# Jhuighuy/StormRuler

Hardware: AMD Instinct MI355X
Metric: CG iterations/sec, 256^3 Poisson per GPU (+ SpMV achieved HBM GB/s in `roofline`) (higher is better)
Workload: dtype f64

## Files before the change

include/storm_hip.h:

```cpp
#ifndef STORM_HIP_H_
#define STORM_HIP_H_

#include <stddef.h>
#include <stdint.h>

#ifdef __cplusplus
extern "C" {
#endif
#pragma GCC visibility push(default)

#define STORM_HIP_ABI_VERSION 6
#define STORM_HIP_HAS_TWO_STAGE 1
#define STORM_HIP_HAS_FACE_UPDATE 1
#define STORM_HIP_HAS_REDUCED_RECORDS 1

enum {
  STORM_HIP_OK = 0,
  STORM_HIP_E_INVALID = -1,
  STORM_HIP_E_HIP = -2,
  STORM_HIP_E_NO_DEVICE = -3,
  STORM_HIP_E_COMM = -4,
  STORM_HIP_E_ALLOC = -5,
  STORM_HIP_E_UNSUPPORTED = -6
};
// ... 34 lines not shown

int storm_hip_vec_create(storm_hip_ctx *ctx, int64_t n_owned, int64_t n_halo, storm_hip_vec **out);
int storm_hip_vec_create_like(const storm_hip_vec *other, storm_hip_vec **out);
int storm_hip_vec_destroy(storm_hip_vec *v);
int storm_hip_vec_size(const storm_hip_vec *v, int64_t *n_owned, int64_t *n_halo);
int storm_hip_vec_upload(storm_hip_vec *v, const double *host, int64_t n);
int storm_hip_vec_download(const storm_hip_vec *v, double *host, int64_t n);
int storm_hip_vec_device_ptr(storm_hip_vec *v, void **dev_ptr);
int storm_hip_vec_context(const storm_hip_vec *v, storm_hip_ctx **ctx);
int storm_hip_vec_get(const storm_hip_vec *v, int64_t row, double *value);

int storm_hip_block_get_column(const storm_hip_vec *X, int k, int j, storm_hip_vec *v);
int storm_hip_block_set_column(storm_hip_vec *X, int k, int j, const storm_hip_vec *v);
int storm_hip_block_dot(const storm_hip_vec *A, const storm_hip_vec *B, int k, double *out);
int storm_hip_block_axpy(storm_hip_vec *Y, const double *a, const storm_hip_vec *X, int k);

int storm_hip_fill(storm_hip_vec *y, double value);
int storm_hip_copy(storm_hip_vec *y, const storm_hip_vec *x);
int storm_hip_scale(storm_hip_vec *y, double s);
int storm_hip_div_scalar(storm_hip_vec *y, double s);
int storm_hip_axpy(storm_hip_vec *y, double a, const storm_hip_vec *x);
int storm_hip_xpay(storm_hip_vec *y, const storm_hip_vec *x, double b);
int storm_hip_axpbz(storm_hip_vec *y, double a, const storm_hip_vec *x, double b, const storm_hip_vec *z);
int storm_hip_bicgstab_p(storm_hip_vec *p, const storm_hip_vec *r, double beta, double omega,
                         const storm_hip_vec *v);
int storm_hip_lin3(storm_hip_vec *y, const storm_hip_vec *r, double s, double a, const storm_hip_vec *x,
                   double b, const storm_hip_vec *z);
int storm_hip_vmul_add(storm_hip_vec *y, double s, const storm_hip_vec *a, const storm_hip_vec *b);
enum {
  STORM_HIP_MAP_X0 = 0, STORM_HIP_MAP_X1 = 1, STORM_HIP_MAP_Y = 2, STORM_HIP_MAP_CONST = 3,
  STORM_HIP_MAP_NEG = 8, STORM_HIP_MAP_ABS = 9, STORM_HIP_MAP_SQRT = 10,
  STORM_HIP_MAP_ADD = 16, STORM_HIP_MAP_SUB = 17, STORM_HIP_MAP_MUL = 18, STORM_HIP_MAP_DIV = 19,
  STORM_HIP_MAP_MIN = 20, STORM_HIP_MAP_MAX = 21
};
int storm_hip_map(storm_hip_vec *y, const storm_hip_vec *x0, const storm_hip_vec *x1, const int32_t *program, int n_ops,
                  const double *constants, int n_constants);
int storm_hip_vmul(storm_hip_vec *y, const storm_hip_vec *a, const storm_hip_vec *b);
int storm_hip_vdiv(storm_hip_vec *y, double s, const storm_hip_vec *a, const storm_hip_vec *b);
int storm_hip_fill_randomly(storm_hip_vec *y);
void storm_hip_rng_reset(void);
int storm_hip_dot(const storm_hip_vec *a, const storm_hip_vec *b, double *result);
int storm_hip_norm2(const storm_hip_vec *a, double *result);
int storm_hip_multi_dot(const storm_hip_vec *a, const storm_hip_vec *const *bs, int k, double *out);
int storm_hip_multi_dot_begin(const storm_hip_vec *a, const storm_hip_vec *const *bs, int k, int *request);
int storm_hip_multi_dot_end(storm_hip_ctx *ctx, int request, double *out);
int storm_hip_multi_axpy(storm_hip_vec *y, const double *coefs, const storm_hip_vec *const *xs, int k);


int storm_hip_op_create_from_faces(storm_hip_ctx *ctx, int64_t n_owned, int64_t n_halo,
                                   int64_t n_faces, const int64_t *inner, const int64_t *outer,
                                   const double *coef, int64_t n_bfaces, const int64_t *b_cell,
                                   const double *b_coef, const double *volume, storm_hip_op **out);

int storm_hip_op_create_from_mesh(storm_hip_ctx *ctx, int64_t n_owned, int64_t n_halo, int32_t dim, int64_t n_faces,
                                  const int64_t *inner, const int64_t *outer, const double *area, const double *center,
                                  int64_t n_bfaces, const int64_t *b_cell, const double *b_area, const double *b_center,
                                  const double *volume, storm_hip_op **out);

int storm_hip_op_create_from_face_weights(storm_hip_ctx *ctx, int64_t n_owned, int64_t n_halo,
                                          int64_t n_faces, const int64_t *inner,
                                          const int64_t *outer, const double *w_inner,
                                          const double *w_outer, const double *diag_extra,
                                          storm_hip_op **out);

int storm_hip_op_create_from_face_weights_updatable(storm_hip_ctx *ctx, int64_t n_owned, int64_t n_halo,
                                                    int64_t n_faces, const int64_t *inner,
                                                    const int64_t *outer, const double *w_inner,
                                                    const double *w_outer, const double *diag_extra,
                                                    storm_hip_op **out);
int storm_hip_op_face_count(const storm_hip_op *op, int64_t *n_faces);
int storm_hip_op_set_face_weights(storm_hip_op *op, const storm_hip_vec *w_inner, const storm_hip_vec *w_outer,
                                  const storm_hip_vec *diag_extra);
int storm_hip_op_cells_to_faces(const storm_hip_op *op, const storm_hip_vec *cell, storm_hip_vec *at_inner,
                                storm_hip_vec *at_outer);

int storm_hip_op_create_csr(storm_hip_ctx *ctx, int64_t n_rows, int64_t n_halo,
                            const int64_t *row_ptr, const int64_t *col, const double *val,
                            storm_hip_op **out);

int storm_hip_ctx_set_option(storm_hip_ctx *ctx, const char *key, int64_t value);

int storm_hip_ctx_get_counter(storm_hip_ctx *ctx, const char *key, int64_t *value);

int storm_hip_order_cells(int32_t dim, int64_t n_cells, const double *centers, int32_t mode, int64_t *order_out,
                          int32_t *kind_out);

typedef struct storm_hip_mesh storm_hip_mesh;
typedef struct storm_hip_mesh_view {
  int32_t dim, n_nbrs;
  int64_t n_cells, n_halo, n_faces, n_bfaces;
  const int64_t *inner, *outer;
  const double *area;
  const double *center, *volume;
  const int64_t *b_cell;
  const double *b_area, *b_center;
  const int64_t *global_id;
  const int32_t *halo_owner;
  const int32_t *nbr_rank;
  const int64_t *send_ptr, *send_idx, *recv_ptr;
} storm_hip_mesh_view;

int storm_hip_mesh_read_tetgen(const char *prefix, int32_t dim, storm_hip_mesh **out);
int storm_hip_mesh_from_simplices(int32_t dim, int64_t n_nodes, const double *pos, int64_t n_listed, const int64_t *listed,
                                  const int64_t *listed_label, int64_t n_cells, const int64_t *cells, storm_hip_mesh **out);
int storm_hip_mesh_write_tetgen(const char *prefix, int32_t dim, int64_t n_nodes, const double *pos, int64_t n_listed,
                                const int64_t *listed, const int64_t *listed_label, int64_t n_cells, const int64_t *cells);
int storm_hip_mesh_create(int32_t dim, int64_t n_cells, int64_t n_halo, int64_t n_faces, const int64_t *inner,
                          const int64_t *outer, const double *area, const double *center, const double *volume,
                          int64_t n_bfaces, const int64_t *b_cell, const double *b_area, const double *b_center,
                          const int64_t *global_id, const int32_t *halo_owner, storm_hip_mesh **out);
int storm_hip_mesh_get_view(const storm_hip_mesh *mesh, storm_hip_mesh_view *view);
int storm_hip_mesh_permute_cells(storm_hip_mesh *mesh, const int64_t *order);
int storm_hip_partition_rcb(int32_t dim, int64_t n_cells, const double *centers, int32_t n_parts, int32_t *part_out);
int storm_hip_partition_slabs(int32_t dim, int64_t n_cells, const double *centers, int32_t axis, int32_t n_parts,
                              int32_t *part_out);
int storm_hip_mesh_partition(const storm_hip_mesh *global_mesh, const int32_t *part, int32_t n_parts, int32_t rank,
                             storm_hip_mesh **out);
int storm_hip_mesh_halo_plan(storm_hip_mesh *mesh, int32_t rank);
int storm_hip_op_create_from_mesh_object(storm_hip_ctx *ctx, const storm_hip_mesh *mesh, storm_hip_op **out);
int storm_hip_mesh_destroy(storm_hip_mesh *mesh);

int storm_hip_op_set_halo(storm_hip_op *op, int n_nbrs, const int32_t *nbr_rank,
                          const int64_t *send_ptr, const int64_t *send_idx,
                          const int64_t *recv_ptr);

int storm_hip_op_apply(const storm_hip_op *op, double alpha, double beta, const storm_hip_vec *x,
                       storm_hip_vec *y);

int storm_hip_op_apply_block(const storm_hip_op *op, double alpha, double beta, int k, const storm_hip_vec *X,
                             storm_hip_vec *Y);

int storm_hip_op_get_diagonal(const storm_hip_op *op, double alpha, double beta, int invert, storm_hip_vec *d);

int storm_hip_op_apply_add(const storm_hip_op *op, double alpha, const storm_hip_vec *x, storm_hip_vec *y);

int storm_hip_op_apply2(const storm_hip_op *op, double alpha1, double beta1, double alpha2, double beta2,
                        const storm_hip_vec *x, storm_hip_vec *t, storm_hip_vec *y);

typedef struct storm_hip_op_stats {
  int64_t n_rows, n_cols, nnz_offdiag;
  int64_t ell_slots;
  int64_t tail_nnz, tail_rows;
  int64_t n_slices, max_row_len;
  int64_t n_interior_slices;
  int64_t device_bytes;
  int64_t record_bytes;
  int64_t value_dictionary_size;
  int64_t offset_dictionary_size;
  int64_t paired_rows;
  int64_t tiled_planes;
  int64_t spmv_blocks;
  int64_t xcd_run_blocks;
  int64_t streamed_record_bytes;
} storm_hip_op_stats;
int storm_hip_op_get_stats(const storm_hip_op *op, storm_hip_op_stats *stats);
int storm_hip_op_destroy(storm_hip_op *op);

typedef struct storm_hip_solver_params {
  int64_t num_iterations;
  double absolute_error_tolerance;
  double relative_error_tolerance;
  int64_t num_inner_iterations;
  int32_t check_lag;
  int32_t gram_schmidt;
} storm_hip_solver_params;

typedef struct storm_hip_solver_result {
  int64_t iterations;
  double absolute_error, relative_error, initial_error;
  int32_t converged;
  int32_t path_fallback;
  int64_t num_applies;
} storm_hip_solver_result;

void storm_hip_solver_params_default(storm_hip_solver_params *p);

int storm_hip_solve_cg(const storm_hip_op *op, double alpha, double beta, const storm_hip_vec *b,
                       storm_hip_vec *x, const storm_hip_solver_params *params,
                       storm_hip_solver_result *result, double *history);
int storm_hip_solve_bicgstab(const storm_hip_op *op, double alpha, double beta, const storm_hip_vec *b,
                             storm_hip_vec *x, const storm_hip_solver_params *params,
                             storm_hip_solver_result *result, double *history);
int storm_hip_solve_gmres(const storm_hip_op *op, double alpha, double beta, const storm_hip_vec *b,
                          storm_hip_vec *x, const storm_hip_solver_params *params,
                          storm_hip_solver_result *result, double *history);

int storm_hip_solve_cg2(const storm_hip_op *op, double alpha1, double beta1, double alpha2, double beta2,
                        const storm_hip_vec *b, storm_hip_vec *x, const storm_hip_solver_params *params,
                        storm_hip_solver_result *result, double *history);

int storm_hip_solve_cg_block(const storm_hip_op *op, double alpha, double beta, int k, const storm_hip_vec *B,
                             storm_hip_vec *X, const storm_hip_solver_params *params,
                             storm_hip_solver_result *results, double *histories);

typedef struct storm_hip_krylov storm_hip_krylov;
typedef int (*storm_hip_apply_fn)(void *user, storm_hip_vec *y, const storm_hip_vec *x);

enum storm_hip_method {
  STORM_HIP_CG = 0,
  STORM_HIP_BICGSTAB = 1,
  STORM_HIP_GMRES = 2,
  STORM_HIP_FGMRES = 3,
  STORM_HIP_CGS = 4,
  STORM_HIP_TFQMR = 5,
  STORM_HIP_TFQMR1 = 6,
  STORM_HIP_BICGSTAB_L = 7,
  STORM_HIP_IDRS = 8,
  STORM_HIP_RICHARDSON = 9,
  STORM_HIP_JFNK = 10
};
enum storm_hip_side { STORM_HIP_LEFT = 0, STORM_HIP_RIGHT = 1, STORM_HIP_SYMMETRIC = 2 };

int storm_hip_krylov_create(storm_hip_ctx *ctx, int method, storm_hip_krylov **out);
int storm_hip_krylov_destroy(storm_hip_krylov *k);
int storm_hip_krylov_set_operator(storm_hip_krylov *k, const storm_hip_op *op, double alpha, double beta);
int storm_hip_krylov_set_operator_fn(storm_hip_krylov *k, storm_hip_apply_fn apply, void *user);
int storm_hip_krylov_set_operator_fd(storm_hip_krylov *k, storm_hip_apply_fn apply, void *user,
                                     const storm_hip_vec *x, const storm_hip_vec *w, double mu);
int storm_hip_krylov_apply(storm_hip_krylov *k, const storm_hip_vec *y, storm_hip_vec *z);
int storm_hip_krylov_get_int(const storm_hip_krylov *k, const char *key, int64_t *value);
int storm_hip_krylov_set_operator2(storm_hip_krylov *k, const storm_hip_op *op, double alpha1, double beta1, double alpha2,
                                   double beta2);
int storm_hip_krylov_set_preconditioner_fn(storm_hip_krylov *k, storm_hip_apply_fn apply, void *user, int side);
int storm_hip_krylov_set_preconditioner_diag(storm_hip_krylov *k, const storm_hip_vec *d, int side);
int storm_hip_krylov_set_real(storm_hip_krylov *k, const char *key, double value);
int storm_hip_krylov_solve(storm_hip_krylov *k, const storm_hip_vec *b, storm_hip_vec *x,
                           const storm_hip_solver_params *params, storm_hip_solver_result *result,
                           double *history, int64_t *pre_applies);
int storm_hip_krylov_init(storm_hip_krylov *k, const storm_hip_vec *b, storm_hip_vec *x,
                          const storm_hip_solver_params *params, double *initial_error);
int storm_hip_krylov_iterate(storm_hip_krylov *k, double *error);
int storm_hip_krylov_finalize(storm_hip_krylov *k);

typedef struct storm_hip_cheb storm_hip_cheb;
int storm_hip_cheb_coefficients(double lmin, double lmax, int degree, double *theta, double *c1, double *c2);
int storm_hip_op_gershgorin(const storm_hip_op *op, double alpha, double beta, const storm_hip_vec *scale,
                            double *lambda_max);
int storm_hip_cheb_create(const storm_hip_op *op, double alpha, double beta, const storm_hip_vec *dinv, int degree,
                          double lmin, double lmax, storm_hip_cheb **out);
int storm_hip_cheb_apply(const storm_hip_cheb *h, const storm_hip_vec *r, storm_hip_vec *z);
int storm_hip_cheb_get(const storm_hip_cheb *h, const char *key, double *value);
int storm_hip_cheb_destroy(storm_hip_cheb *h);
int storm_hip_krylov_set_preconditioner_cheb(storm_hip_krylov *k, const storm_hip_cheb *h, int side);

int storm_hip_op_build_reduced(storm_hip_op *op);
int storm_hip_op_drop_reduced(storm_hip_op *op);
int storm_hip_op_reduced_bytes(const storm_hip_op *op, int64_t *record_bytes);
int storm_hip_op_apply_reduced(const storm_hip_op *op, double alpha, double beta, const storm_hip_vec *x, storm_hip_vec *y);
int storm_hip_op_gershgorin_reduced(const storm_hip_op *op, double alpha, double beta, const storm_hip_vec *scale,
                                    double *lambda_max);
int storm_hip_cheb_create_reduced(const storm_hip_op *op, double alpha, double beta, const storm_hip_vec *dinv, int degree,
                                  double lmin, double lmax, storm_hip_cheb **out);

#define STORM_HIP_HAS_AMG 1
typedef struct storm_hip_amg_params {
  double strength_theta;
  double prolongator_omega;
  int32_t smoother_degree;
  double smoother_ratio;
  int32_t max_levels;
  int32_t coarse_rows;
  int32_t reduced_records;
} storm_hip_amg_params;
typedef struct storm_hip_amg_hierarchy storm_hip_amg_hierarchy;
typedef struct storm_hip_amg storm_hip_amg;
void storm_hip_amg_params_default(storm_hip_amg_params *params);
int storm_hip_amg_setup_csr(int64_t n_rows, const int64_t *row_ptr, const int64_t *col, const double *val,
                            const storm_hip_amg_params *params, storm_hip_amg_hierarchy **out);
int storm_hip_amg_hierarchy_destroy(storm_hip_amg_hierarchy *h);
int storm_hip_amg_hierarchy_levels(const storm_hip_amg_hierarchy *h, int *levels);
int storm_hip_amg_hierarchy_level_sizes(const storm_hip_amg_hierarchy *h, int level, int64_t *n_rows, int64_t *nnz_a,
                                        int64_t *n_aggregates, int64_t *nnz_p);
int storm_hip_amg_hierarchy_get_operator(const storm_hip_amg_hierarchy *h, int level, int64_t *row_ptr, int64_t *col,
                                         double *val);
int storm_hip_amg_hierarchy_get_aggregates(const storm_hip_amg_hierarchy *h, int level, int64_t *aggregate);
int storm_hip_amg_hierarchy_get_prolongator(const storm_hip_amg_hierarchy *h, int level, int64_t *row_ptr, int64_t *col,
                                            double *val);
int storm_hip_amg_hierarchy_get_coarse_inverse(const storm_hip_amg_hierarchy *h, double *inverse);
int storm_hip_amg_hierarchy_get(const storm_hip_amg_hierarchy *h, const char *key, double *value);
#define STORM_HIP_HAS_AMG_REFRESH 1
int storm_hip_amg_setup_csr_structural(int64_t n_rows, const int64_t *row_ptr, const int64_t *col, const double *val,
                                       const storm_hip_amg_params *params, storm_hip_amg_hierarchy **out);
int storm_hip_amg_hierarchy_get_strong(const storm_hip_amg_hierarchy *h, int level, uint8_t *mask);
int storm_hip_amg_create_refreshable(storm_hip_op *op, double alpha, double beta, const storm_hip_amg_params *params,
                                     storm_hip_amg **out);
int storm_hip_amg_refresh(storm_hip_amg *h);
int storm_hip_amg_download(storm_hip_amg *h);
int storm_hip_amg_create(storm_hip_op *op, double alpha, double beta, const storm_hip_amg_params *params, storm_hip_amg **out);
int storm_hip_amg_apply(const storm_hip_amg *h, const storm_hip_vec *r, storm_hip_vec *z);
int storm_hip_amg_restrict(const storm_hip_amg *h, int level, const storm_hip_vec *fine, storm_hip_vec *coarse);
int storm_hip_amg_prolong_add(const storm_hip_amg *h, int level, const storm_hip_vec *coarse, storm_hip_vec *fine);
int storm_hip_amg_coarse_solve(const storm_hip_amg *h, const storm_hip_vec *r, storm_hip_vec *z);
int storm_hip_amg_get(const storm_hip_amg *h, const char *key, double *value);
int storm_hip_amg_get_hierarchy(const storm_hip_amg *h, const storm_hip_amg_hierarchy **out);
int storm_hip_amg_destroy(storm_hip_amg *h);
int storm_hip_krylov_set_preconditioner_amg(storm_hip_krylov *k, const storm_hip_amg *h, int side);
#define STORM_HIP_HAS_AMG_NULLSPACE 1
int storm_hip_amg_setup_csr_nullspace(int64_t n_rows, const int64_t *row_ptr, const int64_t *col, const double *val,
                                      const storm_hip_amg_params *params, int structural, storm_hip_amg_hierarchy **out);
int storm_hip_amg_create_nullspace(storm_hip_op *op, double alpha, double beta, const storm_hip_amg_params *params,
                                   int refreshable, storm_hip_amg **out);
int storm_hip_amg_project(const storm_hip_amg *h, storm_hip_vec *v);

#pragma GCC visibility pop
#ifdef __cplusplus
}
// ... 3 lines not shown
```

stormruler_amd/_lib.py:

```python
from __future__ import annotations

import ctypes as C
import os

try:
    import torch
except Exception:
    torch = None

_HERE = os.path.dirname(os.path.abspath(__file__))
LIB_PATH = os.environ.get("STORM_HIP_LIB") or os.path.join(_HERE, "libstorm_hip.so")

if not os.path.exists(LIB_PATH):
    raise ImportError(
        f"{LIB_PATH} is missing: build it with `python -c 'import __graft_entry__ as g; g.build()'` "
        "(or `make -C stormruler_amd/csrc`).  stormruler_amd has no CPU fallback.")

lib = C.CDLL(LIB_PATH, mode=C.RTLD_GLOBAL)

f64p = C.POINTER(C.c_double)
i64p = C.POINTER(C.c_int64)
i32p = C.POINTER(C.c_int32)
vp = C.c_void_p


class SolverParams(C.Structure):
    _fields_ = [("num_iterations", C.c_int64), ("absolute_error_tolerance", C.c_double),
                ("relative_error_tolerance", C.c_double), ("num_inner_iterations", C.c_int64),
                ("check_lag", C.c_int32), ("gram_schmidt", C.c_int32)]


class SolverResult(C.Structure):
    _fields_ = [("iterations", C.c_int64), ("absolute_error", C.c_double), ("relative_error", C.c_double),
                ("initial_error", C.c_double), ("converged", C.c_int32), ("path_fallback", C.c_int32),
                ("num_applies", C.c_int64)]


class OpStats(C.Structure):
    _fields_ = [(n, C.c_int64) for n in ("n_rows", "n_cols", "nnz_offdiag", "ell_slots", "tail_nnz",
                                          "tail_rows", "n_slices", "max_row_len", "n_interior_slices",
                                          "device_bytes", "record_bytes", "value_dictionary_size",
                                          "offset_dictionary_size", "paired_rows", "tiled_planes", "spmv_blocks", "xcd_run_blocks",
                                          "streamed_record_bytes")]


class MeshView(C.Structure):
    _fields_ = [("dim", C.c_int32), ("n_nbrs", C.c_int32), ("n_cells", C.c_int64), ("n_halo", C.c_int64),
                ("n_faces", C.c_int64), ("n_bfaces", C.c_int64), ("inner", i64p), ("outer", i64p), ("area", f64p),
                ("center", f64p), ("volume", f64p), ("b_cell", i64p), ("b_area", f64p), ("b_center", f64p),
                ("global_id", i64p), ("halo_owner", i32p), ("nbr_rank", i32p), ("send_ptr", i64p), ("send_idx", i64p),
                ("recv_ptr", i64p)]


class AmgParams(C.Structure):
    _fields_ = [("strength_theta", C.c_double), ("prolongator_omega", C.c_double), ("smoother_degree", C.c_int32),
                ("smoother_ratio", C.c_double), ("max_levels", C.c_int32), ("coarse_rows", C.c_int32),
                ("reduced_records", C.c_int32)]


ALLREDUCE_FN = C.CFUNCTYPE(C.c_int, C.c_void_p, C.POINTER(C.c_double), C.c_int)
EXCHANGE_FN = C.CFUNCTYPE(C.c_int, C.c_void_p, C.c_int, C.POINTER(C.c_int32), C.POINTER(C.c_int64),
                          C.POINTER(C.c_double), C.POINTER(C.c_int64), C.POINTER(C.c_double))

APPLY_FN = C.CFUNCTYPE(C.c_int, C.c_void_p, C.c_void_p, C.c_void_p)

SIGNATURES = {
    "storm_hip_abi_version": (C.c_int, []),
    "storm_hip_last_error": (C.c_char_p, []),
    "storm_hip_ctx_create": (C.c_int, [C.c_int, C.POINTER(vp)]),
    "storm_hip_ctx_destroy": (C.c_int, [vp]),
    "storm_hip_ctx_sync": (C.c_int, [vp]),
    "storm_hip_ctx_info": (C.c_int, [vp, C.c_char_p, C.c_int, C.POINTER(C.c_int), i64p]),
    "storm_hip_ctx_set_option": (C.c_int, [vp, C.c_char_p, C.c_int64]),
    "storm_hip_order_cells": (C.c_int, [C.c_int32, C.c_int64, C.POINTER(C.c_double), C.c_int32, C.POINTER(C.c_int64),
                                        C.POINTER(C.c_int32)]),
    "storm_hip_ctx_get_counter": (C.c_int, [vp, C.c_char_p, C.POINTER(C.c_int64)]),
    "storm_hip_ctx_get_spmv_profile": (C.c_int, [vp, i64p, f64p, f64p]),
    "storm_hip_ctx_get_spmv_profile_samples": (C.c_int, [vp, C.POINTER(C.c_double), C.c_int64, C.POINTER(C.c_int64)]),
    "storm_hip_timer_start": (C.c_int, [vp]),
    "storm_hip_timer_stop": (C.c_int, [vp, C.POINTER(C.c_float)]),
    "storm_hip_comm_unique_id": (C.c_int, [vp]),
    "storm_hip_ctx_comm_init": (C.c_int, [vp, vp, C.c_int, C.c_int]),
    "storm_hip_ctx_comm_init_host": (C.c_int, [vp, C.c_int, C.c_int, ALLREDUCE_FN, EXCHANGE_FN, vp]),
    "storm_hip_map": (C.c_int, [vp, vp, vp, C.POINTER(C.c_int32), C.c_int, C.POINTER(C.c_double), C.c_int]),
    "storm_hip_ctx_comm_size": (C.c_int, [vp, C.POINTER(C.c_int), C.POINTER(C.c_int)]),
    "storm_hip_ctx_comm_rccl_view": (C.c_int, [vp, C.POINTER(C.c_int), C.POINTER(C.c_int), C.POINTER(C.c_int), C.POINTER(C.c_int),
                                               C.POINTER(C.c_int), C.c_char_p, C.c_int]),
    "storm_hip_ctx_comm_ipc_export": (C.c_int, [vp, C.c_int, C.c_int, C.c_int64, vp]),
    "storm_hip_ctx_comm_init_ipc": (C.c_int, [vp, vp]),
    "storm_hip_vec_create": (C.c_int, [vp, C.c_int64, C.c_int64, C.POINTER(vp)]),
    "storm_hip_vec_create_like": (C.c_int, [vp, C.POINTER(vp)]),
    "storm_hip_vec_destroy": (C.c_int, [vp]),
    "storm_hip_vec_size": (C.c_int, [vp, i64p, i64p]),
    "storm_hip_vec_upload": (C.c_int, [vp, f64p, C.c_int64]),
    "storm_hip_vec_download": (C.c_int, [vp, f64p, C.c_int64]),
    "storm_hip_vec_device_ptr": (C.c_int, [vp, C.POINTER(vp)]),
    "storm_hip_vec_context": (C.c_int, [vp, C.POINTER(vp)]),
    "storm_hip_vec_get": (C.c_int, [vp, C.c_int64, f64p]),
    "storm_hip_fill": (C.c_int, [vp, C.c_double]),
    "storm_hip_copy": (C.c_int, [vp, vp]),
    "storm_hip_scale": (C.c_int, [vp, C.c_double]),
    "storm_hip_div_scalar": (C.c_int, [vp, C.c_double]),
    "storm_hip_axpy": (C.c_int, [vp, C.c_double, vp]),
    "storm_hip_xpay": (C.c_int, [vp, vp, C.c_double]),
    "storm_hip_axpbz": (C.c_int, [vp, C.c_double, vp, C.c_double, vp]),
    "storm_hip_bicgstab_p": (C.c_int, [vp, vp, C.c_double, C.c_double, vp]),
    "storm_hip_fill_randomly": (C.c_int, [vp]),
    "storm_hip_rng_reset": (None, []),
    "storm_hip_lin3": (C.c_int, [vp, vp, C.c_double, C.c_double, vp, C.c_double, vp]),
    "storm_hip_vmul_add": (C.c_int, [vp, C.c_double, vp, vp]),
    "storm_hip_vdiv": (C.c_int, [vp, C.c_double, vp, vp]),
    "storm_hip_vmul": (C.c_int, [vp, vp, vp]),
    "storm_hip_dot": (C.c_int, [vp, vp, f64p]),
    "storm_hip_norm2": (C.c_int, [vp, f64p]),
    "storm_hip_multi_dot": (C.c_int, [vp, C.POINTER(vp), C.c_int, f64p]),
    "storm_hip_multi_dot_begin": (C.c_int, [vp, C.POINTER(vp), C.c_int, C.POINTER(C.c_int)]),
    "storm_hip_multi_dot_end": (C.c_int, [vp, C.c_int, f64p]),
    "storm_hip_multi_axpy": (C.c_int, [vp, f64p, C.POINTER(vp), C.c_int]),
    "storm_hip_block_get_column": (C.c_int, [vp, C.c_int, C.c_int, vp]),
    "storm_hip_block_set_column": (C.c_int, [vp, C.c_int, C.c_int, vp]),
    "storm_hip_block_dot": (C.c_int, [vp, vp, C.c_int, f64p]),
    "storm_hip_block_axpy": (C.c_int, [vp, f64p, vp, C.c_int]),
    "storm_hip_op_create_from_faces": (C.c_int, [vp, C.c_int64, C.c_int64, C.c_int64, i64p, i64p, f64p,
                                                 C.c_int64, i64p, f64p, f64p, C.POINTER(vp)]),
    "storm_hip_op_create_from_mesh": (C.c_int, [vp, C.c_int64, C.c_int64, C.c_int32, C.c_int64, i64p, i64p, f64p, f64p,
                                                C.c_int64, i64p, f64p, f64p, f64p, C.POINTER(vp)]),
    "storm_hip_op_create_from_face_weights": (C.c_int, [vp, C.c_int64, C.c_int64, C.c_int64, i64p, i64p,
                                                        f64p, f64p, f64p, C.POINTER(vp)]),
    "storm_hip_op_create_from_face_weights_updatable": (C.c_int, [vp, C.c_int64, C.c_int64, C.c_int64, i64p, i64p,
                                                                  f64p, f64p, f64p, C.POINTER(vp)]),
    "storm_hip_op_face_count": (C.c_int, [vp, C.POINTER(C.c_int64)]),
    "storm_hip_op_set_face_weights": (C.c_int, [vp, vp, vp, vp]),
    "storm_hip_op_cells_to_faces": (C.c_int, [vp, vp, vp, vp]),
    "storm_hip_op_create_csr": (C.c_int, [vp, C.c_int64, C.c_int64, i64p, i64p, f64p, C.POINTER(vp)]),
    "storm_hip_op_set_halo": (C.c_int, [vp, C.c_int, i32p, i64p, i64p, i64p]),
    "storm_hip_mesh_read_tetgen": (C.c_int, [C.c_char_p, C.c_int32, C.POINTER(vp)]),
    "storm_hip_mesh_from_simplices": (C.c_int, [C.c_int32, C.c_int64, f64p, C.c_int64, i64p, i64p, C.c_int64, i64p, C.POINTER(vp)]),
    "storm_hip_mesh_write_tetgen": (C.c_int, [C.c_char_p, C.c_int32, C.c_int64, f64p, C.c_int64, i64p, i64p, C.c_int64, i64p]),
    "storm_hip_mesh_create": (C.c_int, [C.c_int32, C.c_int64, C.c_int64, C.c_int64, i64p, i64p, f64p, f64p, f64p, C.c_int64,
                                        i64p, f64p, f64p, i64p, i32p, C.POINTER(vp)]),
    "storm_hip_mesh_get_view": (C.c_int, [vp, C.POINTER(MeshView)]),
    "storm_hip_mesh_permute_cells": (C.c_int, [vp, i64p]),
    "storm_hip_partition_rcb": (C.c_int, [C.c_int32, C.c_int64, f64p, C.c_int32, i32p]),
    "storm_hip_partition_slabs": (C.c_int, [C.c_int32, C.c_int64, f64p, C.c_int32, C.c_int32, i32p]),
    "storm_hip_mesh_partition": (C.c_int, [vp, i32p, C.c_int32, C.c_int32, C.POINTER(vp)]),
    "storm_hip_mesh_halo_plan": (C.c_int, [vp, C.c_int32]),
    "storm_hip_op_create_from_mesh_object": (C.c_int, [vp, vp, C.POINTER(vp)]),
    "storm_hip_mesh_destroy": (C.c_int, [vp]),
    "storm_hip_op_apply": (C.c_int, [vp, C.c_double, C.c_double, vp, vp]),
    "storm_hip_op_apply_block": (C.c_int, [vp, C.c_double, C.c_double, C.c_int, vp, vp]),
    "storm_hip_op_apply_add": (C.c_int, [vp, C.c_double, vp, vp]),
    "storm_hip_op_apply2": (C.c_int, [vp, C.c_double, C.c_double, C.c_double, C.c_double, vp, vp, vp]),
    "storm_hip_op_get_diagonal": (C.c_int, [vp, C.c_double, C.c_double, C.c_int, vp]),
    "storm_hip_op_get_stats": (C.c_int, [vp, C.POINTER(OpStats)]),
    "storm_hip_op_destroy": (C.c_int, [vp]),
    "storm_hip_solver_params_default": (None, [C.POINTER(SolverParams)]),
    "storm_hip_solve_cg": (C.c_int, [vp, C.c_double, C.c_double, vp, vp, C.POINTER(SolverParams),
                                     C.POINTER(SolverResult), f64p]),
    "storm_hip_solve_bicgstab": (C.c_int, [vp, C.c_double, C.c_double, vp, vp, C.POINTER(SolverParams),
                                           C.POINTER(SolverResult), f64p]),
    "storm_hip_solve_gmres": (C.c_int, [vp, C.c_double, C.c_double, vp, vp, C.POINTER(SolverParams),
                                        C.POINTER(SolverResult), f64p]),
    "storm_hip_solve_cg2": (C.c_int, [vp, C.c_double, C.c_double, C.c_double, C.c_double, vp, vp, C.POINTER(SolverParams),
                                      C.POINTER(SolverResult), f64p]),
    "storm_hip_solve_cg_block": (C.c_int, [vp, C.c_double, C.c_double, C.c_int, vp, vp, C.POINTER(SolverParams),
                                           C.POINTER(SolverResult), f64p]),
    "storm_hip_krylov_create": (C.c_int, [vp, C.c_int, C.POINTER(vp)]),
    "storm_hip_krylov_destroy": (C.c_int, [vp]),
    "storm_hip_krylov_set_operator": (C.c_int, [vp, vp, C.c_double, C.c_double]),
    "storm_hip_krylov_set_operator2": (C.c_int, [vp, vp, C.c_double, C.c_double, C.c_double, C.c_double]),
    "storm_hip_krylov_set_operator_fn": (C.c_int, [vp, APPLY_FN, vp]),
    "storm_hip_krylov_set_operator_fd": (C.c_int, [vp, APPLY_FN, vp, vp, vp, C.c_double]),
    "storm_hip_krylov_apply": (C.c_int, [vp, vp, vp]),
    "storm_hip_krylov_get_int": (C.c_int, [vp, C.c_char_p, i64p]),
    "storm_hip_krylov_set_preconditioner_fn": (C.c_int, [vp, APPLY_FN, vp, C.c_int]),
    "storm_hip_krylov_set_preconditioner_diag": (C.c_int, [vp, vp, C.c_int]),
    "storm_hip_krylov_set_real": (C.c_int, [vp, C.c_char_p, C.c_double]),
    "storm_hip_krylov_solve": (C.c_int, [vp, vp, vp, C.POINTER(SolverParams), C.POINTER(SolverResult), f64p, i64p]),
    "storm_hip_krylov_init": (C.c_int, [vp, vp, vp, C.POINTER(SolverParams), f64p]),
    "storm_hip_krylov_iterate": (C.c_int, [vp, f64p]),
    "storm_hip_krylov_finalize": (C.c_int, [vp]),
    "storm_hip_cheb_coefficients": (C.c_int, [C.c_double, C.c_double, C.c_int, f64p, f64p, f64p]),
    "storm_hip_op_gershgorin": (C.c_int, [vp, C.c_double, C.c_double, vp, f64p]),
    "storm_hip_cheb_create": (C.c_int, [vp, C.c_double, C.c_double, vp, C.c_int, C.c_double, C.c_double, C.POINTER(vp)]),
    "storm_hip_cheb_create_reduced": (C.c_int, [vp, C.c_double, C.c_double, vp, C.c_int, C.c_double, C.c_double, C.POINTER(vp)]),
    "storm_hip_op_build_reduced": (C.c_int, [vp]),
    "storm_hip_op_drop_reduced": (C.c_int, [vp]),
    "storm_hip_op_reduced_bytes": (C.c_int, [vp, C.POINTER(C.c_int64)]),
    "storm_hip_op_apply_reduced": (C.c_int, [vp, C.c_double, C.c_double, vp, vp]),
    "storm_hip_op_gershgorin_reduced": (C.c_int, [vp, C.c_double, C.c_double, vp, f64p]),
    "storm_hip_cheb_apply": (C.c_int, [vp, vp, vp]),
    "storm_hip_cheb_get": (C.c_int, [vp, C.c_char_p, f64p]),
    "storm_hip_cheb_destroy": (C.c_int, [vp]),
    "storm_hip_krylov_set_preconditioner_cheb": (C.c_int, [vp, vp, C.c_int]),
    "storm_hip_amg_params_default": (None, [C.POINTER(AmgParams)]),
    "storm_hip_amg_setup_csr": (C.c_int, [C.c_int64, i64p, i64p, f64p, C.POINTER(AmgParams), C.POINTER(vp)]),
# ... 47 lines not shown
```

stormruler_amd/csrc/common.hpp:

```cpp
#pragma once

#include <hip/hip_runtime.h>

#include <cstdint>
#include <cstdio>
#include <string>
#include <unordered_map>
#include <vector>

#include "../../include/storm_hip.h"

namespace storm {

void set_error(const char *fmt, ...) __attribute__((format(printf, 1, 2)));

#define STORM_FAIL(code, ...)        \
  do {                               \
    ::storm::set_error(__VA_ARGS__); \
    return (code);                   \
  } while (0)

#define STORM_REQUIRE(cond, ...) \
  do {                           \
    if (!(cond)) STORM_FAIL(STORM_HIP_E_INVALID, __VA_ARGS__); \
  } while (0)

#define HIP_TRY(expr)                                                               \
  do {                                                                              \
    hipError_t e_ = (expr);                                                         \
    if (e_ != hipSuccess)                                                           \
      STORM_FAIL(STORM_HIP_E_HIP, "%s failed: %s (%s:%d)", #expr, hipGetErrorString(e_), \
                 __FILE__, __LINE__);                                               \
  } while (0)

#define STORM_TRY(expr)        \
  do {                         \
    int s_ = (expr);           \
    if (s_ != 0) return s_;    \
  } while (0)

constexpr int kWave = 64;
constexpr int kBlock = 256;
constexpr int kNumXcd = 8;
constexpr int kMaxReduceBlocks = 2048;
constexpr int kMaxMulti = 64;
constexpr int kResultRing = 8;
constexpr int kSlab = 256;
constexpr int kStateRing = 64;
constexpr int kStage2 = 128;
constexpr int kSinglePassPartials = 8192;

struct SolverState {
  double s[kSlab];
  double initial_error;
  double absolute_error;
  double relative_error;
  double abs_tol, rel_tol;
  long long iteration;
  long long num_iterations;
  int done;
  int converged;
  double *history;
  unsigned long long *done_ring;
  int verify_failed;
  unsigned long long ring_gen;
};
constexpr unsigned long long kRingIterMask = (1ull << 43) - 1;
__host__ __device__ inline unsigned long long ring_word(unsigned long long gen, unsigned long long iteration, bool done) {
  return ((gen & 0xfffffull) << 44) | ((iteration & kRingIterMask) << 1) | (done ? 1ull : 0ull);
}

struct Comm;

struct LazyStmt {
  int kind = 0;
  double *y = nullptr;
  const double *v[2] = {nullptr, nullptr};
  double c[2] = {0.0, 0.0};
  int nt = 0;
  int64_t n = 0;
  const storm_hip_op *op = nullptr;
  double alpha = 0.0, beta = 0.0;
  const double *x = nullptr;
  storm_hip_vec *yvec = nullptr;
};

struct KrylovRes {
  SolverState *d_st = nullptr, *h_st = nullptr;
  unsigned long long *h_ring = nullptr, *d_ring = nullptr;
  double *S = nullptr;
  int S_cap = 0;
};

}

struct storm_hip_ctx {
  int device = 0;
  hipStream_t stream = nullptr;
  hipStream_t comm_stream = nullptr;
  hipEvent_t ev_x_ready = nullptr, ev_halo_done = nullptr;
  hipEvent_t ev_t0 = nullptr, ev_t1 = nullptr;
  int num_cus = 0;
  std::string name;
  int64_t total_mem = 0;
  double *d_partials = nullptr;
  int64_t partials_capacity = 0;
  double *d_partials2 = nullptr;
  double *d_scalars = nullptr;
  unsigned long long lat_seq = 0;
  double *d_gmres = nullptr;
  size_t gmres_capacity = 0;
  double *d_ticket_sums = nullptr;
  int *d_tickets = nullptr;
  char *d_lat_slots = nullptr;
  double *h_scalars = nullptr;
  unsigned long long *h_result_words = nullptr, *d_result_words = nullptr;
  unsigned result_seq = 0;
  struct ResultSlot {
    unsigned tag = 0;
    int k = 0;
    bool ready = false;
    double value[storm::kMaxMulti] = {};
  } result_ring[storm::kResultRing];
  storm::SolverState *d_state = nullptr;
  storm::SolverState *h_state = nullptr;
  unsigned long long *h_done_ring = nullptr;
  unsigned long long *d_done_ring = nullptr;
  std::vector<storm::KrylovRes> krylov_free;
  unsigned long long ring_gen = 0;
  int64_t opt_ell_cap = 0;
  int64_t opt_spmv_dict = 4;
  int64_t opt_spmv_spw = 0;
  int64_t opt_spmv_xcd_remap = 8;
  int64_t opt_spmv_xcd_remap_sell = 64;
  int64_t opt_nt = 1;
  int stream_reverse = 0;
  int spmv_reverse = 0;
  int64_t opt_spmv_canon_tile_min_rows = (int64_t)1 << 20;
  int64_t opt_spmv_record_index = 1;
  int64_t opt_spmv_canon_tile = 2;
  int64_t opt_mgs_steps = 4;
  int64_t opt_resident_early = 1;
  int64_t opt_resident_apply_cache = 1;
  int64_t opt_resident_halo_interleave = 1;
  int64_t opt_coop_mgs_prefetch = 1;
  int64_t opt_coop_mgs_lds_prefetch = 1;
  int64_t opt_coop_mgs_rotate_early = 1;
  int64_t opt_coop_mgs_alternate = 1;
  int64_t opt_coop_mgs_xcd_runs = 1;
  int64_t opt_coop_mgs_apply = 1;
  int64_t opt_coop_mgs_quad = 1;
  char *d_quad_slots = nullptr;
  int64_t opt_coop_mgs_lds = 1;
  int64_t opt_spmv_mixed = 1;
  int64_t opt_profile_spmv = 0;
  std::vector<storm::LazyStmt> lazy_q;
  std::unordered_map<const void *, int> occupancy;
  int64_t opt_test_disable = 0;
  int64_t opt_lazy = 0;
  int callback_depth = 0;
  int64_t n_lazy_fused_dots = 0, n_lazy_fused_pairs = 0, n_lazy_apply_dots = 0, n_lazy_cg_steps = 0;
  storm_hip_vec *lazy_spare = nullptr;
  int64_t opt_profile_comm = 0;
  int64_t opt_blas1_nt = 1;
  int64_t opt_coop_mgs = 1;
  int64_t opt_latency_publish = 1;
  int64_t opt_coop_plain = 1;
  int64_t opt_coop_force_fail = 0;
  int coop_ran = 0;
  int coop_disabled = 0;
  int coop_fallback = 0;
  int64_t coop_skip = 0, coop_backoff = 0;
  int64_t opt_latency_path = 1;
  int64_t opt_resident_path = 1;
  int64_t opt_resident_max_rows = (int64_t)1 << 22;
  int64_t opt_resident_planes = 0;
  char *d_res_exch = nullptr;
  int64_t res_exch_rows = 0;
  int64_t opt_resident_profile = 0;
  long long *d_res_prof = nullptr;
  int res_prof_blocks = 0;
  char *d_res_slots = nullptr;
  int opt_lin_fuse = 1;
  int64_t opt_ticket_verify_inject = 0;
  int64_t opt_ticket_verify = 0;
  int opt_ticket_reduce = 1;
  int opt_fused_reduce = 1;
  int opt_latency_cache = 1;
  int64_t opt_latency_rows = 1 << 19;
  int64_t opt_rccl_fused = 1;
  int64_t opt_rccl_ticket = 1;
  int64_t opt_comm_wait_seconds = 120;
  int64_t opt_rccl_flag_wait = 1;
  int64_t opt_rccl_early_halo = 1;
  int64_t opt_generic_solvers = 0;
  int64_t opt_cg_march_fill = 2048;
  int64_t opt_cg_march_alternate = 1;
  int64_t opt_cg_march = 8;
  int64_t opt_cg_residual_march = 1;
  int64_t opt_cg_residual_planes = 1;
  int64_t opt_cg_residual_chunk = 16;
  int64_t opt_cg_residual_fill = 512;
  int64_t opt_cg_pz_fold = 1;
  int64_t opt_cg_fuse = 1;
  std::vector<std::pair<size_t, double *>> pool;
  struct VecArena {
    char *base = nullptr;
    size_t bytes = 0, pitch = 0;
    int slots = 0, used = 0;
  };
  std::vector<VecArena> arenas;
  int64_t opt_vec_arena = 1;
  size_t pool_bytes = 0;
  int64_t opt_pool_bytes = (int64_t)16 << 30;
  std::vector<hipEvent_t> prof_events;
  size_t prof_used = 0;
  const int *api_done = nullptr;
  int64_t n_resident_solves = 0, n_latency_solves = 0, n_throughput_solves = 0, n_engine_solves = 0, n_cg_fused_steps = 0;
  int64_t n_host_reductions = 0;
  int64_t n_jfnk_inner_solves = 0;
  int64_t n_fd_fused_dots = 0;
  int64_t n_block_solves = 0;
  int64_t n_op_face_updates = 0;
  int64_t opt_cheb_fused = 1;
  int64_t n_cheb_fused_applies = 0, n_cheb_statement_applies = 0;
  int64_t n_op_reduced_builds = 0, n_op_reduced_refreshes = 0;
  int64_t n_cheb_reduced_applies = 0;
  int64_t opt_amg_fused = 1;
  int64_t n_amg_applies = 0, n_amg_fused_residuals = 0, n_amg_statement_residuals = 0;
  int64_t n_amg_refreshes = 0;
  int64_t n_amg_projections = 0, n_amg_fused_projections = 0;
  int64_t n_cg_residual_marches = 0;
  int64_t n_cg_residual_plane_marches = 0;
  int64_t n_cg_pz_consumer_folds = 0;
  int64_t n_mgs_chain_steps = 0, n_mgs_quad_steps = 0;
  int64_t n_mgs_lds_steps = 0;
  storm::Comm *comm = nullptr;
  int n_ranks = 1, rank = 0;
};

struct storm_hip_vec {
  storm_hip_ctx *ctx = nullptr;
  int64_t n_owned = 0, n_halo = 0;
  double *d = nullptr;
  double *base = nullptr;
  size_t bytes = 0;
  bool exposed = false;
};
constexpr int kVecGuard = 32;

namespace storm {

struct HaloPlan {
  int n_nbrs = 0;
  std::vector<int> nbr_rank;
  std::vector<int64_t> send_ptr, recv_ptr;
  int *d_send_idx = nullptr;
  double *d_sendbuf = nullptr;
  int64_t n_send = 0;
};

}

struct storm_hip_op {
  storm_hip_ctx *ctx = nullptr;
  int64_t n_rows = 0, n_halo = 0;
  int64_t n_slices = 0, n_interior_slices = 0;
  int64_t nnz = 0, ell_slots = 0, max_row_len = 0;
  int64_t *d_slice_off = nullptr;
  char *d_pack = nullptr;
  double *d_dict = nullptr;
  int dict_size = 0;
  int *d_offs = nullptr;
  int offs_size = 0;
  int xcd_group_sell = 0;
  int pair = 0;
  uint8_t *d_rec_idx = nullptr;
  uint64_t *d_rec_words = nullptr;
  int rec_words = 0;
  char *d_bnd_pack = nullptr;
  int bnd_width = 0;
  int canon_k = 0, canon_m1 = -1;
  int canon_off[7] = {0, 0, 0, 0, 0, 0, 0};
  int64_t pack_bytes = 0;
  int64_t spw = 1;
  int64_t tail_rows = 0, tail_nnz = 0;
  int *d_tail_row = nullptr;
  int64_t *d_tail_ptr = nullptr;
  int *d_tail_col = nullptr;
  double *d_tail_val = nullptr;
  int uniform_width = 0;
  std::vector<int> h_interior, h_boundary;
  int *d_interior = nullptr, *d_boundary = nullptr;
  int64_t n_interior = 0, n_boundary = 0;
  int64_t int_plane0 = 0, int_plane1 = 0;
  int64_t device_bytes = 0;
  char *d_lat_pack = nullptr;
  int64_t *d_lat_off = nullptr;
  int64_t lat_bytes = 0;
  storm::HaloPlan halo;
  int updatable = 0;
  int64_t n_faces = 0;
  int *d_src = nullptr, *d_tail_src = nullptr;
  int *d_face_inner = nullptr, *d_face_outer = nullptr;
  char *d_pack32 = nullptr;
  int64_t *d_slice_off32 = nullptr;
  float *d_tail_val32 = nullptr;
  int64_t pack32_bytes = 0;
};

constexpr int kChebMaxDegree = 16;
struct storm_hip_cheb {
  storm_hip_ctx *ctx = nullptr;
  const storm_hip_op *op = nullptr;
  double alpha = 0.0, beta = 0.0;
  const storm_hip_vec *dinv = nullptr;
  int degree = 0;
  double lmin = 0.0, lmax = 0.0, theta = 0.0, inv_theta = 0.0;
  double c1[kChebMaxDegree] = {}, c2[kChebMaxDegree] = {};
  storm_hip_vec *d[2] = {nullptr, nullptr}, *res = nullptr;
  int reduced = 0;
};

namespace storm {

struct Scal {
  const double *p;
  double v;
  double sign;
};
static inline Scal host_scal(double v) { return Scal{nullptr, v, 1.0}; }
static inline Scal dev_scal(const double *p, double sign = 1.0) { return Scal{p, 0.0, sign}; }

constexpr int kUnroll = 4;
constexpr int kStreamBlockElems = kBlock * kUnroll * 2;
constexpr int kMaxStreamBlocks = 32768;
static inline int stream_blocks(int64_t n) {
  int64_t b = (n + kStreamBlockElems - 1) / kStreamBlockElems;
  if (b < 1) b = 1;
  if (b > kMaxStreamBlocks) b = kMaxStreamBlocks;
  return (int)b;
}

constexpr int64_t kBlas1NtRows = (int64_t)6 << 20;
static inline int stream_nt(const storm_hip_ctx *c, int64_t n) {
  return (c->opt_blas1_nt == 2 || (c->opt_blas1_nt == 1 && n >= kBlas1NtRows)) ? 1 : 0;
}

int k_fill(storm_hip_ctx *c, double *y, int64_t n, double v);
int k_copy(storm_hip_ctx *c, double *y, const double *x, int64_t n, const int *done);
int k_scale(storm_hip_ctx *c, double *y, int64_t n, Scal s, bool divide, const int *done);
int k_axpbz(storm_hip_ctx *c, double *y, Scal a, const double *x, Scal b, const double *z,
            int64_t n, const int *done);
int k_bicg_p(storm_hip_ctx *c, double *p, const double *r, Scal beta, Scal omega, const double *v,
             int64_t n, const int *done);
int k_multi_dot(storm_hip_ctx *c, const double *a, const double *const *bs, int k, int64_t n,
                double *d_out, const int *done);
int k_multi_dot_partials(storm_hip_ctx *c, const double *a, const double *const *bs, int k, int64_t n,
                         int *nb_out, const int *done);
int k_multi_axpy(storm_hip_ctx *c, double *y, const double *d_coef, double sign,
                 const double *const *xs, int k, int64_t n, const int *done);
int k_dot_partials(storm_hip_ctx *c, const double *a, const double *b, int64_t n, double *partials, int nb,
                   const int *done);
int k_reduce_final(storm_hip_ctx *c, const double *partials, int nblocks, int k, double *d_out,
                   const int *done);
int k_reduce_stage1(storm_hip_ctx *c, const double **partials, int *nblocks, int k, const int *done);

int partials_reserve(storm_hip_ctx *c, int64_t need);
#define STORM_K_SWITCH(k, GO) \
  switch (k) {                \
    case 1: GO(1); break;     \
    case 2: GO(2); break;     \
    case 3: GO(3); break;     \
    case 4: GO(4); break;     \
    case 5: GO(5); break;     \
    case 6: GO(6); break;     \
    case 7: GO(7); break;     \
    default: GO(8); break;    \
  }
int vec_create_work(const storm_hip_vec *like, storm_hip_vec **out);
int vec_create_work_batch(const storm_hip_vec *like, int count, storm_hip_vec **out);
int state_read(storm_hip_ctx *c, const SolverState *d_state, SolverState *h_pinned);
int state_init(storm_hip_ctx *c, SolverState *d_state, double abs_tol, double rel_tol, long long num_iterations, double *history,
               unsigned long long *d_ring);

int ring_wait(storm_hip_ctx *c, volatile unsigned long long *ring, int64_t it, bool *stop, unsigned long long generation);

struct SpmvDot {
  const double *w = nullptr;
  bool yy = false;
  double *partials = nullptr;
  int *nblocks_out = nullptr;
  double *out[2] = {nullptr, nullptr};
  int *ticketed_out = nullptr;
  struct {
    const long long *iteration = nullptr;
    long long my_iteration = 0;
    const double *ca = nullptr, *cb = nullptr;
    double *x = nullptr;
    const double *r = nullptr;
    double *p_out = nullptr;
    double ca_imm = 0.0, cb_imm = 0.0;
  } cg;
};
int spmv_launch(const storm_hip_op *op, Scal alpha, Scal beta, const double *x, double *y,
                const SpmvDot *dot, const int *done, bool accumulate = false);
int spmv_grid_blocks(const storm_hip_op *op);
bool spmv_can_fuse_cg(const storm_hip_op *op);
bool spmv_can_march(const storm_hip_op *op);
int op_upload_slice_lists(storm_hip_op *op);
int spmv_block_launch(const storm_hip_op *op, double alpha, double beta, int k, const double *X, double *Y,
                      double *pz_partials, int *n_partials, const int *done);
int spmv_block_check(const storm_hip_op *op, int k, const storm_hip_vec *X, const storm_hip_vec *Y, const char *what);

constexpr int kLatBlock = 1024;
int occupancy_cached(storm_hip_ctx *c, const void *fn, int threads, size_t dyn_lds);
bool coop_launch(storm_hip_ctx *c, const void *fn, unsigned blocks, void **args, size_t dyn_lds = 0, unsigned threads = kLatBlock);
constexpr int kStatusCoopGaveUp = 1000;
int lat_check_gave_up(storm_hip_ctx *c);
int coop_solve_with_fallback(storm_hip_ctx *c, storm_hip_vec *x, int (*run)(void *), void *arg, int *fallback_out);

struct PackOptions {
  int64_t ell_cap = 0, spmv_dict = 4, spmv_mixed = 1, spmv_spw = 0, latency_path = 1, latency_rows = 1 << 19;
  int64_t updatable = 0;
};
struct OpImage {
  int64_t n_rows = 0, n_halo = 0, nnz = 0, n_slices = 0, max_row_len = 0, ell_slots = 0;
  int uniform_width = 0, pair = 0, bnd_width = 0, canon_k = 0, canon_m1 = -1;
  int canon_off[7] = {0, 0, 0, 0, 0, 0, 0};
  int dict_size = 0, offs_size = 0;
  int64_t spw = 1, tail_rows = 0, tail_nnz = 0, pack_bytes = 0;
  std::vector<int64_t> slice_off;
  std::vector<char> pack;
  std::vector<double> dict;
  std::vector<int> offs;
  std::vector<uint8_t> rec_idx;
  std::vector<uint64_t> rec_words;
  std::vector<char> bnd_pack;
  std::vector<int> tail_row;
  std::vector<int64_t> tail_ptr;
  std::vector<int> tail_col;
  std::vector<double> tail_val;
  std::vector<int> interior, boundary;
  std::vector<int64_t> lat_off;
  std::vector<char> lat_pack;
  int updatable = 0;
  int64_t n_faces = 0;
  std::vector<int> src;
  std::vector<int> tail_src;
  std::vector<int> face_inner, face_outer;
};
int op_pack(const PackOptions &o, int64_t n, int64_t n_halo, const std::vector<int64_t> &row_ptr, const std::vector<int> &col,
            const std::vector<double> &val, const std::vector<double> &ext, OpImage *img, const std::vector<int> *src = nullptr);
int op_pack_from_face_weights(const PackOptions &o, int64_t n_owned, int64_t n_halo, int64_t n_faces, const int64_t *inner,
                              const int64_t *outer, const double *w_inner, const double *w_outer, const double *diag_extra,
                              OpImage *img);
int op_pack_from_faces(const PackOptions &o, int64_t n_owned, int64_t n_halo, int64_t n_faces, const int64_t *inner,
                       const int64_t *outer, const double *coef, int64_t n_bfaces, const int64_t *b_cell, const double *b_coef,
                       const double *volume, OpImage *img);
int op_pack_from_mesh(const PackOptions &o, int64_t n_owned, int64_t n_halo, int32_t dim, int64_t n_faces, const int64_t *inner,
                      const int64_t *outer, const double *area, const double *center, int64_t n_bfaces, const int64_t *b_cell,
                      const double *b_area, const double *b_center, const double *volume, OpImage *img);
int op_pack_csr(const PackOptions &o, int64_t n_rows, int64_t n_halo, const int64_t *row_ptr, const int64_t *col,
                const double *val, OpImage *img);

int gershgorin_run(const storm_hip_op *op, bool reduced, double alpha, double beta, const storm_hip_vec *scale, double *lambda_max);
int op_reduced_check(const storm_hip_op *op, const char *who);
int op_reduced_require(const storm_hip_op *op, const char *who);
int op_reduced_convert(storm_hip_op *op, int *d_flag);
int op_reduced_apply(const storm_hip_op *op, double alpha, double beta, const double *x, double *y, const int *done);

bool cg_latency_eligible(const storm_hip_op *op);
int cg_latency_solve(const storm_hip_op *op, double alpha, double beta, const double *b, double *x, double *p,
                     double *r, SolverState *d_state, bool *taken);
int bicgstab_latency_solve(const storm_hip_op *op, double alpha, double beta, const double *b, double *x,
                           double *const work[4], SolverState *d_state, bool *taken);
int cg2_latency_solve(const storm_hip_op *op, double alpha1, double beta1, double alpha2, double beta2, const double *b,
                      double *x, double *const work[3], SolverState *d_state, bool *taken);

struct MgsGivens {
  SolverState *st;
  double *H, *beta, *cs, *sn, *hn_slot;
};
struct ChainApply {
  const storm_hip_op *op;
  double alpha, beta;
  const double *x;
};
int gmres_mgs_chain_coop(storm_hip_ctx *c, int64_t n, const int *done, double *w, const double *const *q, int k, int m,
                         double *H, double *norm2_out, bool normalise, bool *taken, const MgsGivens *givens,
                         const ChainApply *apply = nullptr, bool *applied = nullptr);

int gmres_orthogonalize(storm_hip_ctx *c, int64_t n, const SolverState *st, const int *done, double *qn,
                        const double *const *q, int k, int m, double *H, double *norm2_out, double *scratch,
                        int gram_schmidt, bool *normalised, const MgsGivens *givens = nullptr,
                        bool *givens_done = nullptr, const ChainApply *apply = nullptr);
int cg2_latency_try(const storm_hip_op *op, double alpha1, double beta1, double alpha2, double beta2, const storm_hip_vec *b,
                    storm_hip_vec *x, const storm_hip_solver_params *params, storm_hip_solver_result *result, double *history,
                    bool *taken);

bool res_eligible(const storm_hip_op *op, bool bicgstab);
int res_solve(bool bicgstab, const storm_hip_op *op, double alpha, double beta, const double *b, double *x, double *rt,
              SolverState *d_state, bool *taken);

int lazy_flush(storm_hip_ctx *c);
static inline int lazy_sync(storm_hip_ctx *c) { return (c != nullptr && !c->lazy_q.empty()) ? lazy_flush(c) : 0; }
int lazy_push_lin(storm_hip_ctx *c, storm_hip_vec *y, double c0, const double *v0, double c1, const double *v1, int nt, int64_t n);
int lazy_push_apply(const storm_hip_op *op, double alpha, double beta, const double *x, double *y);
bool lazy_try_dot(storm_hip_ctx *c, const double *a, const double *b, int64_t n, double *result, int *status);

int comm_allreduce_sum(storm_hip_ctx *c, double *d_buf, int count);
int comm_halo_exchange_begin(const storm_hip_op *op, double *x);
int comm_halo_exchange_end(const storm_hip_op *op);
bool comm_is_rccl(const storm_hip_ctx *c);
int comm_halo_exchange_begin_direction(const storm_hip_op *op, const double *p, const double *r, const double *cb, double *p_out);
void comm_forget_prebegun(storm_hip_ctx *c);
int comm_halo_exchange_begin_formed(const storm_hip_op *op, int mode, const double *r, const double *p, const double *v,
                                    const double *sa, const double *sb, double *target, double *alpha_seen = nullptr);
void comm_destroy(storm_hip_ctx *c);
int comm_check_error(storm_hip_ctx *c);
struct IpcDev;
struct IpcSendPlan;
struct IpcRecvPlan;
bool comm_ipc_next(storm_hip_ctx *c, IpcDev *w);
bool comm_is_ipc(const storm_hip_ctx *c);
long long comm_ipc_stat(storm_hip_ctx *c, int k);
int comm_profile_reset(storm_hip_ctx *c);
long long comm_profile_read(storm_hip_ctx *c, int k);
int comm_ipc_exchange(const storm_hip_op *op, IpcDev *w, IpcSendPlan *sp, IpcRecvPlan *rp);
int comm_ipc_send(const storm_hip_op *op, const double *x, const IpcDev &w, const IpcSendPlan &sp);
int comm_ipc_recv_copy(const storm_hip_op *op, double *x, const IpcDev &w, const IpcRecvPlan &rp);

}
```

stormruler_amd/csrc/context.hip:

```cpp
#include <cstdarg>
#include <cstring>
#include <random>

#include <algorithm>
#include "common.hpp"

#include <cstddef>

namespace storm {

static thread_local char g_error[1024] = "";

void set_error(const char *fmt, ...) {
  va_list ap;
  va_start(ap, fmt);
  vsnprintf(g_error, sizeof g_error, fmt, ap);
  va_end(ap);
}

}

using namespace storm;

static void pool_release(storm_hip_ctx *c);
// ... 42 lines not shown
  HIP_TRY(hipMalloc((void **)&c->d_lat_slots, 2 * 256 * 256 + 256));
  HIP_TRY(hipMemset(c->d_lat_slots, 0, 2 * 256 * 256 + 256));
  HIP_TRY(hipMalloc((void **)&c->d_ticket_sums, sizeof(double) * 8 * 2048));
  HIP_TRY(hipMalloc((void **)&c->d_tickets, sizeof(int) * (1 + 2048) * 16));
  HIP_TRY(hipMemset(c->d_tickets, 0, sizeof(int) * (1 + 2048) * 16));
  HIP_TRY(hipMalloc((void **)&c->d_state, sizeof(SolverState)));
  HIP_TRY(hipMemset(c->d_state, 0, sizeof(SolverState)));
  HIP_TRY(hipHostMalloc((void **)&c->h_state, sizeof(SolverState), hipHostMallocMapped));
  HIP_TRY(hipHostMalloc((void **)&c->h_done_ring, sizeof(unsigned long long) * kStateRing, hipHostMallocMapped));
  HIP_TRY(hipHostGetDevicePointer((void **)&c->d_done_ring, c->h_done_ring, 0));
  *out = c;
  return STORM_HIP_OK;
}

int storm_hip_ctx_destroy(storm_hip_ctx *c) {
  if (!c) return STORM_HIP_OK;
  (void)hipSetDevice(c->device);
  c->lazy_q.clear();
  if (c->lazy_spare) (void)storm_hip_vec_destroy(c->lazy_spare), c->lazy_spare = nullptr;
  (void)hipDeviceSynchronize();
  comm_destroy(c);
  for (auto &r : c->krylov_free) {
    if (r.S) (void)hipFree(r.S);
    (void)hipFree(r.d_st);
    (void)hipHostFree(r.h_st);
    (void)hipHostFree(r.h_ring);
  }
  for (auto &ev : c->prof_events) (void)hipEventDestroy(ev);
  pool_release(c);
  for (auto &a : c->arenas) (void)hipFree(a.base);
  (void)hipFree(c->d_partials);
  if (c->d_gmres) (void)hipFree(c->d_gmres);
  (void)hipFree(c->d_partials2);
  (void)hipFree(c->d_scalars);
  (void)hipFree(c->d_lat_slots);
  if (c->d_res_exch) (void)hipFree(c->d_res_exch);
  if (c->d_res_slots) (void)hipFree(c->d_res_slots);
  if (c->d_quad_slots) (void)hipFree(c->d_quad_slots);
  if (c->d_res_prof) (void)hipFree(c->d_res_prof);
  (void)hipFree(c->d_tickets);
  (void)hipFree(c->d_ticket_sums);
  (void)hipHostFree(c->h_scalars);
  (void)hipHostFree(c->h_result_words);
  (void)hipFree(c->d_state);
  (void)hipHostFree(c->h_state);
  (void)hipHostFree(c->h_done_ring);
  (void)hipEventDestroy(c->ev_x_ready);
  (void)hipEventDestroy(c->ev_halo_done);
  (void)hipEventDestroy(c->ev_t0);
  (void)hipEventDestroy(c->ev_t1);
  (void)hipStreamDestroy(c->stream);
  (void)hipStreamDestroy(c->comm_stream);
  delete c;
  return STORM_HIP_OK;
}

int storm_hip_ctx_sync(storm_hip_ctx *c) {
  STORM_REQUIRE(c, "ctx_sync: null context");
  STORM_TRY(lazy_sync(c));
  HIP_TRY(hipStreamSynchronize(c->comm_stream));
  HIP_TRY(hipStreamSynchronize(c->stream));
  return comm_check_error(c);
}

int storm_hip_ctx_info(storm_hip_ctx *c, char *name, int name_len, int *num_cus,
                       int64_t *total_mem_bytes) {
  STORM_REQUIRE(c, "ctx_info: null context");
  if (name && name_len > 0) {
    strncpy(name, c->name.c_str(), (size_t)name_len - 1);
    name[name_len - 1] = 0;
  }
  if (num_cus) *num_cus = c->num_cus;
  if (total_mem_bytes) *total_mem_bytes = c->total_mem;
  return STORM_HIP_OK;
}

int storm_hip_ctx_set_option(storm_hip_ctx *c, const char *key, int64_t value) {
  STORM_REQUIRE(c && key, "ctx_set_option: null argument");
  if (!strcmp(key, "ell_cap")) c->opt_ell_cap = value;
  else if (!strcmp(key, "generic_solvers")) c->opt_generic_solvers = value;
  else if (!strcmp(key, "rccl_fused")) c->opt_rccl_fused = value;
  else if (!strcmp(key, "rccl_ticket")) c->opt_rccl_ticket = value;
  else if (!strcmp(key, "rccl_early_halo")) c->opt_rccl_early_halo = value;
  else if (!strcmp(key, "rccl_flag_wait")) c->opt_rccl_flag_wait = value;
  else if (!strcmp(key, "comm_wait_seconds")) {
    STORM_REQUIRE(value >= 1 && value <= 3600, "ctx_set_option: comm_wait_seconds %lld (1 .. 3600)", (long long)value);
    c->opt_comm_wait_seconds = value;
  }
  else if (!strcmp(key, "latency_path")) c->opt_latency_path = value;
  else if (!strcmp(key, "resident_path")) c->opt_resident_path = value;
  else if (!strcmp(key, "resident_max_rows")) c->opt_resident_max_rows = value;
  else if (!strcmp(key, "resident_planes")) c->opt_resident_planes = value;
  else if (!strcmp(key, "resident_profile")) c->opt_resident_profile = value;
  else if (!strcmp(key, "coop_force_fail")) c->opt_coop_force_fail = value;
  else if (!strcmp(key, "coop_mgs")) c->opt_coop_mgs = value;
  else if (!strcmp(key, "coop_mgs_lds")) c->opt_coop_mgs_lds = value;
  else if (!strcmp(key, "coop_mgs_quad")) c->opt_coop_mgs_quad = value;
  else if (!strcmp(key, "cg_march_fill")) c->opt_cg_march_fill = value;
  else if (!strcmp(key, "resident_early")) c->opt_resident_early = value;
  else if (!strcmp(key, "mgs_steps")) c->opt_mgs_steps = value;
  else if (!strcmp(key, "vec_arena")) c->opt_vec_arena = value;
  else if (!strcmp(key, "spmv_mixed")) c->opt_spmv_mixed = value;
  else if (!strcmp(key, "spmv_canon_tile")) c->opt_spmv_canon_tile = value;
  else if (!strcmp(key, "spmv_canon_tile_min_rows")) c->opt_spmv_canon_tile_min_rows = value;
  else if (!strcmp(key, "fused_reduce")) c->opt_fused_reduce = (int)value;
  else if (!strcmp(key, "ticket_reduce")) c->opt_ticket_reduce = (int)value;
  else if (!strcmp(key, "ticket_verify")) c->opt_ticket_verify = value;
  else if (!strcmp(key, "ticket_verify_inject")) c->opt_ticket_verify_inject = value;
  else if (!strcmp(key, "lin_fuse")) c->opt_lin_fuse = (int)value;
  else if (!strcmp(key, "latency_rows")) c->opt_latency_rows = value;
  else if (!strcmp(key, "latency_cache")) c->opt_latency_cache = (int)value;
  else if (!strcmp(key, "nontemporal")) c->opt_nt = value;
  else if (!strcmp(key, "spmv_dict")) c->opt_spmv_dict = value;
  else if (!strcmp(key, "pool_bytes")) {
    c->opt_pool_bytes = value;
    if ((int64_t)c->pool_bytes > value || (value == 0 && !c->pool.empty())) {
      (void)hipStreamSynchronize(c->stream);
      pool_release(c);
    }
  }
  else if (!strcmp(key, "spmv_spw")) c->opt_spmv_spw = value;
  else if (!strcmp(key, "spmv_xcd_remap")) {
    STORM_REQUIRE(value >= 0 && value <= 4096, "ctx_set_option: spmv_xcd_remap %lld (0 .. 4096)", (long long)value);
    c->opt_spmv_xcd_remap = c->opt_spmv_xcd_remap_sell = value;
  }
  else if (!strcmp(key, "test_disable")) {
    c->opt_test_disable = value;
    c->opt_coop_mgs_apply = !(value & 1), c->opt_coop_mgs_prefetch = c->opt_coop_mgs_lds_prefetch = !(value & 2);
    c->opt_resident_apply_cache = !(value & 4), c->opt_resident_halo_interleave = !(value & 8);
    c->opt_latency_publish = !(value & 16), c->opt_coop_plain = !(value & 32), c->opt_cg_march_alternate = !(value & 64);
    c->opt_coop_mgs_xcd_runs = !(value & 128), c->opt_coop_mgs_alternate = !(value & 256);
    c->opt_coop_mgs_rotate_early = !(value & 512);
  }
  else if (!strcmp(key, "lazy_statements")) {
    if (value == 0) {
      STORM_TRY(lazy_sync(c));
      if (c->lazy_spare) (void)storm_hip_vec_destroy(c->lazy_spare), c->lazy_spare = nullptr;
    }
    c->opt_lazy = value;
  }
  else if (!strcmp(key, "profile_spmv")) c->opt_profile_spmv = value;
  else if (!strcmp(key, "profile_comm")) {
    c->opt_profile_comm = value;
    if (value != 0) STORM_TRY(comm_profile_reset(c));
  }
  else if (!strcmp(key, "cg_fuse")) c->opt_cg_fuse = value;
  else if (!strcmp(key, "cg_march")) c->opt_cg_march = value;
  else if (!strcmp(key, "cg_residual_march")) c->opt_cg_residual_march = value;
  else if (!strcmp(key, "cg_residual_planes")) c->opt_cg_residual_planes = value;
  else if (!strcmp(key, "cg_residual_chunk")) c->opt_cg_residual_chunk = value;
  else if (!strcmp(key, "cg_residual_fill")) c->opt_cg_residual_fill = value;
  else if (!strcmp(key, "cg_pz_fold")) c->opt_cg_pz_fold = value;
  else if (!strcmp(key, "spmv_record_index")) c->opt_spmv_record_index = value;
  else if (!strcmp(key, "blas1_nt")) c->opt_blas1_nt = value;
  else if (!strcmp(key, "cheb_fused")) c->opt_cheb_fused = value;
  else if (!strcmp(key, "amg_fused")) c->opt_amg_fused = value;
  else STORM_FAIL(STORM_HIP_E_INVALID, "ctx_set_option: unknown key '%s'", key);
  return STORM_HIP_OK;
}

int storm_hip_ctx_get_counter(storm_hip_ctx *c, const char *key, int64_t *value) {
  STORM_REQUIRE(c && key && value, "ctx_get_counter: null argument");
  if (!strcmp(key, "resident_solves")) *value = c->n_resident_solves;
  else if (!strcmp(key, "latency_solves")) *value = c->n_latency_solves;
  else if (!strcmp(key, "throughput_solves")) *value = c->n_throughput_solves;
  else if (!strcmp(key, "engine_solves")) *value = c->n_engine_solves;
  else if (!strcmp(key, "block_solves")) *value = c->n_block_solves;
  else if (!strcmp(key, "op_face_updates")) *value = c->n_op_face_updates;
  else if (!strcmp(key, "host_reductions")) *value = c->n_host_reductions;
  else if (!strcmp(key, "cheb_fused_applies")) *value = c->n_cheb_fused_applies;
  else if (!strcmp(key, "cheb_statement_applies")) *value = c->n_cheb_statement_applies;
  else if (!strcmp(key, "cheb_reduced_applies")) *value = c->n_cheb_reduced_applies;
  else if (!strcmp(key, "amg_applies")) *value = c->n_amg_applies;
  else if (!strcmp(key, "amg_fused_residuals")) *value = c->n_amg_fused_residuals;
  else if (!strcmp(key, "amg_statement_residuals")) *value = c->n_amg_statement_residuals;
  else if (!strcmp(key, "amg_refreshes")) *value = c->n_amg_refreshes;
  else if (!strcmp(key, "option_spmv_dict")) *value = c->opt_spmv_dict;
  else if (!strcmp(key, "amg_projections")) *value = c->n_amg_projections;
  else if (!strcmp(key, "amg_fused_projections")) *value = c->n_amg_fused_projections;
  else if (!strcmp(key, "op_reduced_builds")) *value = c->n_op_reduced_builds;
  else if (!strcmp(key, "op_reduced_refreshes")) *value = c->n_op_reduced_refreshes;
  else if (!strcmp(key, "jfnk_inner_solves")) *value = c->n_jfnk_inner_solves;
  else if (!strcmp(key, "fd_fused_dots")) *value = c->n_fd_fused_dots;
  else if (!strcmp(key, "cg_fused_steps")) *value = c->n_cg_fused_steps;
  else if (!strcmp(key, "cg_residual_marches")) *value = c->n_cg_residual_marches;
  else if (!strcmp(key, "cg_residual_plane_marches")) *value = c->n_cg_residual_plane_marches;
  else if (!strcmp(key, "cg_pz_consumer_folds")) *value = c->n_cg_pz_consumer_folds;
  else if (!strcmp(key, "mgs_chain_steps")) *value = c->n_mgs_chain_steps;
  else if (!strcmp(key, "mgs_quad_steps")) *value = c->n_mgs_quad_steps;
  else if (!strcmp(key, "mgs_lds_steps")) *value = c->n_mgs_lds_steps;
  else if (!strcmp(key, "lazy_fused_dots")) *value = c->n_lazy_fused_dots;
  else if (!strcmp(key, "lazy_fused_pairs")) *value = c->n_lazy_fused_pairs;
  else if (!strcmp(key, "lazy_apply_dots")) *value = c->n_lazy_apply_dots;
  else if (!strcmp(key, "lazy_cg_steps")) *value = c->n_lazy_cg_steps;
  else if (!strcmp(key, "lazy_waiting")) *value = (int64_t)c->lazy_q.size();
  else if (!strncmp(key, "ipc_", 4)) {
    static const char *names[6] = {"ipc_allreduce_wait_ticks", "ipc_allreduces", "ipc_ack_wait_ticks", "ipc_ack_waits",
                                   "ipc_halo_slow_poll_ticks", "ipc_halo_slow_polls"};
    int k = -1;
    for (int i = 0; i < 6; ++i)
      if (!strcmp(key, names[i])) k = i;
    STORM_REQUIRE(k >= 0, "ctx_get_counter: unknown key '%s'", key);
    const long long v = comm_ipc_stat(c, k);
    STORM_REQUIRE(v >= 0, "ctx_get_counter: '%s' needs the peer-window transport", key);
    *value = v;
  }
  else if (!strncmp(key, "rccl_prof_", 10)) {
    static const char *names[8] = {"rccl_prof_exchanges", "rccl_prof_event_to_comm_ticks", "rccl_prof_pack_ticks",
                                   "rccl_prof_sendrecv_ticks", "rccl_prof_unhidden_wait_ticks", "rccl_prof_resume_ticks",
                                   "rccl_prof_allreduces", "rccl_prof_allreduce_ticks"};
    int k = -1;
    for (int i = 0; i < 8; ++i)
      if (!strcmp(key, names[i])) k = i;
    STORM_REQUIRE(k >= 0, "ctx_get_counter: unknown key '%s'", key);
    const long long v = comm_profile_read(c, k);
    STORM_REQUIRE(v >= 0, "ctx_get_counter: '%s' needs the RCCL transport with option profile_comm = 1", key);
    *value = v;
  }
  else if (!strncmp(key, "resident_phase_max_", 19) || !strncmp(key, "resident_phase_mean_", 20)) {
    const bool mx = key[15] == 'm' && key[16] == 'a';
    const int k = atoi(key + (mx ? 19 : 20));
    STORM_REQUIRE(c->d_res_prof != nullptr && c->res_prof_blocks > 0 && k >= 0 && k < 8, "ctx_get_counter: no resident profile (option resident_profile)");
    std::vector<long long> h((size_t)c->res_prof_blocks * 8);
    HIP_TRY(hipStreamSynchronize(c->stream));
    HIP_TRY(hipMemcpy(h.data(), c->d_res_prof, sizeof(long long) * h.size(), hipMemcpyDeviceToHost));
    long long m = 0, sum = 0;
    for (int b = 0; b < c->res_prof_blocks; ++b) m = std::max(m, h[(size_t)b * 8 + k]), sum += h[(size_t)b * 8 + k];
    *value = mx ? m : sum / c->res_prof_blocks;
  } else if (!strncmp(key, "resident_phase_block_", 21)) {
    int b = 0, k = 0;
    STORM_REQUIRE(sscanf(key + 21, "%d_%d", &b, &k) == 2 && c->d_res_prof != nullptr && b >= 0 && b < c->res_prof_blocks && k >= 0 && k < 8,
                  "ctx_get_counter: no such block / phase");
    long long v = 0;
    HIP_TRY(hipStreamSynchronize(c->stream));
    HIP_TRY(hipMemcpy(&v, c->d_res_prof + (size_t)b * 8 + k, sizeof v, hipMemcpyDeviceToHost));
    *value = v;
  }
  else STORM_FAIL(STORM_HIP_E_INVALID, "ctx_get_counter: unknown key '%s'", key);
  return STORM_HIP_OK;
}

int storm_hip_ctx_get_spmv_profile(storm_hip_ctx *c, int64_t *launches, double *total_ms, double *min_ms) {
  STORM_REQUIRE(c, "get_spmv_profile: null context");
  HIP_TRY(hipStreamSynchronize(c->stream));
  double total = 0.0, mn = 0.0;
  const size_t pairs = c->prof_used / 2;
  for (size_t i = 0; i < pairs; ++i) {
    float ms = 0.f;
    HIP_TRY(hipEventElapsedTime(&ms, c->prof_events[2 * i], c->prof_events[2 * i + 1]));
    total += ms;
    if (i == 0 || ms < mn) mn = ms;
  }
  if (launches) *launches = (int64_t)pairs;
  if (total_ms) *total_ms = total;
  if (min_ms) *min_ms = mn;
  c->prof_used = 0;
  return STORM_HIP_OK;
}

int storm_hip_ctx_get_spmv_profile_samples(storm_hip_ctx *c, double *ms_out, int64_t capacity, int64_t *count) {
  STORM_REQUIRE(c && count && (ms_out || capacity == 0), "get_spmv_profile_samples: null argument");
  HIP_TRY(hipStreamSynchronize(c->stream));
  const size_t pairs = c->prof_used / 2;
  for (size_t i = 0; i < pairs && (int64_t)i < capacity; ++i) {
    float ms = 0.f;
    HIP_TRY(hipEventElapsedTime(&ms, c->prof_events[2 * i], c->prof_events[2 * i + 1]));
    ms_out[i] = ms;
  }
  *count = (int64_t)pairs;
  c->prof_used = 0;
  return STORM_HIP_OK;
}

int storm_hip_timer_start(storm_hip_ctx *c) {
  STORM_REQUIRE(c, "timer_start: null context");
  STORM_TRY(lazy_sync(c));
  HIP_TRY(hipEventRecord(c->ev_t0, c->stream));
  return STORM_HIP_OK;
}

int storm_hip_timer_stop(storm_hip_ctx *c, float *elapsed_ms) {
  STORM_REQUIRE(c && elapsed_ms, "timer_stop: null argument");
  STORM_TRY(lazy_sync(c));
  HIP_TRY(hipEventRecord(c->ev_t1, c->stream));
  HIP_TRY(hipEventSynchronize(c->ev_t1));
  HIP_TRY(hipEventElapsedTime(elapsed_ms, c->ev_t0, c->ev_t1));
  return STORM_HIP_OK;
}


}
enum { kZeroAll = 0, kZeroEdges = 1, kZeroNothing = 2 };
static int vec_create_impl(storm_hip_ctx *c, int64_t n_owned, int64_t n_halo, storm_hip_vec **out, int zero_mode);
extern "C" int storm_hip_vec_create(storm_hip_ctx *c, int64_t n_owned, int64_t n_halo, storm_hip_vec **out) {
  return vec_create_impl(c, n_owned, n_halo, out, kZeroAll);
}
namespace storm {
int ring_wait(storm_hip_ctx *c, volatile unsigned long long *ring, int64_t it, bool *stop, unsigned long long generation) {
  volatile unsigned long long *w = ring + it % kStateRing;
  const unsigned long long want = (unsigned long long)(it + 1);
  const unsigned long long gen = generation & 0xfffffull;
  auto posted = [&](bool *s) {
    const unsigned long long v = *w;
    if ((v >> 44) != gen) return false;
    const unsigned long long i = (v >> 1) & kRingIterMask;
    if (i == kRingIterMask) return *s = true, true;
// ... 319 lines not shown
```

stormruler_amd/csrc/op_pack.hip:

```cpp
#include <algorithm>
#include <atomic>
#include <cmath>
#include <cstdlib>
#include <cstring>
#include <numeric>
#include <thread>

#include "common.hpp"
#include "host_threads.hpp"
#include "op_layout.hpp"

namespace storm {
namespace {

int64_t forced_min_chunk() {
  static const int64_t forced = getenv("STORM_HIP_BUILD_MIN_CHUNK") ? atoll(getenv("STORM_HIP_BUILD_MIN_CHUNK")) : 0;
  return forced;
}
template <class F>
int parallel_chunks(int64_t n, int64_t min_chunk, F &&fn) {
  if (forced_min_chunk() > 0) min_chunk = forced_min_chunk();
  const int T = (int)std::max<int64_t>(1, std::min<int64_t>(host_threads(), n / std::max<int64_t>(1, min_chunk)));
  const int64_t per = (n + T - 1) / T;
  if (T == 1) {
// ... 185 lines not shown
      for (int k = 0; k < 7; ++k) {
        wa |= zero_v << (8 * (k + 1)), wb |= zero_v << (8 * (k + 1));
        jw |= (k < m ? ((uint64_t)od.lookup((uint64_t)merged[k]) << 2) : zero_o) << (8 * k);
      }
      for (int k = 0; k < na; ++k) {
        wa &= ~(0xffull << (8 * (pa[k] + 1)));
        wa |= ((uint64_t)vd.lookup(A.val[(size_t)(A.row_ptr[ra] + k)]) << 3) << (8 * (pa[k] + 1));
      }
      for (int k = 0; k < nb2; ++k) {
        wb &= ~(0xffull << (8 * (pb[k] + 1)));
        wb |= ((uint64_t)vd.lookup(A.val[(size_t)(A.row_ptr[rb] + k)]) << 3) << (8 * (pb[k] + 1));
      }
      char *rec = pack.data() + (p / kWave) * kPairRecBytes;
      const int l = (int)(p % kWave);
      reinterpret_cast<uint64_t *>(rec)[2 * l] = wa;
      reinterpret_cast<uint64_t *>(rec)[2 * l + 1] = wb;
      reinterpret_cast<uint64_t *>(rec + 2 * kWave * 8)[l] = jw;
    }
    widths[(size_t)t_] = pair_width;
  });
  return pr_ok.load() != 0 ? *std::max_element(widths.begin(), widths.end()) : 0;
}

int64_t boundary_groups(const Rows &A, std::vector<char> &grp_bnd) {
  grp_bnd.assign((size_t)A.groups(), 0);
  if (A.n_halo == 0) return 0;
  std::vector<int64_t> cnt((size_t)host_threads(), 0);
  parallel_chunks(A.groups(), 1 << 10, [&](int t, int64_t gb, int64_t ge) {
    for (int64_t g = gb; g < ge; ++g) {
      const int64_t r1 = std::min<int64_t>(A.n, (g + 1) * 2 * kWave);
      for (int64_t k = A.row_ptr[g * 2 * kWave]; k < A.row_ptr[r1] && !grp_bnd[(size_t)g]; ++k) grp_bnd[(size_t)g] = A.col[(size_t)k] >= A.n;
      cnt[(size_t)t] += grp_bnd[(size_t)g];
    }
  });
  return std::accumulate(cnt.begin(), cnt.end(), (int64_t)0);
}

struct OffsetRelation {
  int64_t dist[8];
  int nd = 0;
  bool before[8][8] = {};
  bool ok = true;
};
OffsetRelation offset_relation(const Rows &A, const std::vector<char> &grp_bnd) {
  std::vector<OffsetRelation> loc((size_t)host_threads());
  const int T = parallel_chunks(A.n, 1 << 14, [&](int t, int64_t rb_, int64_t re_) {
    OffsetRelation &L = loc[(size_t)t];
    for (int64_t r = rb_; L.ok && r < re_; ++r) {
      if (grp_bnd[(size_t)(r / (2 * kWave))]) continue;
      int idx[8], no = 0;
      for (int64_t k = A.row_ptr[r]; L.ok && k < A.row_ptr[r + 1]; ++k) {
        const int64_t o = (int64_t)A.col[(size_t)k] - r;
        int q = 0;
        while (q < L.nd && L.dist[q] != o) ++q;
        if (q == L.nd) {
          if (L.nd == 7) { L.ok = false; break; }
          L.dist[L.nd++] = o;
        }
        idx[no++] = q;
      }
      for (int i = 0; L.ok && i < no; ++i)
        for (int j = i + 1; j < no; ++j) {
          if (idx[i] == idx[j]) L.ok = false;
          L.before[idx[i]][idx[j]] = true;
        }
    }
  });
  OffsetRelation R;
  for (int t = 0; R.ok && t < T; ++t) {
    const OffsetRelation &L = loc[(size_t)t];
    R.ok = L.ok;
    int map_[8];
    for (int q = 0; R.ok && q < L.nd; ++q) {
      int g = 0;
      while (g < R.nd && R.dist[g] != L.dist[q]) ++g;
      if (g == R.nd) {
        if (R.nd == 7) { R.ok = false; break; }
        R.dist[R.nd++] = L.dist[q];
      }
      map_[q] = g;
    }
    for (int i = 0; R.ok && i < L.nd; ++i)
      for (int j = 0; j < L.nd; ++j)
        if (L.before[i][j]) R.before[map_[i]][map_[j]] = true;
  }
  return R;
}
int common_offset_order(const OffsetRelation &R, int64_t *canon, int *canon_m1) {
  int len = 0, m1 = -1;
  bool placed[8] = {};
  while (R.ok && len < R.nd) {
    int pick = -1;
    for (int q = 0; q < R.nd; ++q) {
      if (placed[q]) continue;
      bool free_ = true;
      for (int q2 = 0; q2 < R.nd; ++q2) free_ = free_ && !(R.before[q2][q] && !placed[q2]);
      if (free_ && (pick < 0 || R.dist[q] < R.dist[pick])) pick = q;
    }
    if (pick < 0) return 0;
    placed[pick] = true;
    canon[len++] = R.dist[pick];
  }
  for (int q = 0; q + 1 < len; ++q)
    if (canon[q] == -1 && canon[q + 1] == 1) m1 = q;
  bool cn = R.ok && ((len == 6 && m1 == 2) || (len == 4 && m1 == 1) || (len == 2 && m1 == 0));
  for (int q = 0; cn && q < len; ++q) cn = canon[q] > -(int64_t)INT32_MAX / 2 && canon[q] < (int64_t)INT32_MAX / 2;
  *canon_m1 = m1;
  return cn ? len : 0;
}

void canonical_records(const Rows &A, const ValueDict &vd, uint64_t zero_v, const std::vector<char> &grp_bnd, const int64_t *canon,
                       std::vector<char> &pack) {
  const int64_t n = A.n;
  pack.assign((size_t)A.groups() * kCanonRecBytes, 0);
  parallel_chunks(A.groups() * kWave, 1 << 13, [&](int, int64_t p_begin, int64_t p_end) {
    for (int64_t p = p_begin; p < p_end; ++p) {
      uint64_t w2[2];
      for (int half = 0; half < 2; ++half) {
        const int64_t r = 2 * p + half;
        uint64_t w = r < n ? ((uint64_t)vd.lookup(A.ext[(size_t)r]) << 3) : zero_v;
        for (int k = 0; k < 7; ++k) w |= zero_v << (8 * (k + 1));
        if (r < n) {
          int q = 0;
          const bool by_entry = grp_bnd[(size_t)(r / (2 * kWave))] != 0;
          for (int64_t k = A.row_ptr[r]; k < A.row_ptr[r + 1]; ++k) {
            if (by_entry) q = (int)(k - A.row_ptr[r]);
            else while (canon[q] != (int64_t)A.col[(size_t)k] - r) ++q;
            w &= ~(0xffull << (8 * (q + 1)));
            w |= ((uint64_t)vd.lookup(A.val[(size_t)k]) << 3) << (8 * (q + 1));
          }
        }
        w2[half] = w;
      }
      uint64_t *rec = reinterpret_cast<uint64_t *>(pack.data() + (p / kWave) * kCanonRecBytes);
      rec[2 * (p % kWave)] = w2[0], rec[2 * (p % kWave) + 1] = w2[1];
    }
  });
}

void row_record_index(const std::vector<char> &pack, std::vector<uint8_t> &rec_idx, std::vector<uint64_t> &rec_words) {
  const int64_t n_words = (int64_t)pack.size() / 8;
  auto word_at = [&](int64_t i) {
    uint64_t w;
    memcpy(&w, pack.data() + (size_t)i * 8, 8);
    return w;
  };
  ValueDict wd;
  if (!wd.add_all(n_words, word_at)) return;
  rec_idx.resize((size_t)n_words);
  parallel_chunks(n_words, 1 << 16, [&](int, int64_t b, int64_t e) {
    for (int64_t i = b; i < e; ++i) rec_idx[(size_t)i] = (uint8_t)wd.lookup(word_at(i));
  });
  rec_words = std::move(wd.values);
}

std::vector<int> slice_widths(const Rows &A, int64_t cap, int64_t slot_bytes, int64_t w_op, OpImage *img) {
  const int64_t n_slices = img->n_slices;
  std::vector<int> width((size_t)n_slices, 0);
  img->slice_off.assign((size_t)n_slices + 1, 0);
  bool uniform = true;
  for (int64_t s = 0; s < n_slices; ++s) {
    int64_t w = 0;
    const int64_t r1 = std::min<int64_t>(A.n, (s + 1) * kWave);
    for (int64_t r = s * kWave; r < r1; ++r) w = std::max(w, A.len(r));
    w = std::min(w, cap);
    if (w_op > 0) w = w_op;
    width[(size_t)s] = (int)w;
    img->slice_off[(size_t)s + 1] = img->slice_off[(size_t)s] + (w_op > 0 ? (int64_t)kWave * 16 : kExtBytes + w * slot_bytes);
    if (s > 0 && width[(size_t)s] != width[0]) uniform = false;
    img->ell_slots += w * kWave;
  }
  img->uniform_width = (uniform && n_slices > 0 && width[0] > 0) ? width[0] : 0;
  return width;
}
void sell_records(const Rows &A, const std::vector<int> &width, ValueDict *vd, ValueDict *od, OpImage *img) {
  const int64_t n = A.n;
  const bool cv = vd != nullptr, co = od != nullptr;
  img->pack.assign((size_t)img->slice_off[(size_t)img->n_slices], 0);
  if (A.src) img->src.assign((size_t)((img->slice_off[(size_t)img->n_slices] - img->n_slices * kExtBytes) / (kSlotBytes / kWave)), -1);
  for (int64_t s = 0; s < img->n_slices; ++s) {
    const int W = width[(size_t)s];
    char *rec = img->pack.data() + img->slice_off[(size_t)s];
    int *s_ = A.src ? img->src.data() + (img->slice_off[(size_t)s] - s * kExtBytes) / (kSlotBytes / kWave) : nullptr;
    double *e_ = reinterpret_cast<double *>(rec);
    uint64_t *i_ = reinterpret_cast<uint64_t *>(rec);
    int *c_ = reinterpret_cast<int *>(rec + kExtBytes);
    double *v_ = reinterpret_cast<double *>(rec + kExtBytes + (int64_t)W * (kWave * 4));
    bool touches_halo = false;
    for (int l = 0; l < kWave; ++l) {
      const int64_t r = s * kWave + l;
      const int64_t pad_col = r < n ? r : (n > 0 ? n - 1 : 0);
      const int64_t b = r < n ? A.row_ptr[r] : 0, e = r < n ? A.row_ptr[r + 1] : 0;
      uint64_t iw = 0, jw = 0;
      if (cv) iw = (uint64_t)vd->index(r < n ? A.ext[(size_t)r] : 0.0);
      else e_[l] = r < n ? A.ext[(size_t)r] : 0.0;
      if (co) {
        for (int k = 0; k < W; ++k) {
          const bool real = b + k < e;
          iw |= (uint64_t)vd->index(real ? A.val[(size_t)(b + k)] : 0.0) << (8 * (k + 1));
          jw |= (uint64_t)od->find(real ? (uint64_t)((int64_t)A.col[(size_t)(b + k)] - r) : 0, false) << (8 * k);
          touches_halo |= real && A.col[(size_t)(b + k)] >= n;
        }
        i_[2 * l] = iw, i_[2 * l + 1] = jw;
      }
      const int np2 = W >> 1;
      for (int k = 0; k < (co ? 0 : W); ++k) {
        const int at = (k < 2 * np2) ? ((k >> 1) * kWave + l) * 2 + (k & 1) : np2 * 2 * kWave + l;
        const bool real = b + k < e;
        c_[at] = real ? A.col[(size_t)(b + k)] : (int)pad_col;
        const double w_k = real ? A.val[(size_t)(b + k)] : 0.0;
        if (cv) iw |= (uint64_t)vd->index(w_k) << (8 * (k + 1));
        else v_[at] = w_k;
        if (s_ && real) s_[at] = (*A.src)[(size_t)(b + k)];
        touches_halo |= real && c_[at] >= n;
      }
      if (cv && !co) i_[l] = iw;
      if (e - b > W) {
        img->tail_row.push_back((int)r);
        for (int64_t k = b + W; k < e; ++k) {
          img->tail_col.push_back(A.col[(size_t)k]);
          img->tail_val.push_back(A.val[(size_t)k]);
          if (A.src) img->tail_src.push_back((*A.src)[(size_t)k]);
          touches_halo |= A.col[(size_t)k] >= n;
        }
        img->tail_ptr.push_back((int64_t)img->tail_col.size());
      }
    }
    (touches_halo ? img->boundary : img->interior).push_back((int)s);
  }
}

void dictionary_tables(const ValueDict *vd, const ValueDict *od, OpImage *img) {
  if (vd) {
    img->dict.assign((size_t)kDictSize, 0.0);
    for (size_t k = 0; k < vd->values.size(); ++k) memcpy(&img->dict[k], &vd->values[k], 8);
    img->dict_size = (int)vd->values.size();
  }
  if (od) {
    img->offs.assign((size_t)kDictSize, 0);
    for (size_t k = 0; k < od->values.size(); ++k) img->offs[k] = (int)(int64_t)od->values[k];
    img->offs_size = (int)od->values.size();
  }
}

}

int op_pack(const PackOptions &options, int64_t n, int64_t n_halo, const std::vector<int64_t> &row_ptr, const std::vector<int> &col,
            const std::vector<double> &val, const std::vector<double> &ext, OpImage *img, const std::vector<int> *src) {
  PackOptions o = options;
  if (src) o.spmv_dict = 0, o.latency_path = 0;
  const Rows A{n, n_halo, row_ptr, col, val, ext, src};
  *img = OpImage();
  img->n_rows = n, img->n_halo = n_halo, img->nnz = row_ptr[n];
  BuildTimer timer;
  const int64_t max_len = img->max_row_len = longest_row(A);
  latency_image(o, A, img->lat_off, img->lat_pack);
  int64_t cap = o.ell_cap;
  if (cap <= 0) {
    const double mean = n > 0 ? (double)img->nnz / (double)n : 0.0;
    cap = std::max<int64_t>(8, (int64_t)std::ceil(2.0 * mean));
  }
  const int64_t w_op = std::min(max_len, cap);
  timer.lap("latency copy, max row");
  ValueDict vd, od;
  const bool cv = o.spmv_dict != 0 && w_op <= 7 && value_dictionary(A, vd);
  timer.lap("value dictionary");
  const bool co = cv && o.spmv_dict >= 2 && w_op > 0 && n + n_halo < (int64_t)INT32_MAX && offset_dictionary(A, w_op, od);
  timer.lap("offset dictionary");
  const int64_t n_groups = A.groups();
  const int pair_width = co && o.spmv_dict >= 3 && max_len <= std::min<int64_t>(7, cap) && vd.values.size() <= 32 &&
                                 od.values.size() <= 64 && n + n_halo < ((int64_t)1 << 28)
                             ? paired_records(A, vd, od, img->pack)
                             : 0;
  timer.lap("paired records");
  const bool pr = pair_width > 0;
  img->tail_ptr.assign(1, 0);
  std::vector<char> grp_bnd;
  const int64_t n_bnd_groups = pr ? boundary_groups(A, grp_bnd) : 0;
  int64_t canon[8];
  int canon_len = 0, canon_m1 = -1;
  if (pr && o.spmv_dict >= 4 && 2 * n_bnd_groups <= n_groups && (n_bnd_groups == 0 || o.spmv_mixed != 0))
    canon_len = common_offset_order(offset_relation(A, grp_bnd), canon, &canon_m1);
  if (canon_len > 0) {
    for (int64_t g = 0; g < n_groups; ++g)
      if (grp_bnd[(size_t)g])
        img->bnd_pack.insert(img->bnd_pack.end(), img->pack.begin() + (size_t)g * kPairRecBytes, img->pack.begin() + (size_t)(g + 1) * kPairRecBytes);
    canonical_records(A, vd, (uint64_t)vd.index(0.0) << 3, grp_bnd, canon, img->pack);
    timer.lap("canonical order + records");
    row_record_index(img->pack, img->rec_idx, img->rec_words);
    timer.lap("row-record index");
    img->canon_k = canon_len, img->canon_m1 = canon_m1;
    for (int k = 0; k < canon_len; ++k) img->canon_off[k] = (int)canon[k];
  }
  if (pr) {
    const int rec_bytes = canon_len > 0 ? kCanonRecBytes : kPairRecBytes;
    img->pair = canon_len > 0 ? 2 : 1;
    img->bnd_width = pair_width;
    img->uniform_width = canon_len > 0 ? canon_len : pair_width;
    img->n_slices = n_groups;
    img->ell_slots = n_groups * 2 * kWave * img->uniform_width;
    img->slice_off.resize((size_t)n_groups + 1);
    for (int64_t s = 0; s <= n_groups; ++s) img->slice_off[(size_t)s] = s * rec_bytes;
    for (int64_t s = 0; s < n_groups; ++s) (grp_bnd[(size_t)s] ? img->boundary : img->interior).push_back((int)s);
    img->spw = 1;
  } else {
    img->n_slices = (n + kWave - 1) / kWave;
    sell_records(A, slice_widths(A, cap, cv ? kColSlotBytes : kSlotBytes, co ? w_op : 0, img), cv ? &vd : nullptr, co ? &od : nullptr, img);
    img->spw = (o.spmv_spw == 1 || o.spmv_spw == 2 || o.spmv_spw == 4) ? o.spmv_spw : 2;
  }
  dictionary_tables(cv ? &vd : nullptr, co ? &od : nullptr, img);
  img->tail_rows = (int64_t)img->tail_row.size();
  img->tail_nnz = (int64_t)img->tail_col.size();
  img->pack_bytes = (int64_t)img->pack.size() + (int64_t)img->bnd_pack.size();
  return STORM_HIP_OK;
}

namespace {

template <class W>
void rows_from_faces(int64_t n_owned, int64_t n_faces, const int64_t *inner, const int64_t *outer, W &&weight,
                     std::vector<int64_t> &row_ptr, std::vector<int> &col, std::vector<double> &val, std::vector<int> *src = nullptr) {
  row_ptr.assign((size_t)n_owned + 1, 0);
  auto put = [&](size_t at, int64_t c, int64_t f, bool outer_side) {
    col[at] = (int)c, val[at] = weight(f, outer_side);
    if (src) (*src)[at] = (int)(2 * f + (outer_side ? 1 : 0));
  };
  const int64_t face_chunk = forced_min_chunk() > 0 ? forced_min_chunk() : (1 << 16);
  const int T = (int)std::max<int64_t>(1, std::min<int64_t>(host_threads(), n_faces / face_chunk));
  const int64_t per = (n_faces + T - 1) / T;
  std::vector<std::vector<unsigned char>> cnt((size_t)T);
  std::atomic<int> overflow{0};
  parallel_chunks(T, 1, [&](int, int64_t tb, int64_t te) {
    for (int64_t t = tb; t < te; ++t) {
      std::vector<unsigned char> &c_ = cnt[(size_t)t];
      c_.assign((size_t)n_owned, 0);
      for (int64_t f = t * per; f < std::min(n_faces, (t + 1) * per); ++f) {
        const int64_t a = inner[f], b = outer[f];
        if (a < n_owned && ++c_[(size_t)a] == 0) overflow = 1;
        if (b < n_owned && ++c_[(size_t)b] == 0) overflow = 1;
      }
    }
  });
  if (overflow.load()) {
    parallel_chunks(n_owned, 1 << 15, [&](int, int64_t r0, int64_t r1) {
      for (int64_t f = 0; f < n_faces; ++f) {
        const int64_t a = inner[f], b = outer[f];
        if (a >= r0 && a < r1) row_ptr[(size_t)a + 1]++;
        if (b >= r0 && b < r1) row_ptr[(size_t)b + 1]++;
      }
    });
    for (int64_t i = 0; i < n_owned; ++i) row_ptr[(size_t)i + 1] += row_ptr[(size_t)i];
    col.resize((size_t)row_ptr[(size_t)n_owned]), val.resize(col.size());
    if (src) src->resize(col.size());
    std::vector<int64_t> fill(row_ptr.begin(), row_ptr.end() - 1);
    parallel_chunks(n_owned, 1 << 15, [&](int, int64_t r0, int64_t r1) {
      for (int64_t f = 0; f < n_faces; ++f) {
        const int64_t a = inner[f], b = outer[f];
        if (a >= r0 && a < r1) {
          const size_t at = (size_t)fill[(size_t)a]++;
          put(at, b, f, false);
        }
        if (b >= r0 && b < r1) {
          const size_t at = (size_t)fill[(size_t)b]++;
          put(at, a, f, true);
        }
      }
    });
    return;
  }
  parallel_chunks(n_owned, 1 << 16, [&](int, int64_t r0, int64_t r1) {
    for (int64_t r = r0; r < r1; ++r) {
      int64_t run = 0;
      for (int t = 0; t < T; ++t) {
        const int64_t here = cnt[(size_t)t][(size_t)r];
        cnt[(size_t)t][(size_t)r] = (unsigned char)run;
        run += here;
      }
      row_ptr[(size_t)r + 1] = run;
    }
  });
  bool long_rows = false;
  for (int64_t i = 0; i < n_owned; ++i) {
    long_rows |= row_ptr[(size_t)i + 1] > 255;
    row_ptr[(size_t)i + 1] += row_ptr[(size_t)i];
  }
  col.resize((size_t)row_ptr[(size_t)n_owned]), val.resize(col.size());
  if (src) src->resize(col.size());
  if (long_rows) {
    std::vector<int64_t> fill(row_ptr.begin(), row_ptr.end() - 1);
    for (int64_t f = 0; f < n_faces; ++f) {
      const int64_t a = inner[f], b = outer[f];
      if (a < n_owned) {
        const size_t at = (size_t)fill[(size_t)a]++;
        put(at, b, f, false);
      }
      if (b < n_owned) {
        const size_t at = (size_t)fill[(size_t)b]++;
        put(at, a, f, true);
      }
    }
    return;
  }
  parallel_chunks(T, 1, [&](int, int64_t tb, int64_t te) {
    for (int64_t t = tb; t < te; ++t) {
      std::vector<unsigned char> &o_ = cnt[(size_t)t];
      for (int64_t f = t * per; f < std::min(n_faces, (t + 1) * per); ++f) {
        const int64_t a = inner[f], b = outer[f];
        if (a < n_owned) {
          const size_t at = (size_t)(row_ptr[(size_t)a] + o_[(size_t)a]++);
          put(at, b, f, false);
        }
        if (b < n_owned) {
          const size_t at = (size_t)(row_ptr[(size_t)b] + o_[(size_t)b]++);
          put(at, a, f, true);
        }
      }
    }
  });
}

int64_t first_bad_face(int64_t n_faces, const int64_t *inner, const int64_t *outer, int64_t nt) {
  std::atomic<int64_t> bad{-1};
  parallel_chunks(n_faces, 1 << 16, [&](int, int64_t fb, int64_t fe) {
    for (int64_t f = fb; f < fe; ++f) {
      const int64_t a = inner[f], b = outer[f];
      if (!(a >= 0 && a < nt && b >= 0 && b < nt) || a == b) {
        int64_t cur = bad.load();
        while ((cur < 0 || f < cur) && !bad.compare_exchange_weak(cur, f)) {
        }
        return;
      }
    }
  });
  return bad.load();
}
int require_valid_faces(const char *who, int64_t n_faces, const int64_t *inner, const int64_t *outer, int64_t nt) {
  const int64_t f = first_bad_face(n_faces, inner, outer, nt);
  if (f < 0) return STORM_HIP_OK;
  const int64_t a = inner[f], b = outer[f];
  STORM_REQUIRE(a >= 0 && a < nt && b >= 0 && b < nt, "%s: face %lld joins cells (%lld, %lld) outside [0, %lld)", who,
                (long long)f, (long long)a, (long long)b, (long long)nt);
  STORM_REQUIRE(a != b, "%s: face %lld joins cell %lld to itself", who, (long long)f, (long long)a);
// ... 126 lines not shown
```

stormruler_amd/csrc/solver_cg.hip:

```cpp
#include <algorithm>
#include "solver_fused.hpp"
#include "blas1_device.hpp"
#include "spmv_device.hpp"

namespace storm {

template <class Fold, class Gamma>
__device__ __forceinline__ double cg_r_alpha_of(SolverState *st, bool folds, Fold fold, Gamma gamma) {
  double pz;
  if (folds) {
    pz = fold();
    if (blockIdx.x == 0 && threadIdx.x == 0) st->s[S_PZ] = pz;
  } else {
    pz = st->s[S_PZ];
  }
  const double alpha = safe_divide(gamma(), pz);
  if (blockIdx.x == 0 && threadIdx.x == 0) st->s[S_ALPHA] = alpha;
  return alpha;
}
__device__ __forceinline__ double cg_r_alpha(SolverState *st, const double *__restrict__ pz_partials, int n_pz, double *lds4) {
  return cg_r_alpha_of(st, pz_partials != nullptr, [&] { return block_fold(pz_partials, n_pz, lds4); }, [&] { return st->s[S_GAMMA]; });
}
__device__ __forceinline__ double cg_r_alpha(SolverState *st, bool folds, const FoldWhole &pz_flight, int n_pz, double gamma,
                                             double *lds4) {
// ... 16 lines not shown
      if (use_ipc != 2) do_step(STEP_CG_RR, st, GmresDev{});
    }
  }
}

__global__ __launch_bounds__(kBlock) void cg_r_kernel(int64_t n, SolverState *st, double *__restrict__ r,
                                                      const double *__restrict__ z,
                                                      double *__restrict__ partials, int nt,
                                                      const double *__restrict__ pz_partials, int n_pz, int reverse,
                                                      TicketArgs tickets, IpcDev w, int use_ipc) {
  if (st->done) return;
  __shared__ double lds4[4];
  const unsigned bx = reverse ? gridDim.x - 1 - blockIdx.x : blockIdx.x;
  const double alpha = cg_r_alpha(st, pz_partials, n_pz, lds4);
  double acc = 0.0;
  const int64_t n2 = n >> 1;
  double2v *r2 = reinterpret_cast<double2v *>(r);
  const double2v *z2 = reinterpret_cast<const double2v *>(z);
  nt_dispatch(nt, [&](auto nt) {
  for (int64_t base = (int64_t)bx * (kBlock * kUnroll) + threadIdx.x; base < n2;
       base += (int64_t)gridDim.x * (kBlock * kUnroll)) {
    double2v vr[kUnroll], vz[kUnroll];
#pragma unroll
    for (int u = 0; u < kUnroll; ++u) {
      const int64_t i = base + u * kBlock;
      if (i < n2) vr[u] = ldv(r2 + i, nt), vz[u] = ldv(z2 + i, nt);
    }
#pragma unroll
    for (int u = 0; u < kUnroll; ++u) {
      const int64_t i = base + u * kBlock;
      if (i < n2) {
        vr[u] -= alpha * vz[u];
        stv(r2 + i, vr[u], nt);
        acc += vr[u].x * vr[u].x;
        acc += vr[u].y * vr[u].y;
      }
    }
  }
  });
  if ((n & 1) && bx == 0 && threadIdx.x == 0) {
    const double vr = r[n - 1] - alpha * z[n - 1];
    r[n - 1] = vr;
    acc += vr * vr;
  }
  cg_r_finish(st, acc, bx, partials, tickets, w, use_ipc, lds4);
}

template <bool IDX>
__global__ __launch_bounds__(kBlock) void cg_r_recompute_kernel(int64_t n, SolverState *st, double *__restrict__ r,
                                                                const double *__restrict__ p, SellArgs A, CanonTileArgs T,
                                                                Scal alpha_s, Scal beta_s, const double *__restrict__ pz_partials,
                                                                int n_pz, int reverse, TicketArgs tickets) {
  if (st->done) return;
  __shared__ double lds4[4];
  __shared__ double dict_sh[32];
  extern __shared__ __attribute__((aligned(16))) unsigned long long words_sh[];
  const int lane = threadIdx.x & (kWave - 1);
  if (threadIdx.x < 32) dict_sh[threadIdx.x] = A.dict[threadIdx.x];
  if (IDX) rec_table_fill(A, words_sh);
  __syncthreads();
  const unsigned bx = reverse ? gridDim.x - 1 - blockIdx.x : blockIdx.x;
  const double alpha = cg_r_alpha(st, pz_partials, n_pz, lds4);
  const double op_alpha = ld_scal2(alpha_s), op_beta = ld_scal2(beta_s);
  const int64_t a = T.a, b = T.b, mg = T.max_gather;
  const char *pg = reinterpret_cast<const char *>(p) - (size_t)kVecGuard * 8;
  auto pair_at = [&](int64_t row) {
    int64_t gi = row + kVecGuard;
    gi = gi < 0 ? 0 : (gi > mg ? mg : gi);
    return *reinterpret_cast<const double2v *>(pg + (size_t)gi * 8);
  };
  auto one_at = [&](int64_t row) {
    int64_t gi = row + kVecGuard;
    gi = gi < 0 ? 0 : (gi > mg + 1 ? mg + 1 : gi);
    return *reinterpret_cast<const double *>(pg + (size_t)gi * 8);
  };
  double acc = 0.0;
  const int64_t n2 = n >> 1;
  double2v *r2 = reinterpret_cast<double2v *>(r);
  for (int64_t base = (int64_t)bx * (kBlock * kUnroll) + threadIdx.x; base - lane < n2;
       base += (int64_t)gridDim.x * (kBlock * kUnroll)) {
    double2v vr[kUnroll], c[kUnroll], nb[kUnroll][4];
    double el[kUnroll];
    RecRaw<IDX> w[kUnroll];
#pragma unroll
    for (int u = 0; u < kUnroll; ++u) {
      const int64_t i = base + u * kBlock;
      const int64_t row = 2 * (i < n2 ? i : n2 - 1);
      vr[u] = r2[row >> 1];
      c[u] = pair_at(row);
      w[u] = rec_load<IDX>(A, (uint32_t)row);
      nb[u][0] = pair_at(row - b), nb[u][1] = pair_at(row - a), nb[u][2] = pair_at(row + a), nb[u][3] = pair_at(row + b);
      el[u] = 0.0;
      if (lane == 0) el[u] = one_at(row - 1);
      if (lane == kWave - 1) el[u] = one_at(row + 2);
    }
#pragma unroll
    for (int u = 0; u < kUnroll; ++u) {
      const int64_t i = base + u * kBlock;
      double2v xg[6];
      xg[0] = nb[u][0], xg[1] = nb[u][1], xg[4] = nb[u][2], xg[5] = nb[u][3];
      const double left = dpp_shift<0x138>(c[u].y);
      const double right = dpp_shift<0x130>(c[u].x);
      xg[2].x = lane == 0 ? el[u] : left;
      xg[2].y = c[u].x;
      xg[3].x = c[u].y;
      xg[3].y = lane == kWave - 1 ? el[u] : right;
      const double2v vz = lattice_pair_apply(dict_sh, rec_word<IDX>(w[u], words_sh), xg, c[u], op_alpha, op_beta);
      if (i < n2) {
        vr[u] -= alpha * vz;
        r2[i] = vr[u];
        acc += vr[u].x * vr[u].x;
        acc += vr[u].y * vr[u].y;
      }
    }
  }
  cg_r_finish(st, acc, bx, nullptr, tickets, IpcDev{}, 0, lds4);
}

static bool cg_r_recompute_applies(const storm_hip_op *op, bool tick) {
  storm_hip_ctx *c = op->ctx;
  MarchArgs M;
  int nb = 0;
  return c->opt_cg_residual_march != 0 && tick && c->comm == nullptr && c->opt_ticket_verify == 0 && op->n_rows % 2 == 0 &&
         spmv_can_march(op) && cg_march_geometry(op, &M, &nb);
}
static int cg_r_recompute_run(const storm_hip_op *op, int nbv, Scal alpha, Scal beta, const double *p, SolverState *st, double *r,
                              const double *pz_partials, int n_pz, int reverse) {
  storm_hip_ctx *c = op->ctx;
  CanonTileArgs T;
  int nbt = 0;
  STORM_REQUIRE(canon_tile_geometry(op, &T, &nbt), "cg: the residual recompute needs a lattice operator");
  const SellArgs A = lattice_args(op);
  const size_t lds = sizeof(uint64_t) * (size_t)A.rec_words_n;
  const TicketArgs tk{c->d_tickets, c->d_partials, c->d_ticket_sums};
  if (A.rec_idx != nullptr)
    hipLaunchKernelGGL(cg_r_recompute_kernel<true>, dim3(nbv), dim3(kBlock), lds, c->stream, op->n_rows, st, r, p, A, T, alpha,
                       beta, pz_partials, n_pz, reverse, tk);
  else
    hipLaunchKernelGGL(cg_r_recompute_kernel<false>, dim3(nbv), dim3(kBlock), lds, c->stream, op->n_rows, st, r, p, A, T, alpha,
                       beta, pz_partials, n_pz, reverse, tk);
  HIP_TRY(hipGetLastError());
  return STORM_HIP_OK;
}

struct ResidualPlanesArgs {
  int a, b;
  int runs_per_plane;
  int per_xcd;
  int planes;
  int nz;
  int max_gather;
};
constexpr int kResidualMaxChunk = 32;
template <int HLP, bool IDX>
__global__ __launch_bounds__(kBlock) void cg_r_planes_kernel(SolverState *st, double *__restrict__ r, const double *__restrict__ p,
                                                             SellArgs A, ResidualPlanesArgs G, Scal alpha_s, Scal beta_s,
                                                             const double *__restrict__ pz_partials, int n_pz, int reverse,
                                                             TicketArgs tickets) {
  const int done = st->done;
  const double gamma = st->s[S_GAMMA];
  __shared__ double lds4[4];
  __shared__ double dict_sh[32];
  __shared__ double wave_part[kResidualMaxChunk * (kBlock / kWave)];
  extern __shared__ __attribute__((aligned(16))) double plane_sh[];
  const int a = G.a, b = G.b;
  const int ldw = kStreamBlockElems + 2 * a;
  unsigned long long *words_sh = reinterpret_cast<unsigned long long *>(plane_sh + 2 * ldw);
  const int lane = threadIdx.x & (kWave - 1);
  const int wave = __builtin_amdgcn_readfirstlane(threadIdx.x >> 6);
  const int bidx = reverse ? (int)(gridDim.x - 1 - blockIdx.x) : (int)blockIdx.x;
  int zc, yt;
  if (G.per_xcd > 0) {
    const int xcd = bidx & (kNumXcd - 1), j = bidx >> 3;
    zc = j / G.per_xcd;
    yt = xcd * G.per_xcd + (j - zc * G.per_xcd);
  } else {
    zc = bidx / G.runs_per_plane;
    yt = bidx - zc * G.runs_per_plane;
  }
  const int z_begin = zc * G.nz, z_end = min(z_begin + G.nz, G.planes), nz = z_end - z_begin;
  auto plane = [&](int s) { return z_begin + s; };
  const int p0 = yt * kStreamBlockElems;
  const char *pg = reinterpret_cast<const char *>(p) - (size_t)kVecGuard * 8;
  double2v *r2 = reinterpret_cast<double2v *>(r);

  struct Flight {
    double2v p[kUnroll], hp[HLP];
  };
  int hat[HLP], hjj[HLP];
#pragma unroll
  for (int i = 0; i < HLP; ++i) {
    const int h = (int)threadIdx.x + kBlock * i;
    hjj[i] = 2 * h < a ? 2 * h - a : kStreamBlockElems + 2 * h - a;
    hat[i] = h < a ? a + hjj[i] : -1;
  }
  auto load_p = [&](int64_t row) {
    int64_t gi = row + kVecGuard;
    gi = gi < 0 ? 0 : (gi > (int64_t)G.max_gather ? (int64_t)G.max_gather : gi);
    return *reinterpret_cast<const double2v *>(pg + (size_t)gi * 8);
  };
  auto issue_p = [&](int zp, bool own, Flight &f) {
    const int64_t row0 = (int64_t)zp * b + p0;
#pragma unroll
    for (int u = 0; u < kUnroll; ++u) f.p[u] = load_p(row0 + 2 * ((int)threadIdx.x + kBlock * u));
#pragma unroll
    for (int i = 0; i < HLP; ++i) {
      f.hp[i] = double2v{0.0, 0.0};
      if (own && hat[i] >= 0) f.hp[i] = load_p(row0 + hjj[i]);
    }
  };
  auto issue_rw = [&](int zp, double2v (&vr)[kUnroll], RecRaw<IDX> (&w)[kUnroll]) {
    const int64_t row0 = (int64_t)zp * b + p0;
#pragma unroll
    for (int u = 0; u < kUnroll; ++u) {
      const int64_t row = row0 + 2 * ((int)threadIdx.x + kBlock * u);
      vr[u] = r2[row >> 1];
      w[u] = rec_load<IDX>(A, (uint32_t)row);
    }
  };

  Flight cur, nxt, fl;
  double2v pm[kUnroll], vr[kUnroll];
  RecRaw<IDX> w[kUnroll];
  issue_p(plane(-1), false, fl);
#pragma unroll
  for (int u = 0; u < kUnroll; ++u) pm[u] = fl.p[u];
  issue_p(plane(0), true, cur);
  issue_rw(plane(0), vr, w);
  issue_p(plane(1), 1 < nz, nxt);
  const bool folds = pz_partials != nullptr;
  FoldWhole pz_flight;
  if (folds) block_fold_issue(pz_partials, n_pz, pz_flight);
  if (threadIdx.x < 32) dict_sh[threadIdx.x] = A.dict[threadIdx.x];
  if (IDX) rec_table_fill(A, words_sh);
  if (done) return;
  const double alpha = cg_r_alpha(st, folds, pz_flight, n_pz, gamma, lds4);
  const double op_alpha = ld_scal2(alpha_s), op_beta = ld_scal2(beta_s);
  for (int s = 0; s < nz; ++s) {
    const int zp = plane(s);
    double *buf = plane_sh + (s & 1) * ldw;
#pragma unroll
    for (int u = 0; u < kUnroll; ++u) *reinterpret_cast<double2v *>(&buf[a + 2 * ((int)threadIdx.x + kBlock * u)]) = cur.p[u];
#pragma unroll
    for (int i = 0; i < HLP; ++i)
      if (hat[i] >= 0) *reinterpret_cast<double2v *>(&buf[hat[i]]) = cur.hp[i];
    double2v vrn[kUnroll];
    RecRaw<IDX> wn[kUnroll];
    if (s + 2 <= nz) issue_p(plane(s + 2), s + 2 < nz, fl);
    if (s + 1 < nz) issue_rw(plane(s + 1), vrn, wn);
    __syncthreads();
    const int64_t i0 = (((int64_t)zp * b + p0) >> 1) + threadIdx.x;
    double acc = 0.0;
#pragma unroll
    for (int u = 0; u < kUnroll; ++u) {
      const int at = a + 2 * ((int)threadIdx.x + kBlock * u);
      double2v xg[6];
      march_neighbours(buf, at, a, lane, pm[u], nxt.p[u], cur.p[u], xg);
      const double2v vz = lattice_pair_apply(dict_sh, rec_word<IDX>(w[u], words_sh), xg, cur.p[u], op_alpha, op_beta);
      vr[u] -= alpha * vz;
      r2[i0 + u * kBlock] = vr[u];
      acc += vr[u].x * vr[u].x;
      acc += vr[u].y * vr[u].y;
    }
    acc = wave_sum_down(acc);
    if (lane == 0) wave_part[s * (kBlock / kWave) + wave] = acc;
#pragma unroll
    for (int u = 0; u < kUnroll; ++u) pm[u] = cur.p[u], vr[u] = vrn[u], w[u] = wn[u];
    cur = nxt, nxt = fl;
  }
  __syncthreads();
  if (threadIdx.x >= kWave) return;
  const bool on = lane < nz;
  const double mine = on ? block_sum256_of_waves(wave_part + lane * (kBlock / kWave)) : 0.0;
  const unsigned bxv = on ? (unsigned)(plane(lane) * G.runs_per_plane + yt) : 0u;
  double total;
  if (ticket_reduce_wave0_slots(tickets, mine, on, bxv, (unsigned)(G.planes * G.runs_per_plane), &total) && threadIdx.x == 0) {
    st->s[S_GAMMA_NEW] = total;
    do_step(STEP_CG_RR, st, GmresDev{});
  }
}

static bool cg_r_planes_geometry(const storm_hip_op *op, ResidualPlanesArgs *G, int *n_blocks) {
  storm_hip_ctx *c = op->ctx;
  CanonTileArgs T;
  int nbt = 0;
  if (c->opt_cg_residual_planes == 0 || !canon_tile_geometry(op, &T, &nbt)) return false;
  const int64_t n = op->n_rows;
  if (T.b % kStreamBlockElems != 0 || n % T.b != 0 || n / kStreamBlockElems > kMaxStreamBlocks) return false;
  if ((int64_t)sizeof(double) * 2 * (kStreamBlockElems + 2 * T.a) + (int64_t)sizeof(uint64_t) * op->rec_words > 60 * 1024) return false;
  G->a = T.a, G->b = T.b, G->max_gather = T.max_gather;
  G->runs_per_plane = T.b / kStreamBlockElems;
  G->per_xcd = (G->runs_per_plane % kNumXcd == 0 && c->opt_spmv_xcd_remap != 0) ? G->runs_per_plane / kNumXcd : 0;
  G->planes = (int)(n / T.b);
  const int64_t zc = std::min<int64_t>(std::max<int64_t>(c->opt_cg_residual_chunk, 2), kResidualMaxChunk);
  const int64_t want = c->opt_cg_residual_fill;
  const int64_t fill = want > 0 ? (int64_t)G->planes * G->runs_per_plane / want : zc;
  G->nz = (int)std::min<int64_t>(std::min<int64_t>(zc, std::max<int64_t>(2, fill)), G->planes);
  *n_blocks = ((G->planes + G->nz - 1) / G->nz) * G->runs_per_plane;
  return true;
}
static int cg_r_planes_run(const storm_hip_op *op, const ResidualPlanesArgs &G, int n_blocks, Scal alpha, Scal beta, const double *p,
                           SolverState *st, double *r, const double *pz_partials, int n_pz, int reverse, double *rr_partials) {
  storm_hip_ctx *c = op->ctx;
  STORM_REQUIRE(pz_partials == nullptr || n_pz <= kSinglePassPartials, "cg: the plane march folds at most %d partials of <p,z>, not %d",
                kSinglePassPartials, n_pz);
  const SellArgs A = lattice_args(op);
  const size_t lds = sizeof(double) * 2 * (size_t)(kStreamBlockElems + 2 * G.a) + sizeof(uint64_t) * (size_t)A.rec_words_n;
  const TicketArgs tk{c->d_tickets, rr_partials, c->d_ticket_sums};
#define PLANES_GO(HLP_, IX_)                                                                                                   \
  hipLaunchKernelGGL((cg_r_planes_kernel<HLP_, IX_>), dim3(n_blocks), dim3(kBlock), lds, c->stream, st, r, p, A, G, alpha, beta, \
                     pz_partials, n_pz, reverse, tk)
  if (G.a <= kBlock) {
    if (A.rec_idx != nullptr) PLANES_GO(1, true);
    else PLANES_GO(1, false);
  } else {
    if (A.rec_idx != nullptr) PLANES_GO(2, true);
    else PLANES_GO(2, false);
  }
#undef PLANES_GO
  HIP_TRY(hipGetLastError());
  return STORM_HIP_OK;
}

constexpr int kUnrollXp = 1;
__global__ __launch_bounds__(kBlock) void cg_xp_kernel(int64_t n, const SolverState *st, long long my_iteration,
                                                       double *__restrict__ x, double *__restrict__ p,
                                                       const double *__restrict__ r, int nt, int reverse) {
  if (st->iteration < my_iteration) return;
  const unsigned bx = reverse ? gridDim.x - 1 - blockIdx.x : blockIdx.x;
  const bool update_p = !st->done && r != nullptr;
  const double alpha = st->s[S_ALPHA], beta = st->s[S_BETA];
  const int64_t n2 = n >> 1;
  double2v *x2 = reinterpret_cast<double2v *>(x), *p2 = reinterpret_cast<double2v *>(p);
  const double2v *r2 = reinterpret_cast<const double2v *>(r);
  nt_dispatch(nt, [&](auto nt) {
  for (int64_t base = (int64_t)bx * (kBlock * kUnrollXp) + threadIdx.x; base < n2;
       base += (int64_t)gridDim.x * (kBlock * kUnrollXp)) {
    double2v vx[kUnrollXp], vp[kUnrollXp], vr[kUnrollXp];
#pragma unroll
    for (int u = 0; u < kUnrollXp; ++u) {
      const int64_t i = base + u * kBlock;
      if (i < n2) {
        vx[u] = ldv(x2 + i, nt), vp[u] = ldv(p2 + i, nt);
        if (update_p) vr[u] = ldv(r2 + i, nt);
      }
    }
#pragma unroll
    for (int u = 0; u < kUnrollXp; ++u) {
      const int64_t i = base + u * kBlock;
      if (i < n2) {
        vx[u] += alpha * vp[u];
        stv(x2 + i, vx[u], nt);
        if (update_p) stv(p2 + i, vr[u] + beta * vp[u], nt);
      }
    }
  }
  });
  if ((n & 1) && bx == 0 && threadIdx.x == 0) {
    const int64_t i = n - 1;
    x[i] += alpha * p[i];
    if (update_p) p[i] = r[i] + beta * p[i];
  }
}
static inline int xp_blocks(int64_t n) {
  int64_t b = ((n >> 1) + kBlock * kUnrollXp - 1) / (kBlock * kUnrollXp);
  return (int)(b < 1 ? 1 : (b > 131072 ? 131072 : b));
}


struct CgRoads {
  bool may_fuse_step;
  bool ipc, tick;
  bool tick_spmv;
  bool rccl, fuse_step;
  bool rtick;
  bool r_march;
  bool r_planes;
  ResidualPlanesArgs planes_args;
  int planes_blocks = 0;
};
static CgRoads cg_roads(Driver &d, int nbv) {
  storm_hip_ctx *c = d.c;
  CgRoads w;
  w.may_fuse_step = c->opt_cg_fuse != 0 && spmv_can_fuse_cg(d.op);
  w.ipc = c->comm != nullptr && comm_ipc_next(c, &d.ipc_w);
  w.tick = c->opt_ticket_reduce != 0 && (c->comm == nullptr || w.ipc) && nbv <= kTicketGroup * kTicketMaxGroups;
  w.tick_spmv = w.tick && !w.ipc && 4 * (int64_t)spmv_grid_blocks(d.op) <= kSinglePassPartials;
  w.rccl = c->comm != nullptr && comm_is_rccl(c);
  w.fuse_step = w.may_fuse_step && (w.rccl ? true : ((c->comm == nullptr || w.ipc) && w.tick && !w.tick_spmv));
  w.rtick = w.rccl && w.fuse_step && c->opt_ticket_reduce != 0 && c->opt_rccl_ticket != 0 && nbv <= kTicketGroup * kTicketMaxGroups;
  w.r_march = w.fuse_step && !w.rccl && cg_r_recompute_applies(d.op, w.tick);
  w.r_planes = w.r_march && cg_r_planes_geometry(d.op, &w.planes_args, &w.planes_blocks);
  if (w.fuse_step) ++c->n_cg_fused_steps;
  if (w.r_march) ++c->n_cg_residual_marches;
  if (w.r_planes) ++c->n_cg_residual_plane_marches;
  return w;
}

static int solve_cg_body(const FusedSolveArgs &args) {
  const storm_hip_op *op = args.op;
  const double *b = args.b->d;
  double *x = args.x->d;
  Driver d;
  STORM_TRY(prepare_state(args, &d));
  storm_hip_ctx *c = d.c;
  const int64_t n = d.n;
  VecPool pool;
  if (res_eligible(op, false)) {
    bool taken = false;
    STORM_TRY(res_solve(false, op, d.alpha, d.beta, b, x, nullptr, c->d_state, &taken));
    if (taken) return ++c->n_resident_solves, collect(d, args, 1);
  }
  if (cg_latency_eligible(op)) {
    STORM_TRY(pool.make(args.x, 2));
    bool taken = false;
    STORM_TRY(cg_latency_solve(op, d.alpha, d.beta, b, x, pool.v[0]->d, pool.v[1]->d, c->d_state, &taken));
    if (taken) return ++c->n_latency_solves, collect(d, args, 1);
  }
  ++c->n_throughput_solves;
  const size_t v0 = pool.v.size();
  const int nbv = stream_blocks(n);
  const CgRoads road = cg_roads(d, nbv);
  STORM_TRY(pool.make(args.x, road.may_fuse_step ? 4 : 3, false));
  static const int kRolesFused[4] = {1, 2, 0, 3}, kRolesPlain[3] = {0, 1, 2};
  const int *role = road.may_fuse_step ? kRolesFused : kRolesPlain;
  double *p = pool.v[v0 + role[0]]->d, *r = pool.v[v0 + role[1]]->d, *z = pool.v[v0 + role[2]]->d;
  double *p_alt = road.fuse_step ? pool.v[v0 + role[3]]->d : nullptr;

  int nb = 0;
  STORM_TRY(d.apply(x, r, &nb, {}, false));
  STORM_TRY(d.init_residual(r, b, p));
  STORM_TRY(d.finish(nbv, 1, S_GAMMA, STEP_CG_INIT, true));
  int64_t cur_it = 0;
  const int nt_stream = stream_nt(c, n);
  int64_t last_enqueued = -1;
  bool pz_fold_counted = false;
  auto enqueue_iteration = [&]() -> int {
    const int q = road.fuse_step ? 0 : (int)(cur_it & 1);
    c->spmv_reverse = q;
    int pz_done = 0;
    int st_apply;
    const bool r_march_now = road.r_march && cur_it > 0;
    if (road.fuse_step && cur_it > 0) {
      const CgStep step{(long long)cur_it, x, r, p_alt};
      st_apply = d.apply(p, r_march_now ? nullptr : z, &nb, {.w = p, .ticketed = &pz_done}, true, &step);
      std::swap(p, p_alt);
    } else {
      st_apply = d.apply(p, z, &nb, {.w = p, .out0 = road.tick_spmv ? (int)S_PZ : -1, .ticketed = &pz_done});
    }
    last_enqueued = cur_it;
    c->spmv_reverse = 0;
    STORM_TRY(st_apply);
    const bool tickets_now = road.tick && (nb > kSinglePassPartials || road.ipc);
    const Driver::Road allow = road.rtick ? Driver::ROAD_TICKETS_RCCL
                                          : !tickets_now ? Driver::ROAD_PLAIN : road.ipc ? Driver::ROAD_TICKETS_IPC : Driver::ROAD_TICKETS;
    Driver::Road ran;
    const double *pz_partials = nullptr, *const pz_with[1] = {z};
    const int64_t rr_slots = road.r_planes ? (int64_t)road.planes_args.planes * road.planes_args.runs_per_plane : 0;
    const bool pz_fold_now = c->opt_cg_pz_fold != 0 && r_march_now && road.r_planes && c->comm == nullptr && !tickets_now &&
                             !pz_done && nb > 0 && nb <= kSinglePassPartials && nb + rr_slots <= c->partials_capacity;
    if (pz_fold_now && !pz_fold_counted) ++c->n_cg_pz_consumer_folds, pz_fold_counted = true;
    if (!pz_fold_now) STORM_TRY(d.finish_dots(pz_done, nb, 1, S_PZ, p, pz_with, allow, STEP_NONE, &ran, &pz_partials));
    if (pz_fold_now) {
      STORM_TRY(cg_r_planes_run(op, road.planes_args, road.planes_blocks, host_scal(d.alpha), host_scal(d.beta), p, d.st, r, c->d_partials,
                                nb, 1 - q, c->d_partials + nb));
    } else if (r_march_now && road.r_planes) {
      STORM_TRY(cg_r_planes_run(op, road.planes_args, road.planes_blocks, host_scal(d.alpha), host_scal(d.beta), p, d.st, r, pz_partials,
                                (int)kStage2, 1 - q, c->d_partials));
    } else if (r_march_now) {
      STORM_TRY(cg_r_recompute_run(op, nbv, host_scal(d.alpha), host_scal(d.beta), p, d.st, r, pz_partials, (int)kStage2, 1 - q));
// ... 68 lines not shown
```

stormruler_amd/csrc/spmv.hip:

```cpp
#include <algorithm>
#include <cstring>

#include "spmv_device.hpp"

namespace storm {


static int interior_blocks(const storm_hip_op *op, bool accumulate, int n_send_blocks) {
  CanonTileArgs T;
  int nbt = 0;
  if (!accumulate && canon_tile_geometry(op, &T, &nbt, true)) return nbt + n_send_blocks;
  return -1;
}

struct SpmvFormat {
  const char *name;
  bool (*run)(const RangeLaunch &L);
};
static const SpmvFormat kSpmvFormats[] = {
    {"format 4 on a lattice: tiles of 1024 rows x 2|4 planes (spmv_lattice.hip)", spmv_tile_run},
    {"formats 4, 5: paired rows, common offsets (spmv_pair.hip)", spmv_canon_run},
    {"format 3: paired rows, per-lane offsets (spmv_pair.hip)", spmv_pair_run},
    {"formats 1, 2 of one width: value (+ offset) dictionaries (spmv_dict.hip)", spmv_dict_run},
    {"format 0 and mixed-width dictionary records: sliced ELL (spmv_sell.hip)", spmv_sell_run},
// ... 271 lines not shown
    const double row = fabs(beta + alpha * md[i]) + fabs(alpha) * ab[i];
    v = fmax(v, scale ? fabs(scale[i]) * row : row);
  }
  for (int off = kWave / 2; off > 0; off >>= 1) v = fmax(v, __shfl_xor(v, off, kWave));
  if ((threadIdx.x & (kWave - 1)) == 0) atomicMax(out, (unsigned long long)__double_as_longlong(v));
}

__global__ void safe_invert_kernel(int64_t n, double *__restrict__ d) {
  const int64_t i = (int64_t)blockIdx.x * blockDim.x + threadIdx.x;
  if (i < n) d[i] = d[i] == 0.0 ? 0.0 : 1.0 / d[i];
}


}

using namespace storm;

extern "C" {

int storm_hip_op_apply(const storm_hip_op *op, double alpha, double beta, const storm_hip_vec *x,
                       storm_hip_vec *y) {
  STORM_REQUIRE(op && x && y, "op_apply: null argument");
  STORM_REQUIRE(x->ctx == op->ctx && y->ctx == op->ctx, "op_apply: context mismatch");
  STORM_REQUIRE(x != y && x->d != y->d, "op_apply: x and y must not alias");
  STORM_REQUIRE(x->n_owned == op->n_rows && y->n_owned == op->n_rows, "op_apply: operator has %lld rows, x %lld, y %lld",
                (long long)op->n_rows, (long long)x->n_owned, (long long)y->n_owned);
  STORM_REQUIRE(x->n_halo >= op->n_halo, "op_apply: x has %lld halo rows, operator needs %lld", (long long)x->n_halo,
                (long long)op->n_halo);
  if (op->ctx->opt_lazy != 0 && op->ctx->callback_depth == 0 && op->ctx->api_done == nullptr)
    return lazy_push_apply(op, alpha, beta, x->d, y->d);
  STORM_TRY(lazy_sync(op->ctx));
  return spmv_launch(op, host_scal(alpha), host_scal(beta), x->d, y->d, nullptr, op->ctx->api_done);
}

int storm_hip_op_apply_block(const storm_hip_op *op, double alpha, double beta, int k, const storm_hip_vec *X,
                             storm_hip_vec *Y) {
  STORM_TRY(spmv_block_check(op, k, X, Y, "op_apply_block"));
  HIP_TRY(hipSetDevice(op->ctx->device));
  STORM_TRY(lazy_sync(op->ctx));
  return spmv_block_launch(op, alpha, beta, k, X->d, Y->d, nullptr, nullptr, op->ctx->api_done);
}

int storm_hip_op_apply_add(const storm_hip_op *op, double alpha, const storm_hip_vec *x, storm_hip_vec *y) {
  STORM_REQUIRE(op && x && y, "op_apply_add: null argument");
  STORM_REQUIRE(x->ctx == op->ctx && y->ctx == op->ctx, "op_apply_add: context mismatch");
  STORM_REQUIRE(x != y && x->d != y->d, "op_apply_add: x and y must not alias");
  STORM_REQUIRE(x->n_owned == op->n_rows && y->n_owned == op->n_rows, "op_apply_add: operator has %lld rows, x %lld, y %lld",
                (long long)op->n_rows, (long long)x->n_owned, (long long)y->n_owned);
  STORM_REQUIRE(x->n_halo >= op->n_halo, "op_apply_add: x has %lld halo rows, operator needs %lld", (long long)x->n_halo,
                (long long)op->n_halo);
  STORM_TRY(lazy_sync(op->ctx));
  return spmv_launch(op, host_scal(alpha), host_scal(0.0), x->d, y->d, nullptr, op->ctx->api_done, true);
}

int storm_hip_op_get_diagonal(const storm_hip_op *op, double alpha, double beta, int invert, storm_hip_vec *d) {
  STORM_REQUIRE(op && d, "op_get_diagonal: null argument");
  STORM_REQUIRE(d->ctx == op->ctx, "op_get_diagonal: context mismatch");
  STORM_REQUIRE(d->n_owned == op->n_rows, "op_get_diagonal: operator has %lld rows, d %lld", (long long)op->n_rows,
                (long long)d->n_owned);
  if (op->n_rows == 0) return STORM_HIP_OK;
  storm_hip_ctx *c = op->ctx;
  HIP_TRY(hipSetDevice(c->device));
  STORM_TRY(lazy_sync(c));
  const int64_t n64 = (op->n_rows + kWave - 1) / kWave;
  const int nb = (int)((n64 + (kBlock / kWave) - 1) / (kBlock / kWave));
  hipLaunchKernelGGL(diag_sell_kernel, dim3(nb), dim3(kBlock), 0, c->stream, op->d_pack, op->d_slice_off, op->n_rows,
                     op->d_dict, op->pair >= 2 ? op->pair + 2 : op->pair ? 3 : (int)(op->offs_size > 0), alpha, beta, d->d);
  if (op->tail_rows > 0)
    hipLaunchKernelGGL(diag_tail_kernel, dim3((int)((op->tail_rows + 255) / 256)), dim3(256), 0, c->stream,
                       op->tail_rows, op->d_tail_row, op->d_tail_ptr, op->d_tail_val, alpha, d->d);
  if (invert)
    hipLaunchKernelGGL(safe_invert_kernel, dim3((int)((op->n_rows + 255) / 256)), dim3(256), 0, c->stream, op->n_rows,
                       d->d);
  HIP_TRY(hipGetLastError());
  return STORM_HIP_OK;
}

int storm_hip_op_gershgorin(const storm_hip_op *op, double alpha, double beta, const storm_hip_vec *scale, double *lambda_max) {
  STORM_REQUIRE(op && lambda_max, "op_gershgorin: null argument");
  STORM_REQUIRE(scale == nullptr || (scale->ctx == op->ctx && scale->n_owned == op->n_rows),
                "op_gershgorin: the scale must be a vector of the operator's context and size");
  if (op->halo.n_nbrs > 0 || op->n_halo > 0 || op->ctx->comm != nullptr)
    STORM_FAIL(STORM_HIP_E_UNSUPPORTED, "op_gershgorin: single-rank operators only (the operator has a halo plan or halo "
                                        "columns, or the context a communicator)");
  return gershgorin_run(op, false, alpha, beta, scale, lambda_max);
}

}

int storm::gershgorin_run(const storm_hip_op *op, bool reduced, double alpha, double beta, const storm_hip_vec *scale,
                          double *lambda_max) {
  *lambda_max = 0.0;
  if (op->n_rows == 0) return STORM_HIP_OK;
  storm_hip_ctx *c = op->ctx;
  HIP_TRY(hipSetDevice(c->device));
  STORM_TRY(lazy_sync(c));
  const int64_t n = op->n_rows;
  double *work = nullptr;
  HIP_TRY(hipMalloc((void **)&work, sizeof(double) * (size_t)(2 * n + 1)));
  double *md = work, *ab = work + n;
  unsigned long long *word = reinterpret_cast<unsigned long long *>(work + 2 * n);
  hipError_t e = hipMemsetAsync(word, 0, sizeof(*word), c->stream);
  const int64_t n64 = (n + kWave - 1) / kWave;
  const int nb = (int)((n64 + (kBlock / kWave) - 1) / (kBlock / kWave));
  if (reduced)
    hipLaunchKernelGGL(rowsum_sell_kernel<true>, dim3(nb), dim3(kBlock), 0, c->stream, op->d_pack32, op->d_slice_off32, n,
                       (const double *)nullptr, 0, md, ab, op->uniform_width);
  else
    hipLaunchKernelGGL(rowsum_sell_kernel<false>, dim3(nb), dim3(kBlock), 0, c->stream, op->d_pack, op->d_slice_off, n, op->d_dict,
                       op->pair >= 2 ? op->pair + 2 : op->pair ? 3 : (int)(op->offs_size > 0), md, ab, 0);
  if (op->tail_rows > 0 && reduced)
    hipLaunchKernelGGL(rowsum_tail_kernel<float>, dim3((int)((op->tail_rows + 255) / 256)), dim3(256), 0, c->stream, op->tail_rows,
                       op->d_tail_row, op->d_tail_ptr, op->d_tail_val32, md, ab);
  else if (op->tail_rows > 0)
    hipLaunchKernelGGL(rowsum_tail_kernel<double>, dim3((int)((op->tail_rows + 255) / 256)), dim3(256), 0, c->stream, op->tail_rows,
                       op->d_tail_row, op->d_tail_ptr, op->d_tail_val, md, ab);
  hipLaunchKernelGGL(gershgorin_fold_kernel, dim3((int)std::min<int64_t>((n + kBlock - 1) / kBlock, 1024)), dim3(kBlock), 0,
                     c->stream, n, md, ab, scale ? scale->d : nullptr, alpha, beta, word);
  if (e == hipSuccess) e = hipGetLastError();
  unsigned long long bits = 0;
  if (e == hipSuccess) e = hipMemcpyAsync(&bits, word, sizeof(bits), hipMemcpyDeviceToHost, c->stream);
  if (e == hipSuccess) e = hipStreamSynchronize(c->stream);
  (void)hipFree(work);
  HIP_TRY(e);
  memcpy(lambda_max, &bits, sizeof(bits));
  return STORM_HIP_OK;
}

extern "C" {

int storm_hip_op_get_stats(const storm_hip_op *op, storm_hip_op_stats *s) {
  STORM_REQUIRE(op && s, "op_get_stats: null argument");
  s->n_rows = op->n_rows;
  s->n_cols = op->n_rows + op->n_halo;
  s->nnz_offdiag = op->nnz;
  s->ell_slots = op->ell_slots;
  s->tail_nnz = op->tail_nnz;
  s->tail_rows = op->tail_rows;
  s->n_slices = op->n_slices;
  s->max_row_len = op->max_row_len;
  s->n_interior_slices = op->n_interior_slices;
  s->device_bytes = op->device_bytes;
  s->record_bytes = op->pack_bytes;
  s->value_dictionary_size = op->dict_size;
  s->offset_dictionary_size = op->offs_size;
  s->paired_rows = op->pair;
  CanonTileArgs T;
  int nbt = 0;
  s->tiled_planes = canon_tile_geometry(op, &T, &nbt, op->d_bnd_pack != nullptr) ? canon_tile_planes(op) : 0;
  s->spmv_blocks = spmv_grid_blocks(op);
  s->xcd_run_blocks = op->xcd_group_sell;
  const bool idx = s->tiled_planes > 0 && op->ctx->opt_spmv_record_index != 0 && op->rec_words > 0;
  s->streamed_record_bytes = idx ? op->n_slices * 2 * kWave + (int64_t)sizeof(uint64_t) * op->rec_words : op->pack_bytes;
  return STORM_HIP_OK;
}

int storm_hip_op_destroy(storm_hip_op *op) {
  if (!op) return STORM_HIP_OK;
  if (op->ctx) (void)storm_hip_ctx_sync(op->ctx);
  (void)hipFree(op->d_interior);
  (void)hipFree(op->d_boundary);
  (void)hipFree(op->d_slice_off);
  (void)hipFree(op->d_pack);
  (void)hipFree(op->d_bnd_pack);
  (void)hipFree(op->d_rec_idx);
  (void)hipFree(op->d_rec_words);
  (void)hipFree(op->d_dict);
  (void)hipFree(op->d_offs);
  (void)hipFree(op->d_tail_row);
  (void)hipFree(op->d_tail_ptr);
  (void)hipFree(op->d_tail_col);
  (void)hipFree(op->d_tail_val);
  (void)hipFree(op->d_lat_pack);
  (void)hipFree(op->d_lat_off);
  (void)hipFree(op->d_src);
  (void)hipFree(op->d_tail_src);
  (void)hipFree(op->d_face_inner);
  (void)hipFree(op->d_face_outer);
  (void)hipFree(op->d_pack32);
  (void)hipFree(op->d_slice_off32);
  (void)hipFree(op->d_tail_val32);
  (void)hipFree(op->halo.d_send_idx);
  (void)hipFree(op->halo.d_sendbuf);
  delete op;
  return STORM_HIP_OK;
}

}
```

stormruler_amd/csrc/spmv_build.hip:

```cpp
#include <algorithm>
#include <utility>

#include <hip/hip_runtime.h>

#include "common.hpp"
#include "host_threads.hpp"

namespace storm {

template <class T>
static int upload(T **dst, const std::vector<T> &src, int64_t *bytes) {
  const size_t nbytes = sizeof(T) * (src.size() ? src.size() : 1);
  hipError_t e = hipMalloc((void **)dst, nbytes);
  if (e != hipSuccess) STORM_FAIL(STORM_HIP_E_ALLOC, "hipMalloc(%zu) failed: %s", nbytes, hipGetErrorString(e));
  if (!src.empty()) HIP_TRY(hipMemcpy(*dst, src.data(), sizeof(T) * src.size(), hipMemcpyHostToDevice));
  *bytes += (int64_t)nbytes;
  return STORM_HIP_OK;
}

int op_upload_slice_lists(storm_hip_op *op) {
  if (op->d_interior || op->d_boundary) return STORM_HIP_OK;
  int64_t bytes = 0;
  STORM_TRY(upload(&op->d_interior, op->h_interior, &bytes));
  STORM_TRY(upload(&op->d_boundary, op->h_boundary, &bytes));
  op->n_interior = (int64_t)op->h_interior.size();
  op->n_boundary = (int64_t)op->h_boundary.size();
  op->int_plane0 = op->int_plane1 = 0;
  if (op->pair == 2 && op->canon_k == 6 && op->n_interior > 0) {
    const int64_t b = op->canon_off[5], g0 = op->h_interior.front(), g1 = (int64_t)op->h_interior.back() + 1;
    const int64_t r0 = g0 * 2 * kWave, r1 = std::min<int64_t>(op->n_rows, g1 * 2 * kWave);
    if (b > 0 && g1 - g0 == op->n_interior && r0 % b == 0 && (r1 % b == 0 || r1 == op->n_rows))
      op->int_plane0 = r0 / b, op->int_plane1 = (r1 + b - 1) / b;
  }
  op->device_bytes += bytes;
  return STORM_HIP_OK;
}

static int op_upload_arrays(storm_hip_ctx *c, const OpImage &img, storm_hip_op *op) {
  HIP_TRY(hipSetDevice(c->device));
  BuildTimer timer;
  int64_t bytes = 0;
  if (!img.lat_off.empty()) {
    HIP_TRY(hipMalloc((void **)&op->d_lat_pack, img.lat_pack.size() ? img.lat_pack.size() : 1));
    HIP_TRY(hipMalloc((void **)&op->d_lat_off, sizeof(int64_t) * img.lat_off.size()));
    HIP_TRY(hipMemcpy(op->d_lat_pack, img.lat_pack.data(), img.lat_pack.size(), hipMemcpyHostToDevice));
    HIP_TRY(hipMemcpy(op->d_lat_off, img.lat_off.data(), sizeof(int64_t) * img.lat_off.size(), hipMemcpyHostToDevice));
    op->lat_bytes = (int64_t)img.lat_pack.size();
  }
  if (!img.dict.empty()) STORM_TRY(upload(&op->d_dict, img.dict, &bytes));
  if (!img.offs.empty()) STORM_TRY(upload(&op->d_offs, img.offs, &bytes));
  STORM_TRY(upload(&op->d_slice_off, img.slice_off, &bytes));
  STORM_TRY(upload(&op->d_pack, img.pack, &bytes));
  STORM_TRY(upload(&op->d_tail_row, img.tail_row, &bytes));
  STORM_TRY(upload(&op->d_tail_ptr, img.tail_ptr, &bytes));
  STORM_TRY(upload(&op->d_tail_col, img.tail_col, &bytes));
  STORM_TRY(upload(&op->d_tail_val, img.tail_val, &bytes));
  if (!img.rec_words.empty()) {
    STORM_TRY(upload(&op->d_rec_idx, img.rec_idx, &bytes));
    STORM_TRY(upload(&op->d_rec_words, img.rec_words, &bytes));
  }
  if (!img.bnd_pack.empty()) {
    STORM_TRY(upload(&op->d_bnd_pack, img.bnd_pack, &bytes));
    STORM_TRY(op_upload_slice_lists(op));
  }
  if (img.updatable) {
    STORM_TRY(upload(&op->d_src, img.src, &bytes));
    STORM_TRY(upload(&op->d_tail_src, img.tail_src, &bytes));
    STORM_TRY(upload(&op->d_face_inner, img.face_inner, &bytes));
    STORM_TRY(upload(&op->d_face_outer, img.face_outer, &bytes));
  }
  timer.lap("upload");
  op->device_bytes += bytes;
  return partials_reserve(c, 8 * (((op->n_rows + kWave - 1) / kWave + 3) / 4) + 16 + 2 * kMaxMulti);
}

static int op_upload(storm_hip_ctx *c, OpImage &&img, storm_hip_op **out) {
  auto *op = new storm_hip_op();
  op->ctx = c;
  op->n_rows = img.n_rows, op->n_halo = img.n_halo, op->nnz = img.nnz;
  op->n_slices = img.n_slices, op->max_row_len = img.max_row_len, op->ell_slots = img.ell_slots;
  op->uniform_width = img.uniform_width, op->pair = img.pair, op->bnd_width = img.bnd_width;
  op->canon_k = img.canon_k, op->canon_m1 = img.canon_m1;
  std::copy(img.canon_off, img.canon_off + 7, op->canon_off);
  op->dict_size = img.dict_size, op->offs_size = img.offs_size, op->rec_words = (int)img.rec_words.size();
  op->spw = img.spw, op->tail_rows = img.tail_rows, op->tail_nnz = img.tail_nnz, op->pack_bytes = img.pack_bytes;
  op->xcd_group_sell = (int)c->opt_spmv_xcd_remap_sell;
  op->updatable = img.updatable, op->n_faces = img.n_faces;
  op->h_interior = std::move(img.interior), op->h_boundary = std::move(img.boundary);
  op->n_interior_slices = (int64_t)op->h_interior.size();
  const int st = op_upload_arrays(c, img, op);
  if (st != STORM_HIP_OK) {
    storm_hip_op_destroy(op);
    return st;
  }
  *out = op;
  return STORM_HIP_OK;
}

static PackOptions pack_options(const storm_hip_ctx *c) {
  PackOptions o;
  o.ell_cap = c->opt_ell_cap, o.spmv_dict = c->opt_spmv_dict, o.spmv_mixed = c->opt_spmv_mixed, o.spmv_spw = c->opt_spmv_spw;
  o.latency_path = c->opt_latency_path, o.latency_rows = c->opt_latency_rows;
  return o;
}

int op_create_csr_fp64(storm_hip_ctx *c, int64_t n_rows, const int64_t *row_ptr, const int64_t *col, const double *val,
                       bool source_map, storm_hip_op **out) {
  *out = nullptr;
  PackOptions o = pack_options(c);
  o.spmv_dict = 0, o.latency_path = 0;
  OpImage img;
  if (!source_map) {
    STORM_TRY(op_pack_csr(o, n_rows, 0, row_ptr, col, val, &img));
    return op_upload(c, std::move(img), out);
  }
  STORM_REQUIRE(n_rows >= 0 && row_ptr[n_rows] < (int64_t)INT32_MAX, "amg: a level operator of %lld entries exceeds int32 source ids",
                (long long)row_ptr[n_rows]);
  std::vector<int64_t> rp((size_t)n_rows + 1, 0);
  std::vector<int> oc, src;
  std::vector<double> ov, ext((size_t)n_rows, 0.0);
  for (int64_t i = 0; i < n_rows; ++i) {
    double rowsum = 0.0;
    for (int64_t k = row_ptr[i]; k < row_ptr[i + 1]; ++k) {
      STORM_REQUIRE(col[k] >= 0 && col[k] < n_rows, "amg: column %lld of row %lld outside [0, %lld)", (long long)col[k], (long long)i,
                    (long long)n_rows);
      rowsum += val[k];
      if (col[k] != i) oc.push_back((int)col[k]), ov.push_back(val[k]), src.push_back((int)k);
    }
    ext[(size_t)i] = rowsum;
    rp[(size_t)i + 1] = (int64_t)oc.size();
  }
  STORM_TRY(op_pack(o, n_rows, 0, rp, oc, ov, ext, &img, &src));
  img.updatable = 1, img.n_faces = 0;
  STORM_TRY(op_upload(c, std::move(img), out));
  (*out)->updatable = 0;
  return STORM_HIP_OK;
}

}

using namespace storm;

extern "C" {

int storm_hip_op_create_from_face_weights(storm_hip_ctx *c, int64_t n_owned, int64_t n_halo,
                                          int64_t n_faces, const int64_t *inner, const int64_t *outer,
                                          const double *w_inner, const double *w_outer,
                                          const double *diag_extra, storm_hip_op **out) {
  STORM_REQUIRE(c && out, "op_create: null argument");
  *out = nullptr;
  OpImage img;
  STORM_TRY(op_pack_from_face_weights(pack_options(c), n_owned, n_halo, n_faces, inner, outer, w_inner, w_outer, diag_extra, &img));
  return op_upload(c, std::move(img), out);
}

int storm_hip_op_create_from_face_weights_updatable(storm_hip_ctx *c, int64_t n_owned, int64_t n_halo, int64_t n_faces,
                                                    const int64_t *inner, const int64_t *outer, const double *w_inner,
                                                    const double *w_outer, const double *diag_extra, storm_hip_op **out) {
  STORM_REQUIRE(c && out, "op_create: null argument");
  *out = nullptr;
  OpImage img;
  PackOptions o = pack_options(c);
  o.updatable = 1;
  STORM_TRY(op_pack_from_face_weights(o, n_owned, n_halo, n_faces, inner, outer, w_inner, w_outer, diag_extra, &img));
  return op_upload(c, std::move(img), out);
}

int storm_hip_op_create_from_faces(storm_hip_ctx *c, int64_t n_owned, int64_t n_halo, int64_t n_faces,
                                   const int64_t *inner, const int64_t *outer, const double *coef,
                                   int64_t n_bfaces, const int64_t *b_cell, const double *b_coef,
                                   const double *volume, storm_hip_op **out) {
  STORM_REQUIRE(c && out, "op_create_from_faces: null argument");
  *out = nullptr;
  OpImage img;
  STORM_TRY(op_pack_from_faces(pack_options(c), n_owned, n_halo, n_faces, inner, outer, coef, n_bfaces, b_cell, b_coef, volume, &img));
  return op_upload(c, std::move(img), out);
}

int storm_hip_op_create_from_mesh(storm_hip_ctx *c, int64_t n_owned, int64_t n_halo, int32_t dim, int64_t n_faces,
                                  const int64_t *inner, const int64_t *outer, const double *area, const double *center,
                                  int64_t n_bfaces, const int64_t *b_cell, const double *b_area, const double *b_center,
                                  const double *volume, storm_hip_op **out) {
  STORM_REQUIRE(c && out, "op_create_from_mesh: null argument");
  *out = nullptr;
  OpImage img;
  STORM_TRY(op_pack_from_mesh(pack_options(c), n_owned, n_halo, dim, n_faces, inner, outer, area, center, n_bfaces, b_cell, b_area,
                              b_center, volume, &img));
  return op_upload(c, std::move(img), out);
}

int storm_hip_op_create_csr(storm_hip_ctx *c, int64_t n_rows, int64_t n_halo, const int64_t *row_ptr,
                            const int64_t *col, const double *val, storm_hip_op **out) {
  STORM_REQUIRE(c && out && row_ptr, "op_create_csr: null argument");
  *out = nullptr;
  OpImage img;
  STORM_TRY(op_pack_csr(pack_options(c), n_rows, n_halo, row_ptr, col, val, &img));
  return op_upload(c, std::move(img), out);
}

}
```

stormruler_amd/csrc/spmv_device.hpp:

```cpp
#pragma once
#include <hip/hip_ext.h>

#include <type_traits>

#include "common.hpp"
#include "op_layout.hpp"
#include "ticket_device.hpp"
#include "ipc_device.hpp"
#include "wave_device.hpp"

namespace storm {

__device__ __forceinline__ double ld_scal2(const Scal &s) { return s.p ? (*s.p) * s.sign : s.v; }

typedef int int2v __attribute__((ext_vector_type(2)));
typedef double double2v __attribute__((ext_vector_type(2)));
typedef unsigned long long u64x2 __attribute__((ext_vector_type(2)));

struct SellArgs {
  const char *__restrict__ pack;
  const int64_t *__restrict__ slice_off;
  int64_t n_rows;
  int uniform_width;
  int xcd_group;
  const double *__restrict__ dict;
  int dict_size;
  const int *__restrict__ offs;
  int offs_size;
  int accumulate;
  int rec_by_pos = 0;
  const uint8_t *__restrict__ rec_idx = nullptr;
  const unsigned long long *__restrict__ rec_words = nullptr;
  int rec_words_n = 0;
};

struct DotArgs {
  const double *w;
  double *partials;
  int yy;
  int nblocks_total;
  int block_offset;
  int *tickets = nullptr;
  double *part2 = nullptr;
  double *out0 = nullptr, *out1 = nullptr;
};

struct IpcFused {
  IpcDev w;
  IpcSendPlan sp;
  IpcRecvPlan rp;
};
struct IpcSendArgs {
  IpcDev w;
  IpcSendPlan sp;
};
struct IpcRecvArgs {
  IpcDev w;
  IpcRecvPlan rp;
  int n_halo;
};

__device__ __forceinline__ int xcd_remap(int b, int nb) {
  const int q = nb / kNumXcd, r = nb % kNumXcd;
  const int x = b % kNumXcd, j = b / kNumXcd;
  return x * q + (x < r ? x : r) + j;
}
__device__ __forceinline__ int xcd_remap_grouped(int b, int nb, int G) {
  const int span = kNumXcd * G;
  if (b >= (nb / span) * span) return b;
  const int x = b % kNumXcd, j = b / kNumXcd;
  return ((j / G) * kNumXcd + x) * G + (j % G);
}

template <bool NT>
__device__ __forceinline__ int ld_i(const int *p) {
  return NT ? __builtin_nontemporal_load(p) : *p;
}
template <bool NT>
__device__ __forceinline__ double ld_d(const double *p) {
  return NT ? __builtin_nontemporal_load(p) : *p;
}

struct CanonArgs {
  int off[7];
  int max_gather;
  int reverse;
  int xcd_shift;
  int xcd_full;
};
template <int CTRL>
__device__ __forceinline__ double dpp_shift(double v) {
  int lo = __double2loint(v), hi = __double2hiint(v);
  lo = __builtin_amdgcn_update_dpp(0, lo, CTRL, 0xf, 0xf, false);
  hi = __builtin_amdgcn_update_dpp(0, hi, CTRL, 0xf, 0xf, false);
  return __hiloint2double(hi, lo);
}

constexpr int kTileRun = 4 * 4 * kWave;
struct CanonTileArgs {
  int a, b;
  unsigned a_magic;
  int tiles_per_plane;
  int per_xcd;
  int max_gather;
  int reverse;
  int plane0, plane_end;
};
struct CgFuseArgs {
  const long long *iteration;
  long long my_iteration;
  const double *ca, *cb;
  double *x;
  const double *r;
  double *p_out;
  double ca_imm, cb_imm;
};

template <bool IDX>
using RecRaw = typename std::conditional<IDX, unsigned, u64x2>::type;
__device__ __forceinline__ void rec_table_fill(const SellArgs &A, unsigned long long *words_sh) {
  for (int i = threadIdx.x; i < A.rec_words_n; i += kBlock) words_sh[i] = A.rec_words[i];
}
template <bool IDX>
__device__ __forceinline__ RecRaw<IDX> rec_load(const SellArgs &A, uint32_t rc) {
  if constexpr (IDX) return __builtin_nontemporal_load(reinterpret_cast<const unsigned short *>(A.rec_idx + rc));
  else return __builtin_nontemporal_load(reinterpret_cast<const u64x2 *>(A.pack + (size_t)(rc << 3)));
}
template <bool IDX>
__device__ __forceinline__ u64x2 rec_word(RecRaw<IDX> v, const unsigned long long *words_sh) {
  if constexpr (IDX) return u64x2{words_sh[v & 0xffu], words_sh[v >> 8]};
  else return v;
}

__device__ __forceinline__ double2v lattice_pair_apply(const double *dict_sh, u64x2 w, const double2v (&xg)[6], double2v c,
                                                       double alpha, double beta) {
  double acc_a = 0.0, acc_b = 0.0;
#pragma unroll
  for (int k = 0; k < 6; ++k) {
    const unsigned ba = (unsigned)(w.x >> (8 * (k + 1))) & 0xffu, bb = (unsigned)(w.y >> (8 * (k + 1))) & 0xffu;
    acc_a += *reinterpret_cast<const double *>(reinterpret_cast<const char *>(dict_sh) + ba) * (xg[k].x - c.x);
    acc_b += *reinterpret_cast<const double *>(reinterpret_cast<const char *>(dict_sh) + bb) * (xg[k].y - c.y);
  }
  const double ext_a = *reinterpret_cast<const double *>(reinterpret_cast<const char *>(dict_sh) + ((unsigned)w.x & 0xffu));
  const double ext_b = *reinterpret_cast<const double *>(reinterpret_cast<const char *>(dict_sh) + ((unsigned)w.y & 0xffu));
  double2v yi;
  yi.x = __builtin_fma(alpha, __builtin_fma(ext_a, c.x, acc_a), beta * c.x);
  yi.y = __builtin_fma(alpha, __builtin_fma(ext_b, c.y, acc_b), beta * c.y);
  return yi;
}
__device__ __forceinline__ void march_neighbours(const double *buf, int at, int a, int lane, double2v below, double2v above,
                                                 double2v c, double2v (&xg)[6]) {
  xg[0] = below, xg[5] = above;
  xg[1] = *reinterpret_cast<const double2v *>(&buf[at - a]);
  xg[4] = *reinterpret_cast<const double2v *>(&buf[at + a]);
  double el = 0.0;
  if (lane == 0) el = buf[at - 1];
  if (lane == kWave - 1) el = buf[at + 2];
  const double left = dpp_shift<0x138>(c.y);
  const double right = dpp_shift<0x130>(c.x);
  xg[2].x = lane == 0 ? el : left;
  xg[2].y = c.x;
  xg[3].x = c.y;
  xg[3].y = lane == kWave - 1 ? el : right;
}

struct MarchArgs {
  CanonTileArgs T;
  int zc_planes;
  int apply_begin, apply_end;
  int alternate;
};

struct RangeLaunch {
  const storm_hip_op *op;
  int nb;
  Scal alpha, beta;
  const double *x;
  double *y;
  const int *slice_list;
  int64_t n_launch;
  DotArgs dot;
  bool want_dot;
  const int *done;
  hipEvent_t ev0, ev1;
  bool accumulate;
  const IpcFused *fused;
  const CgFuseArgs *cg_fuse;
};
bool spmv_tile_run(const RangeLaunch &L);
bool spmv_canon_run(const RangeLaunch &L);
bool spmv_pair_run(const RangeLaunch &L);
bool spmv_dict_run(const RangeLaunch &L);
bool spmv_sell_run(const RangeLaunch &L);
int spmv_tail_run(const storm_hip_op *op, Scal alpha, const double *x, double *y, const int *done);
int spmv_march_run(const storm_hip_op *op, const MarchArgs &M, int n_blocks, Scal alpha, Scal beta, const double *x, double *y,
                   const DotArgs &dot, const int *done, const CgFuseArgs &cgf, const IpcSendArgs &S);
SellArgs lattice_args(const storm_hip_op *op);

constexpr int kCanonGroups = 2;
static inline int op_spw(const storm_hip_op *op) {
  if (op->pair) return 1;
  return (op->dict_size > 0 && op->uniform_width > 0) ? (int)op->spw : 1;
}
static inline int blocks_for(const storm_hip_op *op, int64_t n_launch_slices, bool boundary_of_mixed = false) {
  const int64_t per_block = (kBlock / kWave) * ((op->pair >= 2 && !boundary_of_mixed) ? kCanonGroups : op_spw(op));
  return (int)((n_launch_slices + per_block - 1) / per_block);
}
static inline bool boundary_of_mixed(const RangeLaunch &L) {
  return L.op->d_bnd_pack != nullptr && L.slice_list != nullptr && L.slice_list == L.op->d_boundary;
}
static inline SellArgs paired_args(const RangeLaunch &L, int *width) {
  const storm_hip_op *op = L.op;
  const int group = (L.slice_list == nullptr || L.slice_list == op->d_interior) ? (int)op->ctx->opt_spmv_xcd_remap : 0;
  SellArgs A{op->d_pack, op->d_slice_off, op->n_rows, op->uniform_width, group, op->d_dict, op->dict_size,
             op->d_offs, op->offs_size, (int)L.accumulate};
  *width = op->uniform_width;
  if (boundary_of_mixed(L)) {
    A.pack = op->d_bnd_pack, A.rec_by_pos = 1;
    *width = op->bnd_width;
  } else if (op->ctx->opt_spmv_record_index != 0 && op->rec_words > 0) {
    A.rec_idx = op->d_rec_idx, A.rec_words = reinterpret_cast<const unsigned long long *>(op->d_rec_words), A.rec_words_n = op->rec_words;
  }
  return A;
}
int canon_tile_planes(const storm_hip_op *op);
bool canon_tile_geometry(const storm_hip_op *op, CanonTileArgs *T, int *n_blocks, bool interior = false);
bool cg_march_geometry(const storm_hip_op *op, MarchArgs *M, int *n_blocks, bool partitioned = false);

}
```

stormruler_amd/csrc/spmv_lattice.hip:

```cpp
#include <algorithm>

#include "spmv_device.hpp"

namespace storm {

template <bool DOT, bool WLOAD, int TZ, int HL, bool FUSE, bool IDX>
__global__ __launch_bounds__(kBlock) void spmv_canon_tile_kernel(SellArgs A, CanonTileArgs T, Scal alpha_s, Scal beta_s,
                                                                 const double *__restrict__ x, double *__restrict__ y,
                                                                 DotArgs dot, const int *done, IpcSendArgs S, CgFuseArgs F) {
  if (!FUSE && (int)blockIdx.x < S.sp.n_blocks) {
    ipc_halo_send_block(S.w, S.sp, x, (int)blockIdx.x);
    return;
  }
  if (FUSE && *F.iteration < F.my_iteration) return;
  const int done_flag = done ? *done : 0;
  const double cg_a = FUSE ? *F.ca : 0.0, cg_b = FUSE ? *F.cb : 0.0;
  const char *rb_ = reinterpret_cast<const char *>(F.r);
  extern __shared__ __attribute__((aligned(16))) double tile_sh[];
  __shared__ double dict_sh[32];
  const int lane = threadIdx.x & (kWave - 1);
  const int wave = __builtin_amdgcn_readfirstlane(threadIdx.x >> 6);
  const int n_tiles = (int)gridDim.x - S.sp.n_blocks, tb = (int)blockIdx.x - S.sp.n_blocks;
  const int bidx = T.reverse ? n_tiles - 1 - tb : tb;
  int zc, yt;
  if (T.per_xcd > 0) {
    const int xcd = bidx & (kNumXcd - 1), j = bidx >> 3;
    zc = j / T.per_xcd;
    yt = xcd * T.per_xcd + (j - zc * T.per_xcd);
  } else {
    zc = bidx / T.tiles_per_plane;
    yt = bidx - zc * T.tiles_per_plane;
  }
  const int a = T.a, b = T.b;
  const int p0 = yt * kTileRun, z0 = T.plane0 + zc * TZ;
  const int ldw = kTileRun + 2 * a;
  const double alpha = ld_scal2(alpha_s), beta = ld_scal2(beta_s);
  const uint32_t last_row = (uint32_t)(A.n_rows - 1);
  const bool w_is_x = DOT && dot.w == x;
  const char *xb = reinterpret_cast<const char *>(x);
  const char *xg_base = xb - (size_t)kVecGuard * 8;
  char *yb = reinterpret_cast<char *>(y);
  unsigned long long *words_sh = reinterpret_cast<unsigned long long *>(tile_sh + TZ * ldw);

  const double dict_word = A.dict[lane & 31];
  bool valid_a[TZ][2], valid_b[TZ][2];
  uint32_t rc[TZ][2];
  double2v xi[TZ][2];
#pragma unroll
  for (int t = 0; t < TZ; ++t)
#pragma unroll
    for (int g = 0; g < 2; ++g) {
      const int q = p0 + 256 * wave + 128 * g + 2 * lane;
      const int64_t row = (int64_t)(z0 + t) * b + q;
      const bool in_plane = q < b && z0 + t < T.plane_end;
      valid_a[t][g] = in_plane && row <= (int64_t)last_row, valid_b[t][g] = in_plane && row + 1 <= (int64_t)last_row;
      rc[t][g] = row <= (int64_t)last_row ? (uint32_t)row : (last_row & ~1u);
      xi[t][g] = *reinterpret_cast<const double2v *>(xb + (size_t)(rc[t][g] << 3));
    }
  if (FUSE) {
#pragma unroll
    for (int t = 0; t < TZ; ++t)
#pragma unroll
      for (int g = 0; g < 2; ++g) {
        double2v *xp_ = reinterpret_cast<double2v *>(reinterpret_cast<char *>(F.x) + (size_t)(rc[t][g] << 3));
        const double2v xv = __builtin_nontemporal_load(xp_);
        const double2v rv = *reinterpret_cast<const double2v *>(rb_ + (size_t)(rc[t][g] << 3));
        double2v xn, pn;
        xn.x = __builtin_fma(cg_a, xi[t][g].x, xv.x), xn.y = __builtin_fma(cg_a, xi[t][g].y, xv.y);
        pn.x = __builtin_fma(cg_b, xi[t][g].x, rv.x), pn.y = __builtin_fma(cg_b, xi[t][g].y, rv.y);
        if (valid_b[t][g]) __builtin_nontemporal_store(xn, xp_);
        else if (valid_a[t][g]) F.x[rc[t][g]] = xn.x;
        xi[t][g] = pn;
        if (!done_flag) {
          double2v *pp_ = reinterpret_cast<double2v *>(reinterpret_cast<char *>(F.p_out) + (size_t)(rc[t][g] << 3));
          if (valid_b[t][g]) __builtin_nontemporal_store(pn, pp_);
          else if (valid_a[t][g]) F.p_out[rc[t][g]] = pn.x;
        }
      }
    if (done_flag) return;
  }
  const char *rg_base = FUSE ? rb_ - (size_t)kVecGuard * 8 : nullptr;
  double2v halo[HL];
  int halo_at[HL];
#pragma unroll
  for (int i = 0; i < HL; ++i) {
    const unsigned h = threadIdx.x + (unsigned)kBlock * i;
    const unsigned t = __umulhi(h, T.a_magic), u = h - t * (unsigned)a;
    const bool on = t < (unsigned)TZ;
    const int jj = (int)(2 * u) < a ? (int)(2 * u) - a : kTileRun + (int)(2 * u) - a;
    int64_t gi = (int64_t)(z0 + (int)t) * b + p0 + jj + kVecGuard;
    gi = gi < 0 ? 0 : gi;
    gi = gi > (int64_t)T.max_gather ? (int64_t)T.max_gather : gi;
    halo_at[i] = on ? (int)t * ldw + a + jj : -1;
    halo[i] = double2v{0.0, 0.0};
    if (on) halo[i] = *reinterpret_cast<const double2v *>(xg_base + (size_t)((uint32_t)gi << 3));
    if (FUSE && on) {
      const double2v rv = *reinterpret_cast<const double2v *>(rg_base + (size_t)((uint32_t)gi << 3));
      halo[i].x = __builtin_fma(cg_b, halo[i].x, rv.x), halo[i].y = __builtin_fma(cg_b, halo[i].y, rv.y);
    }
  }
  RecRaw<IDX> vw[TZ][2];
  double2v wi[WLOAD ? TZ : 1][2];
#pragma unroll
  for (int t = 0; t < TZ; ++t)
#pragma unroll
    for (int g = 0; g < 2; ++g) {
      vw[t][g] = rec_load<IDX>(A, rc[t][g]);
      if (WLOAD) wi[t][g] = *reinterpret_cast<const double2v *>(reinterpret_cast<const char *>(dot.w) + (size_t)(rc[t][g] << 3));
    }
  double2v xlo[2], xhi[2];
#pragma unroll
  for (int g = 0; g < 2; ++g) {
    int lo = (int)rc[0][g] - b + kVecGuard, hi = (int)rc[TZ - 1][g] + b + kVecGuard;
    lo = lo < 0 ? 0 : lo;
    hi = hi > T.max_gather ? T.max_gather : hi;
    xlo[g] = *reinterpret_cast<const double2v *>(xg_base + (size_t)((uint32_t)lo << 3));
    xhi[g] = *reinterpret_cast<const double2v *>(xg_base + (size_t)((uint32_t)hi << 3));
    if (FUSE) {
      const double2v rl = *reinterpret_cast<const double2v *>(rg_base + (size_t)((uint32_t)lo << 3));
      const double2v rh = *reinterpret_cast<const double2v *>(rg_base + (size_t)((uint32_t)hi << 3));
      xlo[g].x = __builtin_fma(cg_b, xlo[g].x, rl.x), xlo[g].y = __builtin_fma(cg_b, xlo[g].y, rl.y);
      xhi[g].x = __builtin_fma(cg_b, xhi[g].x, rh.x), xhi[g].y = __builtin_fma(cg_b, xhi[g].y, rh.y);
    }
  }
  if (lane < 32) dict_sh[lane] = dict_word;
  if (IDX) rec_table_fill(A, words_sh);
#pragma unroll
  for (int t = 0; t < TZ; ++t)
#pragma unroll
    for (int g = 0; g < 2; ++g)
      *reinterpret_cast<double2v *>(&tile_sh[t * ldw + a + 256 * wave + 128 * g + 2 * lane]) = xi[t][g];
#pragma unroll
  for (int i = 0; i < HL; ++i)
    if (halo_at[i] >= 0) *reinterpret_cast<double2v *>(&tile_sh[halo_at[i]]) = halo[i];
  __syncthreads();
  double dot_a = 0.0, dot_b = 0.0;
#pragma unroll
  for (int t = 0; t < TZ; ++t)
#pragma unroll
    for (int g = 0; g < 2; ++g) {
      const int at = t * ldw + a + 256 * wave + 128 * g + 2 * lane;
      double2v xg[6];
      xg[0] = t == 0 ? xlo[g] : xi[t == 0 ? 0 : t - 1][g];
      xg[5] = t == TZ - 1 ? xhi[g] : xi[t == TZ - 1 ? t : t + 1][g];
      xg[1] = *reinterpret_cast<const double2v *>(&tile_sh[at - a]);
      xg[4] = *reinterpret_cast<const double2v *>(&tile_sh[at + a]);
      double el = 0.0;
      if (lane == 0) el = tile_sh[at - 1];
      if (lane == kWave - 1) el = tile_sh[at + 2];
      const double left = dpp_shift<0x138>(xi[t][g].y);
      const double right = dpp_shift<0x130>(xi[t][g].x);
      xg[2].x = lane == 0 ? el : left;
      xg[2].y = xi[t][g].x;
      xg[3].x = xi[t][g].y;
      xg[3].y = lane == kWave - 1 ? el : right;
      const u64x2 w = rec_word<IDX>(vw[t][g], words_sh);
      double acc_a = 0.0, acc_b = 0.0;
#pragma unroll
      for (int k = 0; k < 6; ++k) {
        const unsigned ba = (unsigned)(w.x >> (8 * (k + 1))) & 0xffu, bb = (unsigned)(w.y >> (8 * (k + 1))) & 0xffu;
        acc_a += *reinterpret_cast<const double *>(reinterpret_cast<const char *>(dict_sh) + ba) * (xg[k].x - xi[t][g].x);
        acc_b += *reinterpret_cast<const double *>(reinterpret_cast<const char *>(dict_sh) + bb) * (xg[k].y - xi[t][g].y);
      }
      const double ext_a = *reinterpret_cast<const double *>(reinterpret_cast<const char *>(dict_sh) + ((unsigned)w.x & 0xffu));
      const double ext_b = *reinterpret_cast<const double *>(reinterpret_cast<const char *>(dict_sh) + ((unsigned)w.y & 0xffu));
      double2v yi;
      yi.x = __builtin_fma(alpha, __builtin_fma(ext_a, xi[t][g].x, acc_a), beta * xi[t][g].x);
      yi.y = __builtin_fma(alpha, __builtin_fma(ext_b, xi[t][g].y, acc_b), beta * xi[t][g].y);
      if (!done_flag) {
        double2v *yp = reinterpret_cast<double2v *>(yb + (size_t)(rc[t][g] << 3));
        if (valid_b[t][g]) *yp = yi;
        else if (valid_a[t][g]) y[rc[t][g]] = yi.x;
      }
      if (DOT) {
        yi.x = valid_a[t][g] ? yi.x : 0.0;
        yi.y = valid_b[t][g] ? yi.y : 0.0;
        const double2v wv = WLOAD ? wi[WLOAD ? t : 0][g] : xi[t][g];
        const double pa = dot.w ? wv.x * yi.x + wv.y * yi.y : 0.0;
        const double pb = yi.x * yi.x + yi.y * yi.y;
        dot_a = (t == 0 && g == 0) ? pa : dot_a + pa;
        dot_b = (t == 0 && g == 0) ? pb : dot_b + pb;
      }
    }
  (void)w_is_x;
  if (done_flag) return;
  if (DOT) {
    dot_a = wave_sum_to_lane63(dot_a);
    if (dot.yy) dot_b = wave_sum_to_lane63(dot_b);
    if (dot.tickets == nullptr) {
      if (lane == kWave - 1) {
        const int slot = dot.block_offset + bidx * (kBlock / kWave) + wave;
        dot.partials[slot] = dot_a;
        if (dot.yy) dot.partials[dot.nblocks_total + slot] = dot_b;
      }
    } else {
      __shared__ double wave_part[2 * (kBlock / kWave)];
      if (lane == kWave - 1) wave_part[wave] = dot_a, wave_part[kBlock / kWave + wave] = dot.yy ? dot_b : 0.0;
      __syncthreads();
      if (wave != 0) return;
      const double mine[2] = {(wave_part[0] + wave_part[1]) + (wave_part[2] + wave_part[3]),
                              (wave_part[4] + wave_part[5]) + (wave_part[6] + wave_part[7])};
      double total[2];
      const TicketArgs tk{dot.tickets, dot.partials, dot.part2};
      if (ticket_reduce_wave0<2>(tk, mine, dot.yy ? 2 : 1, (unsigned)bidx, (unsigned)n_tiles, total) && lane == 0) {
        *dot.out0 = total[0];
        if (dot.yy) *dot.out1 = total[1];
      }
    }
  }
}

template <int HLP, bool IDX>
__global__ __launch_bounds__(kBlock) void cg_step_march_kernel(SellArgs A, MarchArgs M, Scal alpha_s, Scal beta_s,
                                                               const double *__restrict__ p_in, double *__restrict__ z_out,
                                                               DotArgs dot, const int *done, CgFuseArgs F, IpcSendArgs S) {
  if ((int)blockIdx.x < S.sp.n_blocks) {
    ipc_halo_send_block(S.w, S.sp, p_in, (int)blockIdx.x, F.r, *F.cb);
    return;
  }
  if (F.iteration != nullptr && *F.iteration < F.my_iteration) return;
  const int done_flag = done ? *done : 0;
  const CanonTileArgs &T = M.T;
  extern __shared__ __attribute__((aligned(16))) double tile_sh[];
  __shared__ double dict_sh[32];
  const int lane = threadIdx.x & (kWave - 1);
  const int wave = __builtin_amdgcn_readfirstlane(threadIdx.x >> 6);
  const int n_march = (int)gridDim.x - S.sp.n_blocks, mb = (int)blockIdx.x - S.sp.n_blocks;
  const int bidx = T.reverse ? n_march - 1 - mb : mb;
  int zc, yt;
  if (T.per_xcd > 0) {
    const int xcd = bidx & (kNumXcd - 1), j = bidx >> 3;
    zc = j / T.per_xcd;
    yt = xcd * T.per_xcd + (j - zc * T.per_xcd);
  } else {
    zc = bidx / T.tiles_per_plane;
    yt = bidx - zc * T.tiles_per_plane;
  }
  const int a = T.a, b = T.b;
  const int p0 = yt * kTileRun;
  const int z_begin = zc * M.zc_planes, z_end = min(z_begin + M.zc_planes, T.plane_end);
  const int ldw = kTileRun + 2 * a;
  const double alpha = ld_scal2(alpha_s), beta = ld_scal2(beta_s);
  const double cg_a = F.ca ? *F.ca : F.ca_imm, cg_b = F.cb ? *F.cb : F.cb_imm;
  const uint32_t last_row = (uint32_t)(A.n_rows - 1);
  const char *pb = reinterpret_cast<const char *>(p_in), *rb = reinterpret_cast<const char *>(F.r);
  const char *pg_base = pb - (size_t)kVecGuard * 8, *rg_base = rb - (size_t)kVecGuard * 8;
  unsigned long long *words_sh = reinterpret_cast<unsigned long long *>(tile_sh + 3 * ldw);
  const double dict_word = A.dict[lane & 31];
  if (lane < 32) dict_sh[lane] = dict_word;
  if (IDX) rec_table_fill(A, words_sh);

  struct Flight {
    double2v p[2], r[2], x[2], hp[HLP], hr[HLP];
    RecRaw<IDX> w[2];
    uint32_t rc[2];
    bool va[2], vb[2];
    int hat[HLP];
  };
  auto issue = [&](int zp, bool own, Flight &f) {
#pragma unroll
    for (int g = 0; g < 2; ++g) {
      const int q = p0 + 256 * wave + 128 * g + 2 * lane;
      const int64_t row = (int64_t)zp * b + q;
      const bool in_plane = q < b && own;
      f.va[g] = in_plane && row <= (int64_t)last_row, f.vb[g] = in_plane && row + 1 <= (int64_t)last_row;
      int64_t gi = row + kVecGuard;
      gi = gi < 0 ? 0 : gi;
      gi = gi > (int64_t)T.max_gather ? (int64_t)T.max_gather : gi;
      f.rc[g] = (row >= 0 && row <= (int64_t)last_row) ? (uint32_t)row : (last_row & ~1u);
      f.p[g] = *reinterpret_cast<const double2v *>(pg_base + (size_t)((uint32_t)gi << 3));
      f.r[g] = *reinterpret_cast<const double2v *>(rg_base + (size_t)((uint32_t)gi << 3));
      if (own) {
        f.x[g] = __builtin_nontemporal_load(reinterpret_cast<const double2v *>(reinterpret_cast<const char *>(F.x) + (size_t)(f.rc[g] << 3)));
        f.w[g] = rec_load<IDX>(A, f.rc[g]);
      }
    }
#pragma unroll
    for (int i = 0; i < HLP; ++i) {
      const int u = (int)threadIdx.x + kBlock * i;
      const bool on = own && u < a;
      const int jj = 2 * u < a ? 2 * u - a : kTileRun + 2 * u - a;
      int64_t gi = (int64_t)zp * b + p0 + jj + kVecGuard;
      gi = gi < 0 ? 0 : gi;
      gi = gi > (int64_t)T.max_gather ? (int64_t)T.max_gather : gi;
      f.hat[i] = on ? a + jj : -1;
      f.hp[i] = f.hr[i] = double2v{0.0, 0.0};
      if (on) {
        f.hp[i] = *reinterpret_cast<const double2v *>(pg_base + (size_t)((uint32_t)gi << 3));
        f.hr[i] = *reinterpret_cast<const double2v *>(rg_base + (size_t)((uint32_t)gi << 3));
      }
    }
  };
  auto consume = [&](bool own, const Flight &f, double2v (&out)[2], double *buf) {
#pragma unroll
    for (int g = 0; g < 2; ++g) {
      double2v pn;
      pn.x = __builtin_fma(cg_b, f.p[g].x, f.r[g].x), pn.y = __builtin_fma(cg_b, f.p[g].y, f.r[g].y);
      out[g] = pn;
      if (own) {
        double2v *pp_ = reinterpret_cast<double2v *>(reinterpret_cast<char *>(F.p_out) + (size_t)(f.rc[g] << 3));
        double2v xn;
        xn.x = __builtin_fma(cg_a, f.p[g].x, f.x[g].x), xn.y = __builtin_fma(cg_a, f.p[g].y, f.x[g].y);
        double2v *xp_ = reinterpret_cast<double2v *>(reinterpret_cast<char *>(F.x) + (size_t)(f.rc[g] << 3));
        if (f.vb[g]) __builtin_nontemporal_store(xn, xp_), __builtin_nontemporal_store(pn, pp_);
        else if (f.va[g]) F.x[f.rc[g]] = xn.x, F.p_out[f.rc[g]] = pn.x;
        *reinterpret_cast<double2v *>(&buf[a + 256 * wave + 128 * g + 2 * lane]) = pn;
      }
    }
    if (own) {
#pragma unroll
      for (int i = 0; i < HLP; ++i)
        if (f.hat[i] >= 0) {
          double2v hn;
          hn.x = __builtin_fma(cg_b, f.hp[i].x, f.hr[i].x), hn.y = __builtin_fma(cg_b, f.hp[i].y, f.hr[i].y);
          *reinterpret_cast<double2v *>(&buf[f.hat[i]]) = hn;
        }
    }
  };

  if (done_flag) {
    for (int zp = z_begin; zp < z_end; ++zp) {
#pragma unroll
      for (int g = 0; g < 2; ++g) {
        const int q = p0 + 256 * wave + 128 * g + 2 * lane;
        const int64_t row = (int64_t)zp * b + q;
        if (q < b && row <= (int64_t)last_row) {
          double2v *xp_ = reinterpret_cast<double2v *>(reinterpret_cast<char *>(F.x) + (size_t)((uint32_t)row << 3));
          if (row + 1 <= (int64_t)last_row) {
            const double2v pv = *reinterpret_cast<const double2v *>(pb + (size_t)((uint32_t)row << 3));
            double2v xv = *xp_;
            xv.x = __builtin_fma(cg_a, pv.x, xv.x), xv.y = __builtin_fma(cg_a, pv.y, xv.y);
            *xp_ = xv;
          } else {
            F.x[row] = __builtin_fma(cg_a, p_in[row], F.x[row]);
          }
        }
      }
    }
    return;
  }

  double2v pm[2], pc[2], pn[2];
  RecRaw<IDX> wc[2];
  uint32_t rcc[2];
  bool vac[2], vbc[2];
  Flight fl;
  const bool down = M.alternate != 0 && (zc & 1) != 0;
  const int nz = z_end - z_begin;
  auto plane = [&](int s) { return down ? z_end - 1 - s : z_begin + s; };
  auto lds_of = [&](int zp) { return tile_sh + ((zp % 3 + 3) % 3) * ldw; };
  issue(plane(-1), false, fl);
  consume(false, fl, pm, nullptr);
  issue(plane(0), true, fl);
  consume(true, fl, pc, lds_of(plane(0)));
#pragma unroll
  for (int g = 0; g < 2; ++g) wc[g] = fl.w[g], rcc[g] = fl.rc[g], vac[g] = fl.va[g], vbc[g] = fl.vb[g];
  issue(plane(1), 1 < nz, fl);
  double dot_a = 0.0, dot_b = 0.0;
  for (int s = 0; s < nz; ++s) {
    const int zp = plane(s);
    const bool next_own = s + 1 < nz;
    RecRaw<IDX> wn[2];
    uint32_t rcn[2];
    bool van[2], vbn[2];
    consume(next_own, fl, pn, lds_of(plane(s + 1)));
#pragma unroll
    for (int g = 0; g < 2; ++g) wn[g] = fl.w[g], rcn[g] = fl.rc[g], van[g] = fl.va[g], vbn[g] = fl.vb[g];
    if (s + 2 <= nz) issue(plane(s + 2), s + 2 < nz, fl);
    __syncthreads();
    const double *buf = lds_of(zp);
    const bool applies = zp >= M.apply_begin && zp < M.apply_end;
#pragma unroll
    for (int g = 0; g < 2; ++g) {
      if (!applies) break;
      const int at = a + 256 * wave + 128 * g + 2 * lane;
      double2v xg[6];
      march_neighbours(buf, at, a, lane, down ? pn[g] : pm[g], down ? pm[g] : pn[g], pc[g], xg);
      double2v yi = lattice_pair_apply(dict_sh, rec_word<IDX>(wc[g], words_sh), xg, pc[g], alpha, beta);
      if (z_out != nullptr) {
        double2v *yp = reinterpret_cast<double2v *>(reinterpret_cast<char *>(z_out) + (size_t)(rcc[g] << 3));
        if (vbc[g]) *yp = yi;
        else if (vac[g]) z_out[rcc[g]] = yi.x;
      }
      yi.x = vac[g] ? yi.x : 0.0;
      yi.y = vbc[g] ? yi.y : 0.0;
      dot_a += pc[g].x * yi.x + pc[g].y * yi.y;
      dot_b += yi.x * yi.x + yi.y * yi.y;
    }
#pragma unroll
    for (int g = 0; g < 2; ++g)
      pm[g] = pc[g], pc[g] = pn[g], wc[g] = wn[g], rcc[g] = rcn[g], vac[g] = van[g], vbc[g] = vbn[g];
  }
  dot_a = wave_sum_to_lane63(dot_a);
  if (dot.yy) dot_b = wave_sum_to_lane63(dot_b);
  if (dot.tickets == nullptr) {
    if (lane == kWave - 1) {
      const int slot = dot.block_offset + bidx * (kBlock / kWave) + wave;
      dot.partials[slot] = dot_a;
      if (dot.yy) dot.partials[dot.nblocks_total + slot] = dot_b;
    }
    return;
  }
  __shared__ double wave_part[2 * (kBlock / kWave)];
  if (lane == kWave - 1) wave_part[wave] = dot_a, wave_part[kBlock / kWave + wave] = dot.yy ? dot_b : 0.0;
  __syncthreads();
  if (wave != 0) return;
  const double mine[2] = {(wave_part[0] + wave_part[1]) + (wave_part[2] + wave_part[3]),
                          (wave_part[4] + wave_part[5]) + (wave_part[6] + wave_part[7])};
  double total[2];
  const TicketArgs tk{dot.tickets, dot.partials, dot.part2};
  if (ticket_reduce_wave0<2>(tk, mine, dot.yy ? 2 : 1, (unsigned)bidx, (unsigned)n_march, total) && lane == 0) {
    *dot.out0 = total[0];
    if (dot.yy) *dot.out1 = total[1];
  }
}


int canon_tile_planes(const storm_hip_op *op) {
  const int64_t tz = op->ctx->opt_spmv_canon_tile;
  return tz == 4 ? 4 : 2;
}
bool canon_tile_geometry(const storm_hip_op *op, CanonTileArgs *T, int *n_blocks, bool interior) {
  if (op->ctx->opt_spmv_canon_tile == 0 || op->pair != 2 || op->canon_k != 6 || op->canon_m1 != 2) return false;
  if (interior != (op->d_bnd_pack != nullptr)) return false;
  if (interior && op->int_plane1 <= op->int_plane0) return false;
  const int *o = op->canon_off;
  const int a = o[4], b = o[5];
  if (o[0] != -b || o[1] != -a || o[2] != -1 || o[3] != 1) return false;
  if (a < 2 || a > 512 || (a & 1) || (b & 1) || b < 2 * a) return false;
  const int tz = canon_tile_planes(op);
  if ((int64_t)sizeof(double) * tz * (kTileRun + 2 * a) > 60 * 1024) return false;
  const int64_t plane0 = interior ? op->int_plane0 : 0, plane1 = interior ? op->int_plane1 : (op->n_rows + b - 1) / b;
  const int64_t planes = plane1 - plane0;
  if (planes < 2 * tz || op->n_rows < op->ctx->opt_spmv_canon_tile_min_rows) return false;
  T->a = a, T->b = b;
  T->a_magic = (unsigned)((((uint64_t)1 << 32) + (uint64_t)a - 1) / (uint64_t)a);
  T->tiles_per_plane = (b + kTileRun - 1) / kTileRun;
  T->per_xcd = (T->tiles_per_plane % kNumXcd == 0 && op->ctx->opt_spmv_xcd_remap != 0) ? T->tiles_per_plane / kNumXcd : 0;
  T->max_gather = (int)(op->n_rows + op->n_halo) + kVecGuard + 2;
  T->reverse = op->ctx->spmv_reverse;
  T->plane0 = (int)plane0, T->plane_end = (int)plane1;
  *n_blocks = (int)(((planes + tz - 1) / tz) * T->tiles_per_plane);
  return true;
}

bool cg_march_geometry(const storm_hip_op *op, MarchArgs *M, int *n_blocks, bool partitioned) {
  const int64_t zc = op->ctx->opt_cg_march;
  int nbt = 0;
  if (zc < 2 || !canon_tile_geometry(op, &M->T, &nbt, partitioned)) return false;
  if ((int64_t)sizeof(double) * 3 * (kTileRun + 2 * M->T.a) > 60 * 1024) return false;
  if (partitioned && op->n_rows % M->T.b != 0) return false;
  const int64_t planes = (op->n_rows + M->T.b - 1) / M->T.b;
  const int64_t want = op->ctx->opt_cg_march_fill;
  const int64_t fill = want > 0 ? planes * M->T.tiles_per_plane / want : zc;
  M->zc_planes = (int)std::min<int64_t>(std::min<int64_t>(zc, std::max<int64_t>(2, fill)), planes);
  M->alternate = (int)(op->ctx->opt_cg_march_alternate != 0);
  M->apply_begin = partitioned ? (int)op->int_plane0 : 0;
  M->apply_end = partitioned ? (int)op->int_plane1 : (int)planes;
  M->T.plane0 = 0, M->T.plane_end = (int)planes;
  const int64_t chunks = (planes + M->zc_planes - 1) / M->zc_planes;
  *n_blocks = (int)(chunks * M->T.tiles_per_plane);
  return true;
}

template <bool DOT>
static bool launch_tile(const RangeLaunch &L, SellArgs A) {
  const storm_hip_op *op = L.op;
  const int nb = L.nb;
  hipStream_t st = op->ctx->stream;
  const Scal alpha = L.alpha, beta = L.beta;
  const double *x = L.x;
  double *y = L.y;
  const DotArgs dot = L.dot;
  const int *done = L.done;
  hipEvent_t ev0 = L.ev0, ev1 = L.ev1;
  const CgFuseArgs *cg_fuse = L.cg_fuse;
  CanonTileArgs T;
  int tile_blocks = 0;
  const bool interior_list = L.slice_list != nullptr && L.slice_list == op->d_interior;
  IpcSendArgs S{};
  if (L.fused != nullptr && interior_list) S.w = L.fused->w, S.sp = L.fused->sp;
  if (!(op->pair == 2 && !boundary_of_mixed(L) && (L.slice_list == nullptr || interior_list) && !L.accumulate &&
        canon_tile_geometry(op, &T, &tile_blocks, interior_list) && tile_blocks + S.sp.n_blocks == nb))
    return false;
  const int tz = canon_tile_planes(op);
  const int hl_need = (tz * T.a + kBlock - 1) / kBlock;
  const size_t lds = sizeof(double) * (size_t)tz * (size_t)(kTileRun + 2 * T.a) + sizeof(uint64_t) * (size_t)A.rec_words_n;
  const bool wload = DOT && dot.w != nullptr && dot.w != x;
#define TILE_GO4(WL_, TZ_, HL_, FU_, IX_, CGF_)                                                                             \
  hipExtLaunchKernelGGL((spmv_canon_tile_kernel<DOT, WL_, TZ_, HL_, FU_, IX_>), dim3(nb), dim3(kBlock), lds, st, ev0, ev1, 0, A, \
                        T, alpha, beta, x, y, dot, done, S, CGF_)
#define TILE_GO3(WL_, TZ_, HL_, FU_, CGF_)                                 \
  do {                                                                     \
    if (A.rec_idx != nullptr) TILE_GO4(WL_, TZ_, HL_, FU_, true, CGF_);   \
    else TILE_GO4(WL_, TZ_, HL_, FU_, false, CGF_);                        \
  } while (0)
#define TILE_GO2(TZ_, HL_)                                               \
  do {                                                                   \
    if (cg_fuse != nullptr) {                                            \
      if constexpr (DOT) TILE_GO3(false, TZ_, HL_, true, *cg_fuse);      \
    } else if (wload) TILE_GO3(true, TZ_, HL_, false, CgFuseArgs{});     \
    else TILE_GO3(false, TZ_, HL_, false, CgFuseArgs{});                 \
  } while (0)
#define TILE_GO(TZ_)                       \
  do {                                     \
    if (hl_need <= 1) TILE_GO2(TZ_, 1);     \
    else if (hl_need <= 2) TILE_GO2(TZ_, 2); \
    else if (hl_need <= 4) TILE_GO2(TZ_, 4); \
    else TILE_GO2(TZ_, 8);                  \
  } while (0)
  if (tz == 2) TILE_GO(2);
  else TILE_GO(4);
#undef TILE_GO
#undef TILE_GO2
#undef TILE_GO3
#undef TILE_GO4
  return true;
}

SellArgs lattice_args(const storm_hip_op *op) {
  SellArgs A{op->d_pack, op->d_slice_off, op->n_rows, op->uniform_width, 0, op->d_dict, op->dict_size, op->d_offs, op->offs_size, 0};
  if (op->ctx->opt_spmv_record_index != 0 && op->rec_words > 0)
    A.rec_idx = op->d_rec_idx, A.rec_words = reinterpret_cast<const unsigned long long *>(op->d_rec_words), A.rec_words_n = op->rec_words;
  return A;
}

bool spmv_tile_run(const RangeLaunch &L) {
  if (L.op->pair != 2) return false;
  int width = 0;
  const SellArgs A = paired_args(L, &width);
  return L.want_dot ? launch_tile<true>(L, A) : launch_tile<false>(L, A);
}

int spmv_march_run(const storm_hip_op *op, const MarchArgs &M, int n_blocks, Scal alpha, Scal beta, const double *x, double *y,
                   const DotArgs &dot, const int *done, const CgFuseArgs &cgf, const IpcSendArgs &S) {
  storm_hip_ctx *c = op->ctx;
  hipEvent_t ev0 = nullptr, ev1 = nullptr;
  if (c->opt_profile_spmv != 0) {
    while (c->prof_events.size() < c->prof_used + 2) {
      hipEvent_t ev;
      HIP_TRY(hipEventCreate(&ev));
      c->prof_events.push_back(ev);
    }
    ev0 = c->prof_events[c->prof_used], ev1 = c->prof_events[c->prof_used + 1];
    c->prof_used += 2;
  }
  const SellArgs A = lattice_args(op);
  const size_t lds = sizeof(double) * 3 * (size_t)(kTileRun + 2 * M.T.a) + sizeof(uint64_t) * (size_t)A.rec_words_n;
  const int nb = n_blocks + S.sp.n_blocks;
#define MARCH_GO(HLP_, IX_)                                                                                                 \
  hipExtLaunchKernelGGL((cg_step_march_kernel<HLP_, IX_>), dim3(nb), dim3(kBlock), lds, c->stream, ev0, ev1, 0, A, M, alpha, \
                        beta, x, y, dot, done, cgf, S)
  STORM_REQUIRE(cgf.x != nullptr, "spmv: the marching step updates x");
  if (M.T.a <= kBlock) {
    if (A.rec_idx != nullptr) MARCH_GO(1, true);
    else MARCH_GO(1, false);
  } else {
    if (A.rec_idx != nullptr) MARCH_GO(2, true);
    else MARCH_GO(2, false);
  }
#undef MARCH_GO
  HIP_TRY(hipGetLastError());
  return STORM_HIP_OK;
}

}
```

Before: 5462.

## Deduplicate per-plane record index into a small plane table with slot map

At build time, identical z-planes of the per-row record index are hashed and deduplicated into a small table of unique planes plus a per-plane slot map. The SpMV tile, marching CG step and residual-planes kernels then read record indices from this small table, indexed by slot and in-plane position, instead of streaming a full index over all rows. This targets the HBM traffic of the index stream in the bandwidth-bound stencil SpMV. The cost is extra slot lookups, more kernel template variants, and a host-side hashing pass that falls back to the old path when planes are not repetitive enough.

```diff
diff --git a/include/storm_hip.h b/include/storm_hip.h
--- a/include/storm_hip.h
+++ b/include/storm_hip.h
@@ -210,6 +210,7 @@
   int64_t spmv_blocks;
   int64_t xcd_run_blocks;
   int64_t streamed_record_bytes;
+  int64_t record_plane_bytes;
 } storm_hip_op_stats;
 int storm_hip_op_get_stats(const storm_hip_op *op, storm_hip_op_stats *stats);
 int storm_hip_op_destroy(storm_hip_op *op);
diff --git a/stormruler_amd/_lib.py b/stormruler_amd/_lib.py
--- a/stormruler_amd/_lib.py
+++ b/stormruler_amd/_lib.py
@@ -41,7 +41,7 @@
                                           "tail_rows", "n_slices", "max_row_len", "n_interior_slices",
                                           "device_bytes", "record_bytes", "value_dictionary_size",
                                           "offset_dictionary_size", "paired_rows", "tiled_planes", "spmv_blocks", "xcd_run_blocks",
-                                          "streamed_record_bytes")]
+                                          "streamed_record_bytes", "record_plane_bytes")]
 
 
 class MeshView(C.Structure):
diff --git a/stormruler_amd/csrc/common.hpp b/stormruler_amd/csrc/common.hpp
--- a/stormruler_amd/csrc/common.hpp
+++ b/stormruler_amd/csrc/common.hpp
@@ -138,6 +138,7 @@
   int spmv_reverse = 0;
   int64_t opt_spmv_canon_tile_min_rows = (int64_t)1 << 20;
   int64_t opt_spmv_record_index = 1;
+  int64_t opt_spmv_record_planes = 1;
   int64_t opt_spmv_canon_tile = 2;
   int64_t opt_mgs_steps = 4;
   int64_t opt_resident_early = 1;
@@ -278,6 +279,9 @@
   uint8_t *d_rec_idx = nullptr;
   uint64_t *d_rec_words = nullptr;
   int rec_words = 0;
+  uint8_t *d_rec_planes = nullptr;
+  int *d_rec_slot = nullptr;
+  int64_t rec_planes_bytes = 0;
   char *d_bnd_pack = nullptr;
   int bnd_width = 0;
   int canon_k = 0, canon_m1 = -1;
@@ -436,6 +440,8 @@
   std::vector<int> offs;
   std::vector<uint8_t> rec_idx;
   std::vector<uint64_t> rec_words;
+  std::vector<uint8_t> rec_planes;
+  std::vector<int> rec_slot;
   std::vector<char> bnd_pack;
   std::vector<int> tail_row;
   std::vector<int64_t> tail_ptr;
diff --git a/stormruler_amd/csrc/context.hip b/stormruler_amd/csrc/context.hip
--- a/stormruler_amd/csrc/context.hip
+++ b/stormruler_amd/csrc/context.hip
@@ -218,6 +218,7 @@
   else if (!strcmp(key, "cg_residual_fill")) c->opt_cg_residual_fill = value;
   else if (!strcmp(key, "cg_pz_fold")) c->opt_cg_pz_fold = value;
   else if (!strcmp(key, "spmv_record_index")) c->opt_spmv_record_index = value;
+  else if (!strcmp(key, "spmv_record_planes")) c->opt_spmv_record_planes = value;
   else if (!strcmp(key, "blas1_nt")) c->opt_blas1_nt = value;
   else if (!strcmp(key, "cheb_fused")) c->opt_cheb_fused = value;
   else if (!strcmp(key, "amg_fused")) c->opt_amg_fused = value;
diff --git a/stormruler_amd/csrc/op_pack.hip b/stormruler_amd/csrc/op_pack.hip
--- a/stormruler_amd/csrc/op_pack.hip
+++ b/stormruler_amd/csrc/op_pack.hip
@@ -361,6 +361,47 @@
     for (int64_t i = b; i < e; ++i) rec_idx[(size_t)i] = (uint8_t)wd.lookup(word_at(i));
   });
   rec_words = std::move(wd.values);
+}
+
+constexpr int64_t kRecPlanesMaxBytes = 1 << 20;
+void record_planes(const std::vector<uint8_t> &rec_idx, int64_t b, int64_t n_rows, std::vector<uint8_t> &rec_planes,
+                   std::vector<int> &rec_slot) {
+  const int64_t n_idx = (int64_t)rec_idx.size();
+  if (n_idx == 0 || b <= 0 || n_rows < 2 * b) return;
+  const int64_t planes = (n_idx + b - 1) / b, whole = n_rows / b;
+  std::vector<uint64_t> hash((size_t)planes, 0);
+  parallel_chunks(whole, 1, [&](int, int64_t z0, int64_t z1) {
+    for (int64_t z = z0; z < z1; ++z) {
+      uint64_t h = 0xcbf29ce484222325ull;
+      for (const uint8_t *p = rec_idx.data() + z * b, *e = p + b; p < e; ++p) h = (h ^ *p) * 0x100000001b3ull;
+      hash[(size_t)z] = h;
+    }
+  });
+  std::vector<int64_t> first;
+  std::vector<std::pair<uint64_t, int>> seen;
+  std::vector<int> slot((size_t)planes, 0);
+  for (int64_t z = 0; z < planes; ++z) {
+    int s = -1;
+    if (z < whole) {
+      const auto key = std::make_pair(hash[(size_t)z], 0);
+      for (auto it = std::lower_bound(seen.begin(), seen.end(), key); s < 0 && it != seen.end() && it->first == key.first; ++it)
+        if (memcmp(rec_idx.data() + z * b, rec_idx.data() + first[(size_t)it->second] * b, (size_t)b) == 0) s = it->second;
+    }
+    if (s < 0) {
+      s = (int)first.size();
+      first.push_back(z);
+      if (2 * (int64_t)first.size() > planes || (int64_t)first.size() * b > kRecPlanesMaxBytes) return;
+      if (z < whole) {
+        const auto key = std::make_pair(hash[(size_t)z], s);
+        seen.insert(std::upper_bound(seen.begin(), seen.end(), key), key);
+      }
+    }
+    slot[(size_t)z] = s;
+  }
+  rec_planes.assign(first.size() * (size_t)b, 0);
+  for (size_t s = 0; s < first.size(); ++s)
+    memcpy(rec_planes.data() + s * (size_t)b, rec_idx.data() + first[s] * b, (size_t)std::min<int64_t>(b, n_idx - first[s] * b));
+  rec_slot = std::move(slot);
 }
 
 std::vector<int> slice_widths(const Rows &A, int64_t cap, int64_t slot_bytes, int64_t w_op, OpImage *img) {
@@ -497,6 +538,7 @@
     canonical_records(A, vd, (uint64_t)vd.index(0.0) << 3, grp_bnd, canon, img->pack);
     timer.lap("canonical order + records");
     row_record_index(img->pack, img->rec_idx, img->rec_words);
+    if (canon_len == 6) record_planes(img->rec_idx, canon[5], n, img->rec_planes, img->rec_slot);
     timer.lap("row-record index");
     img->canon_k = canon_len, img->canon_m1 = canon_m1;
     for (int k = 0; k < canon_len; ++k) img->canon_off[k] = (int)canon[k];
diff --git a/stormruler_amd/csrc/solver_cg.hip b/stormruler_amd/csrc/solver_cg.hip
--- a/stormruler_amd/csrc/solver_cg.hip
+++ b/stormruler_amd/csrc/solver_cg.hip
@@ -192,7 +192,7 @@
   int max_gather;
 };
 constexpr int kResidualMaxChunk = 32;
-template <int HLP, bool IDX>
+template <int HLP, int IDX>
 __global__ __launch_bounds__(kBlock) void cg_r_planes_kernel(SolverState *st, double *__restrict__ r, const double *__restrict__ p,
                                                              SellArgs A, ResidualPlanesArgs G, Scal alpha_s, Scal beta_s,
                                                              const double *__restrict__ pz_partials, int n_pz, int reverse,
@@ -249,16 +249,19 @@
       if (own && hat[i] >= 0) f.hp[i] = load_p(row0 + hjj[i]);
     }
   };
-  auto issue_rw = [&](int zp, double2v (&vr)[kUnroll], RecRaw<IDX> (&w)[kUnroll]) {
+  auto slot_of = [&](int zp) { return IDX == kRecPlanes ? rec_plane_slot(A, min(zp, G.planes - 1)) : 0; };
+  auto issue_rw = [&](int zp, double2v (&vr)[kUnroll], RecRaw<IDX> (&w)[kUnroll], int slot) {
     const int64_t row0 = (int64_t)zp * b + p0;
 #pragma unroll
     for (int u = 0; u < kUnroll; ++u) {
       const int64_t row = row0 + 2 * ((int)threadIdx.x + kBlock * u);
       vr[u] = r2[row >> 1];
-      w[u] = rec_load<IDX>(A, (uint32_t)row);
-    }
-  };
-
+      w[u] = rec_load<IDX>(A, slot, p0 + 2 * ((int)threadIdx.x + kBlock * u), (uint32_t)row);
+    }
+  };
+
+  const int slot0 = slot_of(plane(0));
+  int slot_next = slot_of(plane(1));
   Flight cur, nxt, fl;
   double2v pm[kUnroll], vr[kUnroll];
   RecRaw<IDX> w[kUnroll];
@@ -266,7 +269,7 @@
 #pragma unroll
   for (int u = 0; u < kUnroll; ++u) pm[u] = fl.p[u];
   issue_p(plane(0), true, cur);
-  issue_rw(plane(0), vr, w);
+  issue_rw(plane(0), vr, w, slot0);
   issue_p(plane(1), 1 < nz, nxt);
   const bool folds = pz_partials != nullptr;
   FoldWhole pz_flight;
@@ -279,6 +282,7 @@
   for (int s = 0; s < nz; ++s) {
     const int zp = plane(s);
     double *buf = plane_sh + (s & 1) * ldw;
+    const int slot_after = slot_of(plane(s + 2));
 #pragma unroll
     for (int u = 0; u < kUnroll; ++u) *reinterpret_cast<double2v *>(&buf[a + 2 * ((int)threadIdx.x + kBlock * u)]) = cur.p[u];
 #pragma unroll
@@ -287,7 +291,7 @@
     double2v vrn[kUnroll];
     RecRaw<IDX> wn[kUnroll];
     if (s + 2 <= nz) issue_p(plane(s + 2), s + 2 < nz, fl);
-    if (s + 1 < nz) issue_rw(plane(s + 1), vrn, wn);
+    if (s + 1 < nz) issue_rw(plane(s + 1), vrn, wn, slot_next);
     __syncthreads();
     const int64_t i0 = (((int64_t)zp * b + p0) >> 1) + threadIdx.x;
     double acc = 0.0;
@@ -306,7 +310,7 @@
     if (lane == 0) wave_part[s * (kBlock / kWave) + wave] = acc;
 #pragma unroll
     for (int u = 0; u < kUnroll; ++u) pm[u] = cur.p[u], vr[u] = vrn[u], w[u] = wn[u];
-    cur = nxt, nxt = fl;
+    cur = nxt, nxt = fl, slot_next = slot_after;
   }
   __syncthreads();
   if (threadIdx.x >= kWave) return;
@@ -351,11 +355,13 @@
   hipLaunchKernelGGL((cg_r_planes_kernel<HLP_, IX_>), dim3(n_blocks), dim3(kBlock), lds, c->stream, st, r, p, A, G, alpha, beta, \
                      pz_partials, n_pz, reverse, tk)
   if (G.a <= kBlock) {
-    if (A.rec_idx != nullptr) PLANES_GO(1, true);
-    else PLANES_GO(1, false);
+    if (A.rec_planes != nullptr) PLANES_GO(1, kRecPlanes);
+    else if (A.rec_idx != nullptr) PLANES_GO(1, 1);
+    else PLANES_GO(1, 0);
   } else {
-    if (A.rec_idx != nullptr) PLANES_GO(2, true);
-    else PLANES_GO(2, false);
+    if (A.rec_planes != nullptr) PLANES_GO(2, kRecPlanes);
+    else if (A.rec_idx != nullptr) PLANES_GO(2, 1);
+    else PLANES_GO(2, 0);
   }
 #undef PLANES_GO
   HIP_TRY(hipGetLastError());
diff --git a/stormruler_amd/csrc/spmv.hip b/stormruler_amd/csrc/spmv.hip
--- a/stormruler_amd/csrc/spmv.hip
+++ b/stormruler_amd/csrc/spmv.hip
@@ -447,6 +447,7 @@
   s->xcd_run_blocks = op->xcd_group_sell;
   const bool idx = s->tiled_planes > 0 && op->ctx->opt_spmv_record_index != 0 && op->rec_words > 0;
   s->streamed_record_bytes = idx ? op->n_slices * 2 * kWave + (int64_t)sizeof(uint64_t) * op->rec_words : op->pack_bytes;
+  s->record_plane_bytes = idx && op->ctx->opt_spmv_record_planes != 0 ? op->rec_planes_bytes : 0;
   return STORM_HIP_OK;
 }
 
@@ -460,6 +461,8 @@
   (void)hipFree(op->d_bnd_pack);
   (void)hipFree(op->d_rec_idx);
   (void)hipFree(op->d_rec_words);
+  (void)hipFree(op->d_rec_planes);
+  (void)hipFree(op->d_rec_slot);
   (void)hipFree(op->d_dict);
   (void)hipFree(op->d_offs);
   (void)hipFree(op->d_tail_row);
diff --git a/stormruler_amd/csrc/spmv_build.hip b/stormruler_amd/csrc/spmv_build.hip
--- a/stormruler_amd/csrc/spmv_build.hip
+++ b/stormruler_amd/csrc/spmv_build.hip
@@ -58,6 +58,11 @@
   if (!img.rec_words.empty()) {
     STORM_TRY(upload(&op->d_rec_idx, img.rec_idx, &bytes));
     STORM_TRY(upload(&op->d_rec_words, img.rec_words, &bytes));
+  }
+  if (!img.rec_planes.empty()) {
+    STORM_TRY(upload(&op->d_rec_planes, img.rec_planes, &bytes));
+    STORM_TRY(upload(&op->d_rec_slot, img.rec_slot, &bytes));
+    op->rec_planes_bytes = (int64_t)img.rec_planes.size();
   }
   if (!img.bnd_pack.empty()) {
     STORM_TRY(upload(&op->d_bnd_pack, img.bnd_pack, &bytes));
diff --git a/stormruler_amd/csrc/spmv_device.hpp b/stormruler_amd/csrc/spmv_device.hpp
--- a/stormruler_amd/csrc/spmv_device.hpp
+++ b/stormruler_amd/csrc/spmv_device.hpp
@@ -32,6 +32,9 @@
   const uint8_t *__restrict__ rec_idx = nullptr;
   const unsigned long long *__restrict__ rec_words = nullptr;
   int rec_words_n = 0;
+  const uint8_t *__restrict__ rec_planes = nullptr;
+  const int *__restrict__ rec_slot = nullptr;
+  int rec_b = 0;
 };
 
 struct DotArgs {
@@ -116,19 +119,28 @@
   double ca_imm, cb_imm;
 };
 
-template <bool IDX>
-using RecRaw = typename std::conditional<IDX, unsigned, u64x2>::type;
+template <int IDX>
+using RecRaw = typename std::conditional<IDX != 0, unsigned, u64x2>::type;
 __device__ __forceinline__ void rec_table_fill(const SellArgs &A, unsigned long long *words_sh) {
   for (int i = threadIdx.x; i < A.rec_words_n; i += kBlock) words_sh[i] = A.rec_words[i];
 }
-template <bool IDX>
+template <int IDX>
 __device__ __forceinline__ RecRaw<IDX> rec_load(const SellArgs &A, uint32_t rc) {
-  if constexpr (IDX) return __builtin_nontemporal_load(reinterpret_cast<const unsigned short *>(A.rec_idx + rc));
+  if constexpr (IDX != 0) return __builtin_nontemporal_load(reinterpret_cast<const unsigned short *>(A.rec_idx + rc));
   else return __builtin_nontemporal_load(reinterpret_cast<const u64x2 *>(A.pack + (size_t)(rc << 3)));
 }
-template <bool IDX>
+constexpr int kRecPlanes = 2;
+__device__ __forceinline__ int rec_plane_slot(const SellArgs &A, int z) {
+  return *(const __attribute__((address_space(4))) int *)(A.rec_slot + z);
+}
+template <int IDX>
+__device__ __forceinline__ RecRaw<IDX> rec_load(const SellArgs &A, int slot, int q, uint32_t rc) {
+  if constexpr (IDX == kRecPlanes) return *reinterpret_cast<const unsigned short *>(A.rec_planes + (uint32_t)(slot * A.rec_b + q));
+  else return rec_load<IDX>(A, rc);
+}
+template <int IDX>
 __device__ __forceinline__ u64x2 rec_word(RecRaw<IDX> v, const unsigned long long *words_sh) {
-  if constexpr (IDX) return u64x2{words_sh[v & 0xffu], words_sh[v >> 8]};
+  if constexpr (IDX != 0) return u64x2{words_sh[v & 0xffu], words_sh[v >> 8]};
   else return v;
 }
 
@@ -209,6 +221,10 @@
 static inline bool boundary_of_mixed(const RangeLaunch &L) {
   return L.op->d_bnd_pack != nullptr && L.slice_list != nullptr && L.slice_list == L.op->d_boundary;
 }
+static inline void rec_planes_args(const storm_hip_op *op, SellArgs *A) {
+  if (op->ctx->opt_spmv_record_planes != 0 && op->d_rec_planes != nullptr)
+    A->rec_planes = op->d_rec_planes, A->rec_slot = op->d_rec_slot, A->rec_b = op->canon_off[5];
+}
 static inline SellArgs paired_args(const RangeLaunch &L, int *width) {
   const storm_hip_op *op = L.op;
   const int group = (L.slice_list == nullptr || L.slice_list == op->d_interior) ? (int)op->ctx->opt_spmv_xcd_remap : 0;
@@ -220,6 +236,7 @@
     *width = op->bnd_width;
   } else if (op->ctx->opt_spmv_record_index != 0 && op->rec_words > 0) {
     A.rec_idx = op->d_rec_idx, A.rec_words = reinterpret_cast<const unsigned long long *>(op->d_rec_words), A.rec_words_n = op->rec_words;
+    rec_planes_args(op, &A);
   }
   return A;
 }
diff --git a/stormruler_amd/csrc/spmv_lattice.hip b/stormruler_amd/csrc/spmv_lattice.hip
--- a/stormruler_amd/csrc/spmv_lattice.hip
+++ b/stormruler_amd/csrc/spmv_lattice.hip
@@ -4,7 +4,7 @@
 
 namespace storm {
 
-template <bool DOT, bool WLOAD, int TZ, int HL, bool FUSE, bool IDX>
+template <bool DOT, bool WLOAD, int TZ, int HL, bool FUSE, int IDX>
 __global__ __launch_bounds__(kBlock) void spmv_canon_tile_kernel(SellArgs A, CanonTileArgs T, Scal alpha_s, Scal beta_s,
                                                                  const double *__restrict__ x, double *__restrict__ y,
                                                                  DotArgs dot, const int *done, IpcSendArgs S, CgFuseArgs F) {
@@ -43,6 +43,9 @@
   unsigned long long *words_sh = reinterpret_cast<unsigned long long *>(tile_sh + TZ * ldw);
 
   const double dict_word = A.dict[lane & 31];
+  int rslot[TZ];
+#pragma unroll
+  for (int t = 0; t < TZ; ++t) rslot[t] = IDX == kRecPlanes ? rec_plane_slot(A, min(z0 + t, T.plane_end - 1)) : 0;
   bool valid_a[TZ][2], valid_b[TZ][2];
   uint32_t rc[TZ][2];
   double2v xi[TZ][2];
@@ -105,7 +108,7 @@
   for (int t = 0; t < TZ; ++t)
 #pragma unroll
     for (int g = 0; g < 2; ++g) {
-      vw[t][g] = rec_load<IDX>(A, rc[t][g]);
+      vw[t][g] = rec_load<IDX>(A, rslot[t], min(p0 + 256 * wave + 128 * g + 2 * lane, b - 2), rc[t][g]);
       if (WLOAD) wi[t][g] = *reinterpret_cast<const double2v *>(reinterpret_cast<const char *>(dot.w) + (size_t)(rc[t][g] << 3));
     }
   double2v xlo[2], xhi[2];
@@ -210,7 +213,7 @@
   }
 }
 
-template <int HLP, bool IDX>
+template <int HLP, int IDX>
 __global__ __launch_bounds__(kBlock) void cg_step_march_kernel(SellArgs A, MarchArgs M, Scal alpha_s, Scal beta_s,
                                                                const double *__restrict__ p_in, double *__restrict__ z_out,
                                                                DotArgs dot, const int *done, CgFuseArgs F, IpcSendArgs S) {
@@ -257,7 +260,7 @@
     bool va[2], vb[2];
     int hat[HLP];
   };
-  auto issue = [&](int zp, bool own, Flight &f) {
+  auto issue = [&](int zp, bool own, Flight &f, int slot) {
 #pragma unroll
     for (int g = 0; g < 2; ++g) {
       const int q = p0 + 256 * wave + 128 * g + 2 * lane;
@@ -272,7 +275,7 @@
       f.r[g] = *reinterpret_cast<const double2v *>(rg_base + (size_t)((uint32_t)gi << 3));
       if (own) {
         f.x[g] = __builtin_nontemporal_load(reinterpret_cast<const double2v *>(reinterpret_cast<const char *>(F.x) + (size_t)(f.rc[g] << 3)));
-        f.w[g] = rec_load<IDX>(A, f.rc[g]);
+        f.w[g] = rec_load<IDX>(A, slot, min(q, b - 2), f.rc[g]);
       }
     }
 #pragma unroll
@@ -349,13 +352,16 @@
   const int nz = z_end - z_begin;
   auto plane = [&](int s) { return down ? z_end - 1 - s : z_begin + s; };
   auto lds_of = [&](int zp) { return tile_sh + ((zp % 3 + 3) % 3) * ldw; };
-  issue(plane(-1), false, fl);
+  auto slot_of = [&](int zp) { return IDX == kRecPlanes ? rec_plane_slot(A, max(0, min(zp, T.plane_end - 1))) : 0; };
+  const int slot0 = slot_of(plane(0)), slot1 = slot_of(plane(1));
+  int slot_next = slot_of(plane(2));
+  issue(plane(-1), false, fl, 0);
   consume(false, fl, pm, nullptr);
-  issue(plane(0), true, fl);
+  issue(plane(0), true, fl, slot0);
   consume(true, fl, pc, lds_of(plane(0)));
 #pragma unroll
   for (int g = 0; g < 2; ++g) wc[g] = fl.w[g], rcc[g] = fl.rc[g], vac[g] = fl.va[g], vbc[g] = fl.vb[g];
-  issue(plane(1), 1 < nz, fl);
+  issue(plane(1), 1 < nz, fl, slot1);
   double dot_a = 0.0, dot_b = 0.0;
   for (int s = 0; s < nz; ++s) {
     const int zp = plane(s);
@@ -363,10 +369,12 @@
     RecRaw<IDX> wn[2];
     uint32_t rcn[2];
     bool van[2], vbn[2];
+    const int slot_after = slot_of(plane(s + 3));
     consume(next_own, fl, pn, lds_of(plane(s + 1)));
 #pragma unroll
     for (int g = 0; g < 2; ++g) wn[g] = fl.w[g], rcn[g] = fl.rc[g], van[g] = fl.va[g], vbn[g] = fl.vb[g];
-    if (s + 2 <= nz) issue(plane(s + 2), s + 2 < nz, fl);
+    if (s + 2 <= nz) issue(plane(s + 2), s + 2 < nz, fl, slot_next);
+    slot_next = slot_after;
     __syncthreads();
     const double *buf = lds_of(zp);
     const bool applies = zp >= M.apply_begin && zp < M.apply_end;
@@ -492,8 +500,9 @@
                         T, alpha, beta, x, y, dot, done, S, CGF_)
 #define TILE_GO3(WL_, TZ_, HL_, FU_, CGF_)                                 \
   do {                                                                     \
-    if (A.rec_idx != nullptr) TILE_GO4(WL_, TZ_, HL_, FU_, true, CGF_);   \
-    else TILE_GO4(WL_, TZ_, HL_, FU_, false, CGF_);                        \
+    if (A.rec_planes != nullptr) TILE_GO4(WL_, TZ_, HL_, FU_, kRecPlanes, CGF_); \
+    else if (A.rec_idx != nullptr) TILE_GO4(WL_, TZ_, HL_, FU_, 1, CGF_);  \
+    else TILE_GO4(WL_, TZ_, HL_, FU_, 0, CGF_);                            \
   } while (0)
 #define TILE_GO2(TZ_, HL_)                                               \
   do {                                                                   \
@@ -521,7 +530,7 @@
 SellArgs lattice_args(const storm_hip_op *op) {
   SellArgs A{op->d_pack, op->d_slice_off, op->n_rows, op->uniform_width, 0, op->d_dict, op->dict_size, op->d_offs, op->offs_size, 0};
   if (op->ctx->opt_spmv_record_index != 0 && op->rec_words > 0)
-    A.rec_idx = op->d_rec_idx, A.rec_words = reinterpret_cast<const unsigned long long *>(op->d_rec_words), A.rec_words_n = op->rec_words;
+    A.rec_idx = op->d_rec_idx, A.rec_words = reinterpret_cast<const unsigned long long *>(op->d_rec_words), A.rec_words_n = op->rec_words, rec_planes_args(op, &A);
   return A;
 }
 
@@ -553,11 +562,13 @@
                         beta, x, y, dot, done, cgf, S)
   STORM_REQUIRE(cgf.x != nullptr, "spmv: the marching step updates x");
   if (M.T.a <= kBlock) {
-    if (A.rec_idx != nullptr) MARCH_GO(1, true);
-    else MARCH_GO(1, false);
+    if (A.rec_planes != nullptr) MARCH_GO(1, kRecPlanes);
+    else if (A.rec_idx != nullptr) MARCH_GO(1, 1);
+    else MARCH_GO(1, 0);
   } else {
-    if (A.rec_idx != nullptr) MARCH_GO(2, true);
-    else MARCH_GO(2, false);
+    if (A.rec_planes != nullptr) MARCH_GO(2, kRecPlanes);
+    else if (A.rec_idx != nullptr) MARCH_GO(2, 1);
+    else MARCH_GO(2, 0);
   }
 #undef MARCH_GO
   HIP_TRY(hipGetLastError());
```

After: 5504, median of 6. Within noise of the previous version (+0.8%).
